# play-with-HOI-generation/HOIG

Hardware: AMD Instinct MI355X
Metric: HOGAN train images/sec at 256x256 (higher is better)
Workload: dtype f16x3 fwd (both operands split hi+lo on fp16, 3 MFMAs per product) / bf16x2 bwd (dy split hi+lo, weights and x single bf16, 2 MFMAs per product), f32 accumulate; 1 GPU; 256x256 HO3Dv3-shaped synthetic, batch 8 per GPU, G+D full step (generator_spade_attn, VGG19 surrogate weights); global_batch=8, parallelism=dp1

## Files before the change

hoig_amd/csrc/conv_bf16_common.h:

```cpp
#pragma once
#include "common.h"

namespace hoig_detail {

#define HOIG_NS_SWITCH(ns, ...)                                                \
    do {                                                                       \
        if ((ns) == 2) { constexpr int NSX = 2; __VA_ARGS__; }                 \
        else if ((ns) == 3) { constexpr int NSX = 3; __VA_ARGS__; }            \
        else { constexpr int NSX = 1; __VA_ARGS__; }                           \
    } while (0)
#define HOIG_F16_SWITCH(flag, ...)                                             \
    do {                                                                       \
        if (flag) { constexpr bool F16X = true; __VA_ARGS__; }                 \
        else { constexpr bool F16X = false; __VA_ARGS__; }                     \
    } while (0)
__host__ __device__ constexpr int ns_a(int nsx) { return nsx == 1 ? 1 : 2; }
__host__ __device__ constexpr int ns_b(int nsx) { return nsx == 2 ? 2 : 1; }
inline int ns_of_precision(int precision) {
    return precision == HOIG_PREC_BF16X3 ? 2 : (precision == HOIG_PREC_F16X2 ? 3 : 1);
}
inline bool is_16bit_precision(int precision) {
    return precision == HOIG_PREC_BF16X3 || precision == HOIG_PREC_BF16 || precision == HOIG_PREC_F16X2;
}

typedef __bf16 bf2_t __attribute__((ext_vector_type(2)));
typedef float f2_t __attribute__((ext_vector_type(2)));
__device__ __forceinline__ unsigned cvt2(float a, float b) {
    f2_t v = {a, b};
    return __builtin_bit_cast(unsigned, __builtin_convertvector(v, bf2_t));
}
typedef _Float16 h2_t __attribute__((ext_vector_type(2)));
typedef _Float16 f16x8 __attribute__((ext_vector_type(8)));
constexpr float W_SCALE_F16 = 256.f;
__device__ __forceinline__ unsigned cvt2h(float a, float b) {
    f2_t v = {a, b};
    return __builtin_bit_cast(unsigned, __builtin_convertvector(v, h2_t));
}
__device__ __forceinline__ void split4h(const float4 v, uint2 &hi, uint2 &lo) {
    hi.x = cvt2h(v.x, v.y);
    hi.y = cvt2h(v.z, v.w);
    const h2_t h0 = __builtin_bit_cast(h2_t, hi.x), h1 = __builtin_bit_cast(h2_t, hi.y);
    lo.x = cvt2h(v.x - (float)h0[0], v.y - (float)h0[1]);
    lo.y = cvt2h(v.z - (float)h1[0], v.w - (float)h1[1]);
}
template <bool F16>
__device__ __forceinline__ f32x16 mfma16(const bf16x8 a, const bf16x8 b, const f32x16 c) {
    if constexpr (F16)
        return __builtin_amdgcn_mfma_f32_32x32x16_f16(__builtin_bit_cast(f16x8, a), __builtin_bit_cast(f16x8, b), c, 0, 0, 0);
    else
        return __builtin_amdgcn_mfma_f32_32x32x16_bf16(a, b, c, 0, 0, 0);
}

__device__ __forceinline__ void split4(const float4 v, uint2 &hi, uint2 &lo) {
    hi.x = cvt2(v.x, v.y);
    hi.y = cvt2(v.z, v.w);
    const float r0 = v.x - __uint_as_float(hi.x << 16), r1 = v.y - __uint_as_float(hi.x & 0xFFFF0000u);
    const float r2 = v.z - __uint_as_float(hi.y << 16), r3 = v.w - __uint_as_float(hi.y & 0xFFFF0000u);
    lo.x = cvt2(r0, r1);
    lo.y = cvt2(r2, r3);
}
template <bool F16>
__device__ __forceinline__ void split4t(const float4 v, uint2 &hi, uint2 &lo) {
    if constexpr (F16) split4h(v, hi, lo);
    else split4(v, hi, lo);
}

__host__ __device__ __forceinline__ size_t plane_index(int n, int k, int K) {
    return ((size_t)(n >> 5) * (K >> 5) + (k >> 5)) * 1024 + (n & 31) * 32 + (((((k & 31) >> 3) ^ ((n >> 2) & 3))) << 3) +
           (k & 7);
}

struct HaloArgs {
    const float *A = nullptr;
    const unsigned short *Wh = nullptr, *Wl = nullptr;
    const float *bias = nullptr;
    float *C = nullptr;
    int Bn = 0, H = 0, W = 0, Cg = 0;
    int N = 0, K = 0;
    int pad = 0;
    int flip = 0;
    int act = 0;
    float slope = 0.f;
    int nblk_n = 0, nblk = 0;
    int tiles_x = 0, tiles_y = 0;
    int nmajor = 0;
    int f16 = 0;
    float oscale = 0.f;
    const float *A2 = nullptr;
    int cg1 = 0;
    float *C2 = nullptr;
    int n1 = 0;
    const float *addend = nullptr;
    const float *in_scale = nullptr, *in_shift = nullptr;
    int in_relu_c0 = 0;
    int b_split = 0;
    const float *A_g2 = nullptr;
    const unsigned short *Wh_g2 = nullptr, *Wl_g2 = nullptr;
    const float *bias_g2 = nullptr, *addend_g2 = nullptr;
    float *C_g2 = nullptr;
    int a_split = 0;
    double *stats = nullptr;
};

struct Geom {
    int Bn = 0, Hg = 0, Wg = 0, Cg = 0;
    int Hp = 0, Wp = 0;
    int R = 0, S = 0, stride = 0, pad = 0;
    int gatherT = 0, phase_major = 0, tile_skip = 0;
};

struct Args {
    const float *A = nullptr;
    const unsigned short *Wh = nullptr;
    const unsigned short *Wl = nullptr;
    const float *bias = nullptr;
    float *C = nullptr;
    Geom g;
    int M = 0, N = 0, K = 0;
    int act = 0;
    float slope = 0.f;
    int nblk_n = 0, nblk = 0;
    int ksplit = 0, steps_per_split = 0;
    int f16 = 0;
    float oscale = 0.f;
};

__device__ __forceinline__ void decode_m(const Geom &g, int m, int &b, int &hp, int &wp) {
    if (!g.phase_major) {
        const int hw = g.Hp * g.Wp;
        b = m / hw;
        const int rem = m - b * hw;
        hp = rem / g.Wp;
        wp = rem - hp * g.Wp;
    } else {
        const int W2 = g.Wp >> 1, q = (g.Hp >> 1) * W2, bq = g.Bn * q;
        const int ph = m / bq;
        const int rem = m - ph * bq;
        b = rem / q;
        const int r2 = rem - b * q;
        const int h2 = r2 / W2;
        hp = 2 * h2 + (ph >> 1);
        wp = 2 * (r2 - h2 * W2) + (ph & 1);
    }
}
__device__ __forceinline__ int row_base(const Geom &g, int p) { return g.gatherT ? p + g.pad : p * g.stride - g.pad; }
__device__ __forceinline__ int gcoord(const Geom &g, int base, int r, int lim) {
    if (!g.gatherT) {
        const int c = base + r;
        return (c >= 0 && c < lim) ? c : -1;
    }
    int t = base - r;
    if (t < 0) return -1;
    if (g.stride == 2) {
        if (t & 1) return -1;
        t >>= 1;
    } else if (g.stride != 1) {
        if (t % g.stride) return -1;
        t /= g.stride;
    }
    return t < lim ? t : -1;
}
__device__ __forceinline__ bool tap_alive(const Geom &g, int hp, int wp, int rs) {
    const int r = rs / g.S, s = rs - r * g.S;
    return (((hp + g.pad - r) & 1) == 0) && (((wp + g.pad - s) & 1) == 0);
}

struct WFlatArgs {
    const float *X = nullptr, *DY = nullptr;
    float *DW = nullptr, *DB = nullptr;
    int Ci = 0, Co = 0, Wc = 0, HWc = 0, Q = 0, Ho = 0, Wo = 0, HPOS = 0;
    int nblk_ci = 0, nblk = 0, n_mtiles = 0, mt_per_split = 0;
};
int launch_wgrad_flat5(const float *x, const float *dy, float *dw, float *dbias, int Bn, int Hi, int Wi, int Ci, int Co, int ns,
                       hipStream_t st);

int launch_igemm_m16(Args a, int ns, int cfg, hipStream_t st);

struct FlatArgs {
    const float *A = nullptr;
    const unsigned short *Wh = nullptr, *Wl = nullptr;
    const float *bias = nullptr;
    float *C = nullptr;
    const float *addend = nullptr;
    int Bn = 0, Hc = 0, Wc = 0;
    int Hs = 0, Ws = 0, oy = 0, ox = 0;
    int Hd = 0, Wd = 0;
    int KS = 0, Cg = 0, N = 0, K = 0, flip = 0, f16 = 0;
    int act = 0;
    float slope = 0.f, oscale = 0.f;
    int HWc = 0, Q = 0, HP = 0;
    int nblk = 0, nblk_n = 0, steps_per_split = 0;
};
int launch_flat_m16(FlatArgs a, int ns, hipStream_t st);
int launch_halo5_m16(FlatArgs a, int ns, hipStream_t st);

struct WHaloArgs {
    const float *DY = nullptr, *X = nullptr, *X2 = nullptr;
    int ci1 = 0;
    float *DW = nullptr, *DB = nullptr;
    int Bn = 0, H = 0, W = 0, Co = 0, Ci = 0;
    int Hin = 0, Win = 0, pad = 0;
    int tout = 0;
    int tiles_x = 0, tiles_y = 0, n_mtiles = 0, mt_per_split = 0;
    int nblk_ci = 0, nblk = 0;
    int b_split = 0;
    const float *DY_g2 = nullptr, *X_g2 = nullptr;
    float *DW_g2 = nullptr;
};

int launch_halo_s2_m16p(const HaloArgs &a, int ns, bool scatter, bool rows8, hipStream_t st);
int launch_dgrad_thin(const float *dy, const unsigned short *wh, const unsigned short *wl, float *dx, int M, int N, int ns, hipStream_t st);
int launch_wgrad_dma(const WHaloArgs &a, int ns, dim3 grid, hipStream_t st);

int launch_halo3_m16(HaloArgs a, int ns, int bn, hipStream_t st);
int launch_halo_s2_m16(const HaloArgs &a, int ns, bool scatter, hipStream_t st);

template <int KS>
int launch_halo(HaloArgs a, int ns, hipStream_t st);
int launch_halo3(HaloArgs a, int ns, hipStream_t st);
template <bool SCATTER>
int launch_halo_s2(HaloArgs a, int ns, hipStream_t st);

}
```

hoig_amd/csrc/conv_halo16.hip:

```cpp
#include "conv_bf16_common.h"
#include "conv_m16_common.h"
#include "tuning.h"

namespace hoig_detail {
namespace {

template <int WM, int BN>
struct M16Layout {
    static constexpr int TH = 2 * WM, HW = 34, HPIX = (TH + 2) * HW;
    static constexpr int PHALF = HPIX * 32;
    static constexpr int P23 = round128(PHALF) + 64;
    static constexpr int PLANE_P = round128(P23 + PHALF);
    static constexpr int W23 = BN * 32 + 64;
    static constexpr int PLANE_W = round128(W23 + BN * 32);
    static constexpr size_t bytes(int nsx) { return (size_t)ns_a(nsx) * PLANE_P + 2 * 3 * ns_b(nsx) * PLANE_W; }
};

template <int NSX, int WM, int WN, int BN, bool F16, bool ASPLIT = false, bool WDMA = false, bool NORMIN = false>
__global__ __launch_bounds__(64 * WM * WN) void conv_halo3_m16_kernel(const HaloArgs p) {
    constexpr int NS = NSX == 1 ? 1 : 2, NB = NSX == 2 ? 2 : 1;
    using LY = M16Layout<WM, BN>;
    constexpr int KS = 3, TH = LY::TH, HW = LY::HW, HPIX = LY::HPIX;
    constexpr int NT = 64 * WM * WN;
    constexpr int P23 = LY::P23, PLANE_P = LY::PLANE_P, W23 = LY::W23, PLANE_W = LY::PLANE_W;
    constexpr int RB = BN * 4 >= NT ? BN * 4 / NT : 1;
    constexpr bool B_PART = BN * 4 < NT;
    constexpr int MT = 4;
    constexpr int NTW = BN / (16 * WN);
    constexpr int ABUF = NS * PLANE_P, BBUF = KS * NB * PLANE_W;
    extern __shared__ __attribute__((aligned(16))) unsigned char smem[];
    unsigned char *Pbase = smem;
    unsigned char *Wbase = smem + ABUF;

    const int tid = threadIdx.x, lane = tid & 63, wave = tid >> 6;
    const int l15 = lane & 15, lg = lane >> 4;
    const int wm = wave / WN, wn = wave % WN;
    const int tile = hoig_xcd_remap(blockIdx.x, p.nblk);
    const int n_mt = p.nblk / p.nblk_n;
    int mt_ = p.nmajor ? tile % n_mt : tile / p.nblk_n;
    const int n0 = (p.nmajor ? tile / n_mt : tile % p.nblk_n) * BN;
    const int tx_ = mt_ % p.tiles_x;
    mt_ /= p.tiles_x;
    const int ty_ = mt_ % p.tiles_y, b = mt_ / p.tiles_y;
    const int y0 = ty_ * TH, x0 = tx_ * 32;
    const bool g2 = p.b_split > 0 && b >= p.b_split;
    const int bi = g2 ? b - p.b_split : b;
    const float *const gA = g2 ? p.A_g2 : p.A;
    const unsigned short *const gWh = g2 ? p.Wh_g2 : p.Wh, *const gWl = g2 ? p.Wl_g2 : p.Wl;
    const float *const gbias = g2 ? p.bias_g2 : p.bias, *const gadd = g2 ? p.addend_g2 : p.addend;
    float *const gC = g2 ? p.C_g2 : p.C;

    const int brow = tid >> 2, bpos = tid & 3;
    const unsigned short *wrow_h[RB], *wrow_l[RB];
    int woff[RB];
#pragma unroll
    for (int i = 0; i < RB; ++i) {
        const int row = brow + (NT / 4) * i;
        const int n = n0 + row;
        const bool ok = n < p.N && (!B_PART || row < BN);
        const size_t o = ((size_t)(n >> 5) * (p.K >> 5)) * 1024 + (n & 31) * 32 + bpos * 8;
        wrow_h[i] = ok ? gWh + o : nullptr;
        wrow_l[i] = (NB == 2 && ok) ? gWl + o : nullptr;
        const int c = bpos ^ ((row >> 2) & 3);
        woff[i] = (c >> 1) * W23 + row * 32 + (c & 1) * 16;
    }
    int wread[NTW], pread[MT];
#pragma unroll
    for (int j = 0; j < NTW; ++j) wread[j] = (lg >> 1) * W23 + (wn * (NTW * 16) + j * 16 + l15) * 32 + (lg & 1) * 16;
#pragma unroll
    for (int m = 0; m < MT; ++m)
        pread[m] = (lg >> 1) * P23 + ((wm * 2 + (m >> 1)) * HW + (m & 1) * 16 + l15) * 32 + (lg & 1) * 16;

    f32x4 acc[NTW][MT];
#pragma unroll
    for (int j = 0; j < NTW; ++j)
#pragma unroll
        for (int m = 0; m < MT; ++m) acc[j][m] = f32x4{0.f, 0.f, 0.f, 0.f};

    uint4 rbh[KS][RB], rbl[KS][RB];
    const int ncb = p.Cg >> 5, T = ncb * KS;
    auto load_b = [&](int step) {
        const int cb = step / KS, r = step - cb * KS;
#pragma unroll
        for (int t = 0; t < KS; ++t) {
            const int tap = r * KS + t;
            const int wtap = p.flip ? (KS * KS - 1 - tap) : tap;
            const size_t koff = (size_t)(wtap * p.Cg + cb * 32) * 32;
#pragma unroll
            for (int i = 0; i < RB; ++i) {
                rbh[t][i] = wrow_h[i] ? *reinterpret_cast<const uint4 *>(wrow_h[i] + koff) : make_uint4(0, 0, 0, 0);
                if (NB == 2)
                    rbl[t][i] = wrow_l[i] ? *reinterpret_cast<const uint4 *>(wrow_l[i] + koff) : make_uint4(0, 0, 0, 0);
            }
        }
    };
    auto store_b = [&](int buf) {
#pragma unroll
        for (int t = 0; t < KS; ++t) {
            unsigned char *Wh = Wbase + buf * BBUF + t * NB * PLANE_W, *Wl = Wh + PLANE_W;
#pragma unroll
            for (int i = 0; i < RB; ++i) {
                if (B_PART && brow >= BN) continue;
                *reinterpret_cast<uint4 *>(Wh + woff[i]) = rbh[t][i];
                if (NB == 2) *reinterpret_cast<uint4 *>(Wl + woff[i]) = rbl[t][i];
            }
        }
    };
    constexpr int NPIECE_STEP = KS * NB * (BN / 32) * 2, NPW = (NPIECE_STEP + WM * WN - 1) / (WM * WN);
    const int wave_u = __builtin_amdgcn_readfirstlane(wave);
    const unsigned lds_w0 = __builtin_amdgcn_readfirstlane((unsigned)(size_t)(__attribute__((address_space(3))) unsigned char *)Wbase);
    const int drow = lane >> 1;
    const unsigned dlane0 = drow * 32 + (((0 + (lane & 1)) ^ ((drow >> 2) & 3)) << 3);
    const unsigned dlane1 = drow * 32 + (((2 + (lane & 1)) ^ ((drow >> 2) & 3)) << 3);
    auto dma_piece = [&](int step, int buf, int i) {
        const int q = wave_u + (WM * WN) * i;
        if (q >= NPIECE_STEP) return;
        const int h = q & 1, blk = (q >> 1) % (BN / 32), tp = (q >> 1) / (BN / 32);
        const int t = tp / NB, pl = tp - t * NB;
        const int cb = step / KS, r = step - cb * KS;
        const int tap = r * KS + t;
        const int wtap = p.flip ? (KS * KS - 1 - tap) : tap;
        const size_t koff = (size_t)(wtap * p.Cg + cb * 32) * 32;
        const unsigned short *plane = pl ? gWl : gWh;
        const unsigned short *src = plane + ((size_t)((n0 >> 5) + blk) * (p.K >> 5)) * 1024 + koff + (h ? dlane1 : dlane0);
        const unsigned to = __builtin_amdgcn_readfirstlane(lds_w0 + buf * BBUF + tp * PLANE_W + h * W23 + blk * 1024);
        unsigned keep;
        asm volatile("s_mov_b32 %0, m0\n\ts_mov_b32 m0, %2\n\ts_nop 0\n\tglobal_load_lds_dwordx4 %1, off\n\ts_mov_b32 m0, %0"
                     : "=&s"(keep) : "v"(src), "s"(to) : "memory");
    };
    constexpr int HSLICES = (HPIX * 8 + NT - 1) / NT;
    float4 hreg[HSLICES];
    float4 nsc = make_float4(1.f, 1.f, 1.f, 1.f), nsh = make_float4(0.f, 0.f, 0.f, 0.f);
    bool nrelu = false;
    unsigned hin = 0;
    auto halo_load = [&](int cb) {
        if constexpr (ASPLIT) {
            const unsigned short *Aimg = reinterpret_cast<const unsigned short *>(gA) + (size_t)bi * p.H * p.W * 2 * p.Cg + cb * 32;
#pragma unroll
            for (int sl = 0; sl < HSLICES; ++sl) {
                const int i = tid + NT * sl;
                float4 v = make_float4(0.f, 0.f, 0.f, 0.f);
                if (i < HPIX * 8 && (NS == 2 || !(i & 4))) {
                    const int pix = i >> 3, plane = (i >> 2) & 1, c8 = i & 3;
                    const int hy = pix / HW, hx = pix - hy * HW;
                    const int gy = y0 - p.pad + hy, gx = x0 - p.pad + hx;
                    if (gy >= 0 && gy < p.H && gx >= 0 && gx < p.W)
                        v = *reinterpret_cast<const float4 *>(Aimg + ((size_t)gy * p.W + gx) * 2 * p.Cg + plane * p.Cg + c8 * 8);
                }
                hreg[sl] = v;
            }
            return;
        }
        const bool second = p.A2 != nullptr && cb * 32 >= p.cg1;
        const int ld = p.A2 ? (second ? p.Cg - p.cg1 : p.cg1) : p.Cg;
        const float *Aimg = (second ? p.A2 : gA) + (size_t)bi * p.H * p.W * ld + (second ? cb * 32 - p.cg1 : cb * 32);
        if constexpr (NORMIN) {
            const size_t co = (size_t)bi * p.Cg + cb * 32 + (tid & 7) * 4;
            nsc = *reinterpret_cast<const float4 *>(p.in_scale + co);
            nsh = *reinterpret_cast<const float4 *>(p.in_shift + co);
            nrelu = cb * 32 + (tid & 7) * 4 >= p.in_relu_c0;
            hin = 0;
        }
#pragma unroll
        for (int sl = 0; sl < HSLICES; ++sl) {
            const int i = tid + NT * sl;
            float4 v = make_float4(0.f, 0.f, 0.f, 0.f);
            if (i < HPIX * 8) {
                const int pix = i >> 3, c4 = i & 7;
                const int hy = pix / HW, hx = pix - hy * HW;
                const int gy = y0 - p.pad + hy, gx = x0 - p.pad + hx;
                if (gy >= 0 && gy < p.H && gx >= 0 && gx < p.W) {
                    v = *reinterpret_cast<const float4 *>(Aimg + ((size_t)gy * p.W + gx) * ld + c4 * 4);
                    if constexpr (NORMIN) hin |= 1u << sl;
                }
            }
            hreg[sl] = v;
        }
    };
    auto halo_store = [&]() {
        unsigned char *Ph = Pbase, *Pl = Ph + PLANE_P;
        if constexpr (ASPLIT) {
#pragma unroll
            for (int sl = 0; sl < HSLICES; ++sl) {
                const int i = tid + NT * sl;
                if (i < HPIX * 8 && (NS == 2 || !(i & 4))) {
                    const int pix = i >> 3, plane = (i >> 2) & 1, c8 = i & 3;
                    *reinterpret_cast<float4 *>(Pbase + plane * PLANE_P + (c8 >> 1) * P23 + pix * 32 + (c8 & 1) * 16) = hreg[sl];
                }
            }
            return;
        }
#pragma unroll
        for (int sl = 0; sl < HSLICES; ++sl) {
            const int i = tid + NT * sl;
            if (i < HPIX * 8) {
                const int pix = i >> 3, c4 = i & 7;
                uint2 hi, lo;
                float4 v = hreg[sl];
                if constexpr (NORMIN) {
                    if ((hin >> sl) & 1u) {
                        v.x = fmaf(v.x, nsc.x, nsh.x); v.y = fmaf(v.y, nsc.y, nsh.y);
                        v.z = fmaf(v.z, nsc.z, nsh.z); v.w = fmaf(v.w, nsc.w, nsh.w);
                        if (nrelu) { v.x = fmaxf(v.x, 0.f); v.y = fmaxf(v.y, 0.f); v.z = fmaxf(v.z, 0.f); v.w = fmaxf(v.w, 0.f); }
                    }
                }
                split4t<F16>(v, hi, lo);
                const int off = (c4 >> 2) * P23 + pix * 32 + (c4 & 3) * 8;
                *reinterpret_cast<uint2 *>(Ph + off) = hi;
                if (NS == 2) *reinterpret_cast<uint2 *>(Pl + off) = lo;
            }
        }
    };

    struct PF {
        bf16x8 h[MT], l[MT];
    };
    struct WF {
        bf16x8 h, l;
    };
    auto compute = [&](int r, int bbuf, int dma_step) {
        const unsigned char *Ph = Pbase, *Pl = Ph + PLANE_P;
        const unsigned char *Wst = Wbase + bbuf * BBUF;
        auto read_p = [&](PF &f, int t, int m) {
            const int off = pread[m] + (r * HW + t) * 32;
            f.h[m] = *reinterpret_cast<const bf16x8 *>(Ph + off);
            if (NS == 2) f.l[m] = *reinterpret_cast<const bf16x8 *>(Pl + off);
        };
        auto read_w = [&](WF &f, int t, int j) {
            const unsigned char *Wh = Wst + t * NB * PLANE_W, *Wl = Wh + PLANE_W;
            f.h = *reinterpret_cast<const bf16x8 *>(Wh + wread[j]);
            if (NB == 2) f.l = *reinterpret_cast<const bf16x8 *>(Wl + wread[j]);
        };
        PF pf[2];
        WF wf[2];
#pragma unroll
        for (int m = 0; m < MT; ++m) read_p(pf[0], 0, m);
        read_w(wf[0], 0, 0);
        constexpr int NG = KS * NTW;
        constexpr int PPG = (MT + NTW - 1) / NTW;
#pragma unroll
        for (int g = 0; g < NG; ++g) {
            const int t = g / NTW, j = g % NTW;
            if (g + 1 < NG) read_w(wf[(g + 1) & 1], (g + 1) / NTW, (g + 1) % NTW);
            if (t + 1 < KS) {
#pragma unroll
                for (int q = 0; q < PPG; ++q)
                    if (j * PPG + q < MT) read_p(pf[(t + 1) & 1], t + 1, j * PPG + q);
            }
            if constexpr (WDMA) {
                if (dma_step >= 0 && g < NPW) dma_piece(dma_step, bbuf ^ 1, g);
            }
            __builtin_amdgcn_sched_barrier(0);
            const PF &pc = pf[t & 1];
            const WF &wc = wf[g & 1];
#pragma unroll
            for (int m = 0; m < MT; ++m) {
                if (NS == 2) acc[j][m] = mfma_m16<F16>(wc.h, pc.l[m], acc[j][m]);
                if (NB == 2) acc[j][m] = mfma_m16<F16>(wc.l, pc.h[m], acc[j][m]);
                acc[j][m] = mfma_m16<F16>(wc.h, pc.h[m], acc[j][m]);
            }
            __builtin_amdgcn_sched_barrier(0);
        }
    };

    halo_load(0);
    halo_store();
    if constexpr (WDMA) {
#pragma unroll
        for (int i = 0; i < NPW; ++i) dma_piece(0, 0, i);
        asm volatile("s_waitcnt vmcnt(0)" ::: "memory");
    } else {
        load_b(0);
        store_b(0);
        if (T > 1) load_b(1);
    }
    __syncthreads();
    int bbuf = 0;
#pragma unroll 1
    for (int step = 0; step < T; ++step) {
        const int cb = step / KS, r = step - cb * KS;
        const bool more = step + 1 < T;
        const bool boundary = more && r == KS - 1;
        if constexpr (!WDMA) {
            if (more) store_b(bbuf ^ 1);
            if (step + 2 < T) load_b(step + 2);
        }
        if (boundary) halo_load(cb + 1);
        compute(r, bbuf, (WDMA && more) ? step + 1 : -1);
        if (boundary) {
            __syncthreads();
            halo_store();
        }
        if constexpr (WDMA) asm volatile("s_waitcnt vmcnt(0)" ::: "memory");
        __syncthreads();
        bbuf ^= 1;
    }

    const float nslope = p.act == HOIG_ACT_NONE ? 1.f : (p.act == HOIG_ACT_RELU ? 0.f : p.slope);
    const bool special = p.act == HOIG_ACT_TANH || p.act == HOIG_ACT_SIGMOID;
    float4 bias_r[NTW];
#pragma unroll
    for (int j = 0; j < NTW; ++j) {
        const int n = n0 + wn * (NTW * 16) + j * 16 + lg * 4;
        bias_r[j] = (gbias && n < p.N) ? *reinterpret_cast<const float4 *>(gbias + n) : make_float4(0.f, 0.f, 0.f, 0.f);
    }
    float st1[NTW][4], st2[NTW][4];
#pragma unroll
    for (int j = 0; j < NTW; ++j)
#pragma unroll
        for (int q = 0; q < 4; ++q) st1[j][q] = st2[j][q] = 0.f;
#pragma unroll
    for (int m = 0; m < MT; ++m) {
        const int oy = y0 + wm * 2 + (m >> 1), ox = x0 + (m & 1) * 16 + l15;
        const size_t pix = ((size_t)bi * p.H + oy) * p.W + ox;
#pragma unroll
        for (int j = 0; j < NTW; ++j) {
            const int n = n0 + wn * (NTW * 16) + j * 16 + lg * 4;
            if (n < p.N) {
                float v[4];
                const float bq[4] = {bias_r[j].x, bias_r[j].y, bias_r[j].z, bias_r[j].w};
#pragma unroll
                for (int q = 0; q < 4; ++q) v[q] = fast_act(acc[j][m][q] * p.oscale + bq[q], nslope, special, p.act, p.slope);
                if (gadd) {
                    const float4 ad = *reinterpret_cast<const float4 *>(gadd + pix * p.N + n);
                    v[0] += ad.x; v[1] += ad.y; v[2] += ad.z; v[3] += ad.w;
                }
#pragma unroll
                for (int q = 0; q < 4; ++q) {
                    st1[j][q] += v[q];
                    st2[j][q] += v[q] * v[q];
                }
                const float4 o = make_float4(v[0], v[1], v[2], v[3]);
                if (!p.C2) *reinterpret_cast<float4 *>(gC + pix * p.N + n) = o;
                else if (n < p.n1) *reinterpret_cast<float4 *>(gC + pix * p.n1 + n) = o;
                else *reinterpret_cast<float4 *>(p.C2 + pix * (p.N - p.n1) + (n - p.n1)) = o;
            }
        }
    }
    if (p.stats) m16_stats_epilogue<NTW, WM, BN, NT>(st1, st2, smem, p.stats, b, p.N, n0, wm, wn, lane, tid);
}

template <int NSX, int BN, bool SCATTER, bool F16>
__global__ __launch_bounds__(256) void conv_halo_s2_m16_kernel(const HaloArgs p) {
    constexpr int NS = NSX == 1 ? 1 : 2, NB = NSX == 2 ? 2 : 1;
    constexpr int TH = 4, TW = 32, NT = 256, WN = 2;
    constexpr int RB = BN * 4 / NT;
    constexpr int HH = TH + 1, HW = TW + 1, HPIX = HH * HW;
    constexpr int PHALF = HPIX * 32, P23 = round128(PHALF) + 64, PLANE_P = round128(P23 + PHALF);
    constexpr int W23 = BN * 32 + 64, PLANE_W = round128(W23 + BN * 32);
    constexpr int MT = 4, NTW = BN / (16 * WN);
    __shared__ __attribute__((aligned(16))) unsigned char smem[NS * PLANE_P + 2 * NB * PLANE_W];
    unsigned char *Ph = smem, *Pl = smem + PLANE_P;
    unsigned char *Wbase = smem + NS * PLANE_P;

    const int tid = threadIdx.x, lane = tid & 63, wave = tid >> 6;
    const int l15 = lane & 15, lg = lane >> 4;
    const int wm = wave / WN, wn = wave % WN;
    int tile = hoig_xcd_remap(blockIdx.x, p.nblk);
    int P = 0, Q = 0;
    if (SCATTER) {
        P = (tile >> 1) & 1;
        Q = tile & 1;
        tile >>= 2;
    }
    int mt_ = tile / p.nblk_n;
    const int n0 = (tile % p.nblk_n) * BN;
    const int tx_ = mt_ % p.tiles_x;
    mt_ /= p.tiles_x;
    const int ty_ = mt_ % p.tiles_y, b = mt_ / p.tiles_y;
    const int y0 = ty_ * TH, x0 = tx_ * TW;

    const int brow = tid >> 2, bpos = tid & 3;
    const unsigned short *wrow_h[RB], *wrow_l[RB];
    int woff[RB];
#pragma unroll
    for (int i = 0; i < RB; ++i) {
        const int row = brow + (NT / 4) * i;
        const int n = n0 + row;
        const size_t o = ((size_t)(n >> 5) * (p.K >> 5)) * 1024 + (n & 31) * 32 + bpos * 8;
        wrow_h[i] = n < p.N ? p.Wh + o : nullptr;
        wrow_l[i] = (NB == 2 && n < p.N) ? p.Wl + o : nullptr;
        const int c = bpos ^ ((row >> 2) & 3);
        woff[i] = (c >> 1) * W23 + row * 32 + (c & 1) * 16;
    }
    int wread[NTW], pread[MT];
#pragma unroll
    for (int j = 0; j < NTW; ++j) wread[j] = (lg >> 1) * W23 + (wn * (NTW * 16) + j * 16 + l15) * 32 + (lg & 1) * 16;
#pragma unroll
    for (int m = 0; m < MT; ++m)
        pread[m] = (lg >> 1) * P23 + ((wm * 2 + (m >> 1)) * HW + (m & 1) * 16 + l15) * 32 + (lg & 1) * 16;

    f32x4 acc[NTW][MT];
#pragma unroll
    for (int j = 0; j < NTW; ++j)
#pragma unroll
        for (int m = 0; m < MT; ++m) acc[j][m] = f32x4{0.f, 0.f, 0.f, 0.f};

    struct Step {
        int cb, ntap, tap[2], pp, qq;
        bool load;
    };
    const int spc = SCATTER ? ((P ? 2 : 1) * (Q ? 2 : 1) + 1) / 2 : 5;
    const int ncb = p.Cg >> 5, T = ncb * spc;
    auto step_info = [&](int step) -> Step {
        Step s_;
        s_.cb = step / spc;
        const int idx = step - s_.cb * spc;
        s_.pp = s_.qq = 0;
        if (!SCATTER) {
            s_.load = idx != 1;
            switch (idx) {
                case 0: s_.pp = 1; s_.qq = 1; s_.ntap = 2; s_.tap[0] = 0; s_.tap[1] = 2; break;
                case 1: s_.pp = 1; s_.qq = 1; s_.ntap = 2; s_.tap[0] = 6; s_.tap[1] = 8; break;
                case 2: s_.pp = 1; s_.qq = 0; s_.ntap = 2; s_.tap[0] = 1; s_.tap[1] = 7; break;
                case 3: s_.pp = 0; s_.qq = 1; s_.ntap = 2; s_.tap[0] = 3; s_.tap[1] = 5; break;
                default: s_.ntap = 1; s_.tap[0] = 4; s_.tap[1] = 4; break;
            }
        } else {
            s_.load = idx == 0;
            const int r0 = P ? 0 : 1, r1 = 2, s0 = Q ? 0 : 1, s1 = 2;
            if (P && Q) {
                s_.ntap = 2;
                s_.tap[0] = (idx ? r1 : r0) * 3 + s0;
                s_.tap[1] = (idx ? r1 : r0) * 3 + s1;
            } else if (P) {
                s_.ntap = 2; s_.tap[0] = r0 * 3 + s0; s_.tap[1] = r1 * 3 + s0;
            } else if (Q) {
                s_.ntap = 2; s_.tap[0] = r0 * 3 + s0; s_.tap[1] = r0 * 3 + s1;
            } else {
                s_.ntap = 1; s_.tap[0] = s_.tap[1] = 4;
            }
        }
        return s_;
    };
    auto tap_off = [&](int tap) -> int {
        const int r = tap / 3, s_ = tap - r * 3;
        const int dr = SCATTER ? (r == 0) : (r != 0), dc = SCATTER ? (s_ == 0) : (s_ != 0);
        return (dr * HW + dc) * 32;
    };

    uint4 rbh[2][RB], rbl[2][RB];
    auto load_b = [&](const Step &s_) {
#pragma unroll
        for (int t = 0; t < 2; ++t) {
            const size_t koff = (size_t)(s_.tap[t] * p.Cg + s_.cb * 32) * 32;
#pragma unroll
            for (int i = 0; i < RB; ++i) {
                rbh[t][i] = wrow_h[i] ? *reinterpret_cast<const uint4 *>(wrow_h[i] + koff) : make_uint4(0, 0, 0, 0);
                if (NB == 2)
                    rbl[t][i] = wrow_l[i] ? *reinterpret_cast<const uint4 *>(wrow_l[i] + koff) : make_uint4(0, 0, 0, 0);
            }
        }
    };
    auto store_b = [&]() {
#pragma unroll
        for (int t = 0; t < 2; ++t) {
            unsigned char *Wh = Wbase + t * NB * PLANE_W, *Wl = Wh + PLANE_W;
#pragma unroll
            for (int i = 0; i < RB; ++i) {
                *reinterpret_cast<uint4 *>(Wh + woff[i]) = rbh[t][i];
                if (NB == 2) *reinterpret_cast<uint4 *>(Wl + woff[i]) = rbl[t][i];
            }
        }
    };
    const float *Aimg = p.A + (size_t)b * p.H * p.W * p.Cg;
    constexpr int HSLICES = (HPIX * 8 + NT - 1) / NT;
    float4 hregs[2][HSLICES];
    auto halo_load = [&](const Step &s_, float4 (&hreg)[HSLICES]) {
#pragma unroll
        for (int sl = 0; sl < HSLICES; ++sl) {
            const int i = tid + NT * sl;
            float4 v = make_float4(0.f, 0.f, 0.f, 0.f);
            if (i < HPIX * 8) {
                const int pix = i >> 3, c4 = i & 7;
                const int hy = pix / HW, hx = pix - hy * HW;
                const int gy = SCATTER ? y0 + hy : 2 * (y0 - 1 + hy) + s_.pp;
                const int gx = SCATTER ? x0 + hx : 2 * (x0 - 1 + hx) + s_.qq;
                if (gy >= 0 && gy < p.H && gx >= 0 && gx < p.W)
                    v = *reinterpret_cast<const float4 *>(Aimg + ((size_t)gy * p.W + gx) * p.Cg + s_.cb * 32 + c4 * 4);
            }
            hreg[sl] = v;
        }
    };
    auto halo_store = [&](const float4 (&hreg)[HSLICES]) {
#pragma unroll
        for (int sl = 0; sl < HSLICES; ++sl) {
            const int i = tid + NT * sl;
            if (i < HPIX * 8) {
                const int pix = i >> 3, c4 = i & 7;
                uint2 hi, lo;
                split4t<F16>(hreg[sl], hi, lo);
                const int off = (c4 >> 2) * P23 + pix * 32 + (c4 & 3) * 8;
                *reinterpret_cast<uint2 *>(Ph + off) = hi;
                if (NS == 2) *reinterpret_cast<uint2 *>(Pl + off) = lo;
            }
        }
    };
    auto compute = [&](const Step &s_) {
#pragma unroll
        for (int t = 0; t < 2; ++t) {
            if (t >= s_.ntap) break;
            const int tapoff = tap_off(s_.tap[t]);
            const unsigned char *Wh = Wbase + t * NB * PLANE_W, *Wl = Wh + PLANE_W;
            bf16x8 ph[MT], pl[MT];
#pragma unroll
            for (int m = 0; m < MT; ++m) {
                ph[m] = *reinterpret_cast<const bf16x8 *>(Ph + pread[m] + tapoff);
                if (NS == 2) pl[m] = *reinterpret_cast<const bf16x8 *>(Pl + pread[m] + tapoff);
            }
            bf16x8 wh[2], wl[2];
            wh[0] = *reinterpret_cast<const bf16x8 *>(Wh + wread[0]);
            if (NB == 2) wl[0] = *reinterpret_cast<const bf16x8 *>(Wl + wread[0]);
#pragma unroll
            for (int j = 0; j < NTW; ++j) {
                if (j + 1 < NTW) {
                    wh[(j + 1) & 1] = *reinterpret_cast<const bf16x8 *>(Wh + wread[j + 1]);
                    if (NB == 2) wl[(j + 1) & 1] = *reinterpret_cast<const bf16x8 *>(Wl + wread[j + 1]);
                }
                __builtin_amdgcn_sched_barrier(0);
#pragma unroll
                for (int m = 0; m < MT; ++m) {
                    if (NS == 2) acc[j][m] = mfma_m16<F16>(wh[j & 1], pl[m], acc[j][m]);
                    if (NB == 2) acc[j][m] = mfma_m16<F16>(wl[j & 1], ph[m], acc[j][m]);
                    acc[j][m] = mfma_m16<F16>(wh[j & 1], ph[m], acc[j][m]);
                }
                __builtin_amdgcn_sched_barrier(0);
            }
        }
    };

    Step cur = step_info(0);
    halo_load(cur, hregs[0]);
    load_b(cur);
    halo_store(hregs[0]);
    store_b();
    Step nxt = cur;
    if (T > 1) {
        nxt = step_info(1);
        if (nxt.load) halo_load(nxt, hregs[1]);
    }
    __syncthreads();
    auto one_step = [&](int step, float4 (&mine)[HSLICES], float4 (&other)[HSLICES]) {
        const bool more = step + 1 < T;
        if (more) load_b(nxt);
        if (step + 2 < T) {
            const Step n2 = step_info(step + 2);
            if (n2.load) halo_load(n2, mine);
        }
        compute(cur);
        if (more) {
            __syncthreads();
            if (nxt.load) halo_store(other);
            store_b();
            __syncthreads();
            cur = nxt;
            if (step + 2 < T) nxt = step_info(step + 2);
        }
    };
#pragma unroll 1
    for (int step = 0; step < T; step += 2) {
        one_step(step, hregs[0], hregs[1]);
        if (step + 1 < T) one_step(step + 1, hregs[1], hregs[0]);
    }

    const float nslope = p.act == HOIG_ACT_NONE ? 1.f : (p.act == HOIG_ACT_RELU ? 0.f : p.slope);
    const bool special = p.act == HOIG_ACT_TANH || p.act == HOIG_ACT_SIGMOID;
    float4 bias_r[NTW];
#pragma unroll
    for (int j = 0; j < NTW; ++j) {
        const int n = n0 + wn * (NTW * 16) + j * 16 + lg * 4;
        bias_r[j] = (p.bias && n < p.N) ? *reinterpret_cast<const float4 *>(p.bias + n) : make_float4(0.f, 0.f, 0.f, 0.f);
    }
    float st1[NTW][4], st2[NTW][4];
#pragma unroll
    for (int j = 0; j < NTW; ++j)
#pragma unroll
        for (int q = 0; q < 4; ++q) st1[j][q] = st2[j][q] = 0.f;
    const int Ho = SCATTER ? 2 * p.H : p.tiles_y * TH, Wo = SCATTER ? 2 * p.W : p.tiles_x * TW;
#pragma unroll
    for (int m = 0; m < MT; ++m) {
        const int cy = y0 + wm * 2 + (m >> 1), cx = x0 + (m & 1) * 16 + l15;
        const int oy = SCATTER ? 2 * cy + P : cy, ox = SCATTER ? 2 * cx + Q : cx;
        const size_t pix = ((size_t)b * Ho + oy) * Wo + ox;
#pragma unroll
        for (int j = 0; j < NTW; ++j) {
            const int n = n0 + wn * (NTW * 16) + j * 16 + lg * 4;
            if (n < p.N) {
                float v[4];
                const float bq[4] = {bias_r[j].x, bias_r[j].y, bias_r[j].z, bias_r[j].w};
#pragma unroll
                for (int q = 0; q < 4; ++q) v[q] = fast_act(acc[j][m][q] * p.oscale + bq[q], nslope, special, p.act, p.slope);
                if (p.addend) {
                    const float4 ad = *reinterpret_cast<const float4 *>(p.addend + pix * p.N + n);
                    v[0] += ad.x; v[1] += ad.y; v[2] += ad.z; v[3] += ad.w;
                }
#pragma unroll
                for (int q = 0; q < 4; ++q) {
                    st1[j][q] += v[q];
                    st2[j][q] += v[q] * v[q];
                }
                *reinterpret_cast<float4 *>(p.C + pix * p.N + n) = make_float4(v[0], v[1], v[2], v[3]);
            }
        }
    }
    if (p.stats) m16_stats_epilogue<NTW, 2, BN, NT>(st1, st2, smem, p.stats, b, p.N, n0, wm, wn, lane, tid);
}

template <int NS, int BN>
int launch_one(const HaloArgs &a, hipStream_t st) {
    constexpr int WM = 4, WN = 2;
    constexpr int shm = (int)M16Layout<WM, BN>::bytes(NS);
    const dim3 grid(a.nblk), block(64 * WM * WN);
    const bool wdma = hoig_tuning(HOIG_TUNE_WDMA16) != 0 && a.N % BN == 0;
    if (a.a_split) {
        if (a.in_scale) return HOIG_EUNSUPPORTED;
        if constexpr (NS == 2) return HOIG_EUNSUPPORTED;
        else {
            if (a.f16 || a.A2) return HOIG_EUNSUPPORTED;
            if (a.b_split > 0) BN == 64 ? HOIG_ROUTE_D(halo3_m16_64_split_pair) : HOIG_ROUTE_D(halo3_m16_128_split_pair);
            else BN == 64 ? HOIG_ROUTE_D(halo3_m16_64_split) : HOIG_ROUTE_D(halo3_m16_128_split);
            if (wdma) return hoig_launch<conv_halo3_m16_kernel<NS, WM, WN, BN, false, true, true>, shm>(grid, block, shm, st, a);
            return hoig_launch<conv_halo3_m16_kernel<NS, WM, WN, BN, false, true>, shm>(grid, block, shm, st, a);
        }
    }
    if (a.in_scale) {
        if (!a.f16 || a.N % BN || !a.in_shift || a.b_split > 0) return HOIG_EUNSUPPORTED;
        BN == 64 ? HOIG_ROUTE_F(halo3_m16_64_normin) : HOIG_ROUTE_F(halo3_m16_128_normin);
        return hoig_launch<conv_halo3_m16_kernel<NS, WM, WN, BN, true, false, true, true>, shm>(grid, block, shm, st, a);
    }
    if (a.b_split > 0 && a.f16) BN == 64 ? HOIG_ROUTE_F(halo3_m16_64_pair) : HOIG_ROUTE_F(halo3_m16_128_pair);
    else if (BN == 64) HOIG_ROUTE_FD(a.f16, halo3_m16_64);
    else HOIG_ROUTE_FD(a.f16, halo3_m16_128);
    HOIG_F16_SWITCH(a.f16,
                    if (wdma) return hoig_launch<conv_halo3_m16_kernel<NS, WM, WN, BN, F16X, false, true>, shm>(grid, block, shm, st, a);
                    return hoig_launch<conv_halo3_m16_kernel<NS, WM, WN, BN, F16X>, shm>(grid, block, shm, st, a));
}

template <bool SCATTER>
int launch_s2(const HaloArgs &a, int ns, hipStream_t st) {
    const bool n64 = (a.N % 128) != 0;
    const int pipe = hoig_tuning(HOIG_TUNE_S2_PIPE);
    const bool rows8_ok = a.nblk >= 512 && !(a.tiles_y & 1) && a.N % 128 == 0;
    if (rows8_ok && (pipe == 1 || pipe == 3)) return launch_halo_s2_m16p(a, ns, SCATTER, true, st);
    if (pipe == 2 || (pipe != 0 && a.nblk <= 256)) return launch_halo_s2_m16p(a, ns, SCATTER, false, st);
    if (n64) SCATTER ? HOIG_ROUTE_FD(a.f16, s2s_m16_64) : HOIG_ROUTE_FD(a.f16, s2g_m16_64);
    else SCATTER ? HOIG_ROUTE_FD(a.f16, s2s_m16_128) : HOIG_ROUTE_FD(a.f16, s2g_m16_128);
    if (n64)
        HOIG_NS_SWITCH(ns, HOIG_F16_SWITCH(a.f16, return hoig_launch<conv_halo_s2_m16_kernel<NSX, 64, SCATTER, F16X>>(a.nblk, 256, 0, st, a)));
    HOIG_NS_SWITCH(ns, HOIG_F16_SWITCH(a.f16, return hoig_launch<conv_halo_s2_m16_kernel<NSX, 128, SCATTER, F16X>>(a.nblk, 256, 0, st, a)));
}

}

int launch_halo_s2_m16(const HaloArgs &a, int ns, bool scatter, hipStream_t st) {
    if (a.N % 64 || a.Cg % 32) return HOIG_EUNSUPPORTED;
    return scatter ? launch_s2<true>(a, ns, st) : launch_s2<false>(a, ns, st);
}

int launch_halo3_m16(HaloArgs a, int ns, int bn, hipStream_t st) {
    if (a.H % 8 || a.W % 32 || a.Cg % 32 || a.N % 4) return HOIG_EUNSUPPORTED;
    if (a.b_split > 0 && (a.A2 || a.C2 || a.stats || a.b_split >= a.Bn)) return HOIG_EUNSUPPORTED;
    if (bn == 128) HOIG_NS_SWITCH(ns, return launch_one<NSX, 128>(a, st));
    if (bn == 64) HOIG_NS_SWITCH(ns, return launch_one<NSX, 64>(a, st));
    return HOIG_EUNSUPPORTED;
}

}
```

hoig_amd/csrc/conv_igemm_bf16.hip:

```cpp
#include "conv_bf16_common.h"
#include "tuning.h"
#include <cstdlib>

namespace {
using namespace hoig_detail;

template <int BK>
__device__ __forceinline__ int lds_swz(int row) {
    return BK == 32 ? ((row >> 2) & 3) : ((row >> 1) & 7);
}
template <int BK>
__device__ __forceinline__ int lds_off(int row, int k) {
    return row * (BK * 2) + (((k >> 3) ^ lds_swz<BK>(row)) << 4) + ((k & 4) << 1);
}

template <int BM, int BN, int WM, int WN, int NSX, int BK, bool F16>
__global__ __launch_bounds__(WM * WN * 64) void igemm_bf16_kernel(const Args p) {
    constexpr int NS = NSX == 1 ? 1 : 2, NB = NSX == 2 ? 2 : 1;
    constexpr int NT = WM * WN * 64;
    constexpr int TM = BM / (32 * WM), TN = BN / (32 * WN);
    constexpr int TPR_A = BK / 4, TPR_B = BK / 8;
    constexpr int RA = BM * TPR_A / NT;
    constexpr int RB = BN * TPR_B / NT;
    constexpr int AROWS = NT / TPR_A, BROWS = NT / TPR_B;
// ... 134 lines not shown
    int cur = 0;
    while (more) {
        const bool nxt = advance();
        if (nxt) load_tiles();
        const unsigned char *Ah = smem + cur * STAGE, *Al = Ah + PLANE_A;
        const unsigned char *Bh = Ah + NS * PLANE_A, *Bl = Bh + PLANE_B;
#pragma unroll
        for (int ks = 0; ks < BK / 16; ++ks) {
            bf16x8 ah[TM], al[TM], bhf[TN], blf[TN];
#pragma unroll
            for (int i = 0; i < TM; ++i) {
                const int off = aread[i] ^ (ks << 5);
                ah[i] = *reinterpret_cast<const bf16x8 *>(Ah + off);
                if (NS == 2) al[i] = *reinterpret_cast<const bf16x8 *>(Al + off);
            }
#pragma unroll
            for (int j = 0; j < TN; ++j) {
                const int off = bread[j] ^ (ks << 5);
                bhf[j] = *reinterpret_cast<const bf16x8 *>(Bh + off);
                if (NB == 2) blf[j] = *reinterpret_cast<const bf16x8 *>(Bl + off);
            }
#pragma unroll
            for (int i = 0; i < TM; ++i)
#pragma unroll
                for (int j = 0; j < TN; ++j) {
                    if (NS == 2)
                        acc[i][j] = mfma16<F16>(al[i], bhf[j], acc[i][j]);
                        if (NB == 2) acc[i][j] = mfma16<F16>(ah[i], blf[j], acc[i][j]);
                    acc[i][j] = mfma16<F16>(ah[i], bhf[j], acc[i][j]);
                }
        }
        if (NSTAGE == 2) {
            if (nxt) store_tiles(cur ^ 1);
            __syncthreads();
            cur ^= 1;
        } else {
            __syncthreads();
            if (nxt) store_tiles(0);
            __syncthreads();
        }
        more = nxt;
    }

    const float nslope = p.act == HOIG_ACT_NONE ? 1.f : (p.act == HOIG_ACT_RELU ? 0.f : p.slope);
    const bool special = p.act == HOIG_ACT_TANH || p.act == HOIG_ACT_SIGMOID;
    float bias_r[TN];
#pragma unroll
    for (int j = 0; j < TN; ++j) {
        const int n = n0 + wn * (TN * 32) + j * 32 + l31;
        bias_r[j] = (p.bias && n < p.N) ? p.bias[n] : 0.f;
    }
#pragma unroll
    for (int i = 0; i < TM; ++i) {
#pragma unroll
        for (int r = 0; r < 16; ++r) {
            const int m = m0 + wm * (TM * 32) + i * 32 + (r & 3) + 8 * (r >> 2) + 4 * lh;
            if (m >= p.M) continue;
            size_t pix = m;
            if (g.phase_major) {
                int b, hp, wp;
                decode_m(g, m, b, hp, wp);
                pix = ((size_t)b * g.Hp + hp) * g.Wp + wp;
            }
#pragma unroll
            for (int j = 0; j < TN; ++j) {
                const int n = n0 + wn * (TN * 32) + j * 32 + l31;
                if (n < p.N) {
                    float v = acc[i][j][r] * p.oscale;
                    if (p.ksplit > 1) {
                        if (blockIdx.y == 0) v += bias_r[j];
                        atomicAdd(&p.C[pix * p.N + n], v);
                    } else {
                        v += bias_r[j];
                        p.C[pix * p.N + n] = fast_act(v, nslope, special, p.act, p.slope);
                    }
                }
            }
        }
    }
}

template <int BM, int BN, int WM, int WN, int BK = 32>
int launch(Args a, int ns, hipStream_t st) {
    constexpr int NT = WM * WN * 64;
    const int nbm = (int)hoig_cdiv(a.M, BM), nbn = (int)hoig_cdiv(a.N, BN);
    a.nblk_n = nbn;
    a.nblk = nbm * nbn;
    if (a.g.gatherT && a.g.stride == 2 && (a.g.Hp % 2 == 0) && (a.g.Wp % 2 == 0)) {
        a.g.phase_major = 1;
        const long per_phase = (long)a.g.Bn * (a.g.Hp / 2) * (a.g.Wp / 2);
        a.g.tile_skip = (per_phase % BM == 0) ? 1 : 0;
    }
    a.ksplit = 1;
    a.steps_per_split = 0;
    const int steps = (a.K / BK);
    constexpr int sk_target = 1024;
    constexpr int sk_maxblk = 192;
    if (a.nblk < sk_maxblk && steps >= 32 && a.act == HOIG_ACT_NONE && !a.g.tile_skip) {
        int want = (int)hoig_cdiv(sk_target, a.nblk);
        if (want > steps / 8) want = steps / 8;
        if (want > 1) {
            a.steps_per_split = (int)hoig_cdiv(steps, want);
            a.ksplit = (int)hoig_cdiv(steps, a.steps_per_split);
            if (hipMemsetAsync(a.C, 0, (size_t)a.M * a.N * sizeof(float), st) != hipSuccess) return HOIG_ELAUNCH;
        }
    }
    dim3 grid(a.nblk, a.ksplit);
    if (BM == 128 && BN == 128) WN == 4 ? HOIG_ROUTE_FD(a.f16, igemm_bf16_128x128w) : HOIG_ROUTE_FD(a.f16, igemm_bf16_128x128);
    else if (BN == 128) HOIG_ROUTE_FD(a.f16, igemm_bf16_64x128);
    else if (BM == 128) HOIG_ROUTE_FD(a.f16, igemm_bf16_128x64);
    else HOIG_ROUTE_FD(a.f16, igemm_bf16_64x64);
    HOIG_NS_SWITCH(ns, HOIG_F16_SWITCH(a.f16, return hoig_launch<igemm_bf16_kernel<BM, BN, WM, WN, NSX, BK, F16X>>(grid, NT, 0, st, a)));
}

struct InNorm {
    const float *scale, *shift;
    int relu_c0;
};
struct PairSet {
    const float *a;
    const unsigned short *wh, *wl;
    const float *bias, *addend;
    float *c;
};

struct Conv {
    const hoig_conv_desc *d = nullptr;
    const float *a = nullptr;
    const unsigned short *wh = nullptr, *wl = nullptr;
    const float *bias = nullptr;
    float *c = nullptr;
    bool dgrad = false;
    hipStream_t st = nullptr;
    const float *a2 = nullptr;
    int cg1 = 0;
    float *c2 = nullptr;
    int n1 = 0;
    const float *addend = nullptr;
    double *stats = nullptr;
    bool a_split = false;
    const PairSet *g2 = nullptr;
    const InNorm *in = nullptr;
};

HaloArgs halo_args(const Conv &q, const Args &p) {
    HaloArgs h;
    h.A = q.a; h.Wh = q.wh; h.Wl = q.wl; h.bias = q.bias; h.C = q.c;
    h.Bn = q.d->B; h.Cg = p.g.Cg; h.N = p.N; h.K = p.K;
    h.act = p.act; h.slope = p.slope;
    h.f16 = p.f16; h.oscale = p.oscale;
    h.addend = q.addend;
    h.stats = q.stats;
    return h;
}
FlatArgs flat_args(const Conv &q, const Args &p, int ks) {
    FlatArgs f;
    f.A = q.a; f.Wh = q.wh; f.Wl = q.wl; f.bias = q.bias; f.C = q.c; f.addend = q.addend;
    f.Bn = q.d->B; f.KS = ks; f.act = p.act; f.slope = p.slope;
    f.Cg = p.g.Cg; f.N = p.N; f.K = p.K; f.flip = q.dgrad ? 1 : 0; f.f16 = p.f16; f.oscale = p.oscale;
    return f;
}

int run(const Conv &q) {
    const hoig_conv_desc *d = q.d;
    if (q.in && (q.dgrad || d->R != 3 || d->S != 3 || d->stride != 1 || d->pad != 1 || d->transposed || q.a_split || q.g2))
        return HOIG_EUNSUPPORTED;
    Args p;
    p.A = q.a; p.Wh = q.wh; p.Wl = q.wl; p.bias = q.bias; p.C = q.c;
    p.f16 = q.dgrad ? 0 : 1;
    p.oscale = q.dgrad ? 1.f : 1.f / W_SCALE_F16;
    Geom &g = p.g;
    g.Bn = d->B;
    if (!q.dgrad) {
        g.Hg = d->Hi; g.Wg = d->Wi; g.Cg = d->Ci; g.Hp = d->Ho; g.Wp = d->Wo;
        g.gatherT = d->transposed ? 1 : 0;
        p.M = d->B * d->Ho * d->Wo; p.N = d->Co; p.K = d->R * d->S * d->Ci;
        p.act = d->act; p.slope = d->slope;
    } else {
        g.Hg = d->Ho; g.Wg = d->Wo; g.Cg = d->Co; g.Hp = d->Hi; g.Wp = d->Wi;
        g.gatherT = d->transposed ? 0 : 1;
        p.M = d->B * d->Hi * d->Wi; p.N = d->Ci; p.K = d->R * d->S * d->Co;
        p.act = HOIG_ACT_NONE; p.slope = 0.f;
    }
    g.R = d->R; g.S = d->S; g.stride = d->stride; g.pad = d->pad;
    if (g.Cg % 32 != 0) return HOIG_EUNSUPPORTED;
    if (g.gatherT && g.stride == 2 && ((g.Hp | g.Wp) & 1)) return HOIG_EUNSUPPORTED;
    const int ns = ns_of_precision(d->precision);
    if (ns == 2 && !q.wl) return HOIG_EINVAL;
    const long t128 = hoig_cdiv(p.M, 128);
    if (p.N <= 32 || p.N % 32 != 0) return HOIG_EUNSUPPORTED;
    if (q.dgrad && !d->transposed && d->R == 1 && d->S == 1 && d->stride == 1 && d->pad == 0 && g.Cg == 128 &&
        p.N >= 1024 && p.N % 64 == 0 && p.M % 128 == 0 && !q.a2 && !q.c2 && !q.addend && !q.stats)
        return launch_dgrad_thin(q.a, q.wh, q.wl, q.c, p.M, p.N, ns, q.st);
    if (!d->transposed && d->stride == 1 && d->R == d->S && 2 * d->pad == d->R - 1 && (d->R == 1 || d->R == 3 || d->R == 5) &&
        d->Wi % 32 == 0 && d->Hi % 4 == 0 && p.N % 64 == 0 &&
        (long)(q.g2 ? 2 : 1) * d->B * (d->Hi / 4) * (d->Wi / 32) * ((p.N + 127) / 128) >= 160) {
        HaloArgs h = halo_args(q, p);
        h.A2 = q.a2; h.cg1 = q.cg1; h.C2 = q.c2; h.n1 = q.n1;
        h.a_split = q.a_split ? 1 : 0;
        if (q.in) { h.in_scale = q.in->scale; h.in_shift = q.in->shift; h.in_relu_c0 = q.in->relu_c0; }
        if (q.a_split && (d->R != 3 || q.a2 || !q.dgrad)) return HOIG_EUNSUPPORTED;
        if ((q.addend || q.stats) && q.c2) return HOIG_EUNSUPPORTED;
        if (q.stats && d->R != 3) return HOIG_EUNSUPPORTED;
        if ((q.a2 || q.c2) && d->R != 3) return HOIG_EUNSUPPORTED;
        if (q.a2 && (q.cg1 % 32 || q.cg1 <= 0 || q.cg1 >= g.Cg)) return HOIG_EINVAL;
        if (q.c2 && (q.n1 % 64 || q.n1 <= 0 || q.n1 >= p.N)) return HOIG_EINVAL;
        h.H = d->Hi; h.W = d->Wi;
        if (q.g2) {
            if (d->R != 3 || q.a2 || q.c2 || q.stats) return HOIG_EUNSUPPORTED;
            h.Bn = 2 * d->B; h.b_split = d->B;
            h.A_g2 = q.g2->a; h.Wh_g2 = q.g2->wh; h.Wl_g2 = q.g2->wl; h.bias_g2 = q.g2->bias; h.addend_g2 = q.g2->addend; h.C_g2 = q.g2->c;
        }
        h.pad = d->pad;
        h.flip = q.dgrad ? 1 : 0;
        if (d->R == 1) return launch_halo<1>(h, ns, q.st);
        if (d->R == 3) return launch_halo3(h, ns, q.st);
        return launch_halo<5>(h, ns, q.st);
    }
    if (q.a2 || q.c2 || q.a_split || q.g2 || q.in) return HOIG_EUNSUPPORTED;
    if (hoig_tuning(HOIG_TUNE_FLAT5) >= 2 && !d->transposed && d->stride == 1 && d->R == 3 && d->S == 3 && d->pad == 1 &&
        p.N % 128 == 0 && !q.stats) {
        FlatArgs f = flat_args(q, p, 3);
        f.Hc = d->Hi + 2; f.Wc = d->Wi + 2;
        f.Hs = d->Hi; f.Ws = d->Wi; f.oy = f.ox = 1; f.Hd = d->Hi; f.Wd = d->Wi;
        const int rc = launch_flat_m16(f, ns, q.st);
        if (rc != HOIG_EUNSUPPORTED) return rc;
    }
    if (hoig_tuning(HOIG_TUNE_FLAT5) != 0 && !d->transposed && d->stride == 1 && d->R == 5 && d->S == 5 && d->pad == 0 &&
        d->Ho == d->Hi - 4 && d->Wo == d->Wi - 4 && p.N % 128 == 0 && !q.stats) {
        FlatArgs f = flat_args(q, p, 5);
        f.Hc = d->Hi; f.Wc = d->Wi;
        if (!q.dgrad) {
            f.Hs = d->Hi; f.Ws = d->Wi; f.oy = f.ox = 0; f.Hd = d->Ho; f.Wd = d->Wo;
        } else {
            f.Hs = d->Ho; f.Ws = d->Wo; f.oy = f.ox = 4; f.Hd = d->Hi; f.Wd = d->Wi;
        }
        const int rc = launch_flat_m16(f, ns, q.st);
        if (rc != HOIG_EUNSUPPORTED) return rc;
        if (hoig_tuning(HOIG_TUNE_HALO5) != 0) {
            const int rc5 = launch_halo5_m16(f, ns, q.st);
            if (rc5 != HOIG_EUNSUPPORTED) return rc5;
        }
    }
    if (d->stride == 2 && d->R == 3 && d->S == 3 && d->pad == 1 && d->Hi % 2 == 0 && d->Wi % 2 == 0 &&
        p.N % 64 == 0) {
        const int fine_h = d->transposed ? d->Ho : d->Hi, fine_w = d->transposed ? d->Wo : d->Wi;
        const int coarse_h = d->transposed ? d->Hi : d->Ho, coarse_w = d->transposed ? d->Wi : d->Wo;
        if (fine_h == 2 * coarse_h && fine_w == 2 * coarse_w && coarse_w % 32 == 0 && coarse_h % 4 == 0) {
            HaloArgs h = halo_args(q, p);
            h.pad = 1;
            const bool gather = !g.gatherT;
            if (gather) {
                h.H = fine_h; h.W = fine_w;
                return launch_halo_s2<false>(h, ns, q.st);
            }
            h.H = coarse_h; h.W = coarse_w;
            return launch_halo_s2<true>(h, ns, q.st);
        }
    }
    if (q.addend || q.stats) return HOIG_EUNSUPPORTED;
    const int t16 = hoig_tuning(HOIG_TUNE_IGEMM16);
    const bool m16 = t16 >= 2 || (t16 == 1 && !q.dgrad);
    if (p.N <= 64) {
        if (t128 >= 512) return m16 ? launch_igemm_m16(p, ns, 3, q.st) : launch<128, 64, 2, 2>(p, ns, q.st);
        return m16 ? launch_igemm_m16(p, ns, 4, q.st) : launch<64, 64, 2, 2>(p, ns, q.st);
    }
    const long n128 = hoig_cdiv(p.N, 128);
    if (t128 * n128 >= 512) return m16 ? launch_igemm_m16(p, ns, 0, q.st) : launch<128, 128, 2, 2>(p, ns, q.st);
    if (t128 * n128 >= 128) return m16 ? launch_igemm_m16(p, ns, 1, q.st) : launch<128, 128, 2, 4>(p, ns, q.st);
    return m16 ? launch_igemm_m16(p, ns, 2, q.st) : launch<64, 128, 2, 2>(p, ns, q.st);
}

template <class... T>
bool usable(const hoig_conv_desc *d, const T *...needed) {
    return d && (... && needed) && is_16bit_precision(d->precision);
}

}

extern "C" int hoig_conv2d_fwd_packed(const hoig_conv_desc *d, const float *x, const uint16_t *w_hi, const uint16_t *w_lo,
                                      const float *bias, float *y, hoig_stream_t stream) {
    if (!usable(d, x, w_hi, y)) return HOIG_EINVAL;
    return run(Conv{.d = d, .a = x, .wh = w_hi, .wl = w_lo, .bias = bias, .c = y, .st = (hipStream_t)stream});
}

extern "C" int hoig_conv2d_bwd_data_packed(const hoig_conv_desc *d, const float *dy, const uint16_t *wt_hi,
                                           const uint16_t *wt_lo, float *dx, hoig_stream_t stream) {
    if (!usable(d, dy, wt_hi, dx)) return HOIG_EINVAL;
    return run(Conv{.d = d, .a = dy, .wh = wt_hi, .wl = wt_lo, .c = dx, .dgrad = true, .st = (hipStream_t)stream});
}

extern "C" int hoig_conv2d_fwd_packed_stats(const hoig_conv_desc *d, const float *x, const uint16_t *w_hi, const uint16_t *w_lo,
                                            const float *bias, float *y, double *stats, hoig_stream_t stream) {
    if (!usable(d, x, w_hi, y, stats)) return HOIG_EINVAL;
    return run(Conv{.d = d, .a = x, .wh = w_hi, .wl = w_lo, .bias = bias, .c = y, .st = (hipStream_t)stream, .stats = stats});
}
extern "C" int hoig_conv2d_cat_fwd_packed_stats(const hoig_conv_desc *d, const float *x1, int C1, const float *x2,
                                                const uint16_t *w_hi, const uint16_t *w_lo, const float *bias, float *y,
                                                double *stats, hoig_stream_t stream) {
    if (!usable(d, x1, x2, w_hi, y, stats)) return HOIG_EINVAL;
    return run(Conv{.d = d, .a = x1, .wh = w_hi, .wl = w_lo, .bias = bias, .c = y, .st = (hipStream_t)stream, .a2 = x2, .cg1 = C1, .stats = stats});
}

extern "C" int hoig_conv2d_fwd_packed_normin(const hoig_conv_desc *d, const float *x, int C1, const float *x2, const uint16_t *w_hi,
                                             const uint16_t *w_lo, const float *bias, const float *in_scale, const float *in_shift,
                                             int in_relu_c0, float *y, double *stats, hoig_stream_t stream) {
    if (!usable(d, x, w_hi, y, in_scale, in_shift) || in_relu_c0 < 0) return HOIG_EINVAL;
    const InNorm in{in_scale, in_shift, in_relu_c0};
    return run(Conv{.d = d, .a = x, .wh = w_hi, .wl = w_lo, .bias = bias, .c = y, .st = (hipStream_t)stream, .a2 = x2, .cg1 = x2 ? C1 : 0,
                    .stats = stats, .in = &in});
}

extern "C" int hoig_conv2d_bwd_data_packed_add(const hoig_conv_desc *d, const float *dy, const uint16_t *wt_hi,
                                               const uint16_t *wt_lo, const float *addend, float *dx, hoig_stream_t stream) {
    if (!usable(d, dy, wt_hi, dx, addend)) return HOIG_EINVAL;
    return run(Conv{.d = d, .a = dy, .wh = wt_hi, .wl = wt_lo, .c = dx, .dgrad = true, .st = (hipStream_t)stream, .addend = addend});
}

extern "C" int hoig_conv2d_bwd_data_packed_split(const hoig_conv_desc *d, const uint16_t *dy_split, const uint16_t *wt_hi,
                                                 const uint16_t *wt_lo, const float *addend, float *dx, hoig_stream_t stream) {
    if (!usable(d, dy_split, wt_hi, dx)) return HOIG_EINVAL;
    if (d->precision == HOIG_PREC_BF16X3 || d->transposed || d->stride != 1 || d->R != 3 || d->S != 3) return HOIG_EUNSUPPORTED;
    return run(Conv{.d = d, .a = reinterpret_cast<const float *>(dy_split), .wh = wt_hi, .wl = wt_lo, .c = dx, .dgrad = true,
                    .st = (hipStream_t)stream, .addend = addend, .a_split = true});
}

extern "C" int hoig_conv2d_fwd_packed_pair(const hoig_conv_desc *d, const float *xa, const float *xb, const uint16_t *wa_hi,
                                           const uint16_t *wa_lo, const uint16_t *wb_hi, const uint16_t *wb_lo, const float *bias_a,
                                           const float *bias_b, float *ya, float *yb, hoig_stream_t stream) {
    if (!usable(d, xa, xb, wa_hi, wb_hi, ya, yb)) return HOIG_EINVAL;
    if (d->transposed || d->stride != 1 || d->R != 3 || d->S != 3) return HOIG_EUNSUPPORTED;
    const PairSet g2{xb, wb_hi, wb_lo, bias_b, nullptr, yb};
    return run(Conv{.d = d, .a = xa, .wh = wa_hi, .wl = wa_lo, .bias = bias_a, .c = ya, .st = (hipStream_t)stream, .g2 = &g2});
}
extern "C" int hoig_conv2d_bwd_data_packed_split_pair(const hoig_conv_desc *d, const uint16_t *dys_a, const uint16_t *dys_b,
                                                      const uint16_t *wta_hi, const uint16_t *wta_lo, const uint16_t *wtb_hi,
                                                      const uint16_t *wtb_lo, const float *addend_a, const float *addend_b, float *dxa,
                                                      float *dxb, hoig_stream_t stream) {
    if (!usable(d, dys_a, dys_b, wta_hi, wtb_hi, dxa, dxb)) return HOIG_EINVAL;
    if (d->precision == HOIG_PREC_BF16X3 || d->transposed || d->stride != 1 || d->R != 3 || d->S != 3) return HOIG_EUNSUPPORTED;
    if ((addend_a == nullptr) != (addend_b == nullptr)) return HOIG_EINVAL;
    const PairSet g2{reinterpret_cast<const float *>(dys_b), wtb_hi, wtb_lo, nullptr, addend_b, dxb};
    return run(Conv{.d = d, .a = reinterpret_cast<const float *>(dys_a), .wh = wta_hi, .wl = wta_lo, .c = dxa, .dgrad = true,
                    .st = (hipStream_t)stream, .addend = addend_a, .a_split = true, .g2 = &g2});
}

extern "C" int hoig_conv2d_cat_fwd_packed(const hoig_conv_desc *d, const float *x1, int C1, const float *x2,
                                          const uint16_t *w_hi, const uint16_t *w_lo, const float *bias, float *y,
                                          hoig_stream_t stream) {
    if (!usable(d, x1, x2, w_hi, y)) return HOIG_EINVAL;
    return run(Conv{.d = d, .a = x1, .wh = w_hi, .wl = w_lo, .bias = bias, .c = y, .st = (hipStream_t)stream, .a2 = x2, .cg1 = C1});
}
extern "C" int hoig_conv2d_cat_bwd_data_packed(const hoig_conv_desc *d, const float *dy, const uint16_t *wt_hi,
                                               const uint16_t *wt_lo, float *dx1, int C1, float *dx2,
                                               hoig_stream_t stream) {
    if (!usable(d, dy, wt_hi, dx1, dx2)) return HOIG_EINVAL;
    return run(Conv{.d = d, .a = dy, .wh = wt_hi, .wl = wt_lo, .c = dx1, .dgrad = true, .st = (hipStream_t)stream, .c2 = dx2, .n1 = C1});
}
```

hoig_amd/csrc/conv_route.h:

```cpp
#pragma once

#define HOIG_CONV_ROUTES(W, D, F, FD)                                                                                              \
          \
    W(wgrad_thin_in_ws) W(wgrad_thin_in_direct) W(wgrad_thin_out_ws) W(wgrad_thin_out_direct)                                      \
    W(wgrad_small)                                                                                                                 \
                                                                                        \
    W(wgrad_flat5) W(wgrad_tile5)                                                                                                  \
                                                                 \
    W(wgrad_halo_th4) W(wgrad_halo_cm2) W(wgrad_halo_cm1) W(wgrad_halo_s2_cm2) W(wgrad_halo_s2_cm1) W(wgrad_halo_5x5)              \
    W(wgrad_halo_tout)        \
                                                                                                  \
    W(wgrad_dma) W(wgrad_dma_pair)                                                                                                 \
    W(wgrad_bf16_64) W(wgrad_bf16_128)                                                                                             \
                                                                                 \
    W(wgrad_f32_32x64) W(wgrad_f32_32x128) W(wgrad_f32_64x128) W(wgrad_f32_128x64) W(wgrad_f32_128x128)                            \
                                                                                 \
    FD(igemm_f32_128x32) FD(igemm_f32_128x64) FD(igemm_f32_64x64) FD(igemm_f32_128x128) FD(igemm_f32_64x128)                       \
                           \
    FD(halo1_64) FD(halo1_128w) FD(halo1_128) FD(same5_64) FD(same5_128w) FD(same5_128)                                            \
                                                                                                             \
    FD(halo3_64) FD(halo3_128w) FD(halo3_128)                                                                                      \
         \
    FD(halo3_m16_64) FD(halo3_m16_128)                                                                                             \
    D(halo3_m16_64_split) D(halo3_m16_128_split) D(halo3_m16_64_split_pair) D(halo3_m16_128_split_pair)                            \
    F(halo3_m16_64_pair) F(halo3_m16_128_pair) F(halo3_m16_64_normin) F(halo3_m16_128_normin)                                      \
                                                   \
    FD(flat_m16_k3) FD(flat_m16_k5) FD(halo5_m16) FD(halo5_m16_ksplit)                                                             \
     \
    FD(s2g_64) FD(s2g_128) FD(s2s_64) FD(s2s_128)                                                                                  \
    FD(s2g_m16_64) FD(s2g_m16_128) FD(s2s_m16_64) FD(s2s_m16_128)                                                                  \
    FD(s2g_m16p4_64) FD(s2g_m16p4_128) FD(s2s_m16p4_64) FD(s2s_m16p4_128) FD(s2g_m16p8_128) FD(s2s_m16p8_128)                      \
                   \
    FD(igemm_m16_128x128) FD(igemm_m16_128x128w) FD(igemm_m16_64x128) FD(igemm_m16_128x64) FD(igemm_m16_64x64)                     \
    FD(igemm_bf16_128x128) FD(igemm_bf16_128x128w) FD(igemm_bf16_64x128) FD(igemm_bf16_128x64) FD(igemm_bf16_64x64)                \
                                                                                \
    D(k128) D(thin) D(thin_out) D(small)                                                                                           \
    F(head7) F(small) F(small_ci) F(dot) F(thin) F(thin_out)                                                                       \
                                        \
    F(f6_64) F(f6_128) F(f6_64_normin) F(f6_128_normin)

enum HoigConvRoute {
    HOIG_ROUTE_NONE = 0,
#define HOIG_R_W(n) HOIG_ROUTE_##n,
#define HOIG_R_D(n) HOIG_ROUTE_dgrad_##n,
#define HOIG_R_F(n) HOIG_ROUTE_fwd_##n,
#define HOIG_R_FD(n) HOIG_ROUTE_fwd_##n, HOIG_ROUTE_dgrad_##n,
    HOIG_CONV_ROUTES(HOIG_R_W, HOIG_R_D, HOIG_R_F, HOIG_R_FD)
#undef HOIG_R_W
#undef HOIG_R_D
#undef HOIG_R_F
#undef HOIG_R_FD
    HOIG_ROUTE_COUNT
};

enum { HOIG_PASS_FWD = 0, HOIG_PASS_DGRAD = 1, HOIG_PASS_WGRAD = 2 };

extern thread_local int hoig_route_last[3];

static inline void hoig_route_set(int which, int id) { hoig_route_last[which] = id; }
#define HOIG_ROUTE_W(name) hoig_route_set(HOIG_PASS_WGRAD, HOIG_ROUTE_##name)
#define HOIG_ROUTE_F(name) hoig_route_set(HOIG_PASS_FWD, HOIG_ROUTE_fwd_##name)
#define HOIG_ROUTE_D(name) hoig_route_set(HOIG_PASS_DGRAD, HOIG_ROUTE_dgrad_##name)
#define HOIG_ROUTE_FD(fwd, name) ((fwd) ? HOIG_ROUTE_F(name) : HOIG_ROUTE_D(name))
```

hoig_amd/csrc/tuning.h:

```cpp
#pragma once
enum HoigTuning { HOIG_TUNE_IGEMM16 = 0, HOIG_TUNE_S2_16, HOIG_TUNE_FLAT5, HOIG_TUNE_WFLAT5, HOIG_TUNE_HEAD16, HOIG_TUNE_D_EARLY, HOIG_TUNE_SPLIT_GRADS, HOIG_TUNE_PAIR, HOIG_TUNE_WDMA16, HOIG_TUNE_S2_PIPE, HOIG_TUNE_NORM_IN, HOIG_TUNE_WINO8, HOIG_TUNE_HALO5, HOIG_TUNE_PNG_WINDOW, HOIG_TUNE_COUNT };
int hoig_tuning(int id);
```

hoig_amd/csrc/tuning.hip:

```cpp
#include <cstring>
#include "hoig_kernels.h"
#include "tuning.h"
#include "conv_route.h"

namespace {
struct Entry {
    const char *key;
    int value;
};
Entry g_table[HOIG_TUNE_COUNT] = {
    {"igemm16", 1},
    {"s2_16", 1},
    {"flat5", 2},
    {"wflat5", 1},
    {"head16", 1},
    {"d_early", 1},
    {"split_grads", 1},
    {"pair", 2},
    {"wdma16", 2},
    {"s2_pipe", 1},
    {"norm_in", 1},
    {"wino8", 0},
    {"halo5", 1},
    {"png_window", 0},
};
}

int hoig_tuning(int id) { return (id >= 0 && id < HOIG_TUNE_COUNT) ? g_table[id].value : 0; }

extern "C" int hoig_set_tuning(const char *key, int value) {
    if (!key) return -1;
    for (int i = 0; i < HOIG_TUNE_COUNT; ++i)
        if (strcmp(g_table[i].key, key) == 0) {
            const int prev = g_table[i].value;
            if (value >= 0) g_table[i].value = value;
            return prev;
        }
    return -1;
}

thread_local int hoig_route_last[3] = {0, 0, 0};

extern "C" int hoig_conv_last_route(int which) { return (which >= 0 && which < 3) ? hoig_route_last[which] : -1; }

extern "C" const char *hoig_conv_route_name(int id) {
    static const char *const names[HOIG_ROUTE_COUNT] = {
        "none",
#define HOIG_R_W(n) #n,
#define HOIG_R_D(n) "dgrad_" #n,
#define HOIG_R_F(n) "fwd_" #n,
#define HOIG_R_FD(n) "fwd_" #n, "dgrad_" #n,
        HOIG_CONV_ROUTES(HOIG_R_W, HOIG_R_D, HOIG_R_F, HOIG_R_FD)
#undef HOIG_R_W
#undef HOIG_R_D
#undef HOIG_R_F
#undef HOIG_R_FD
    };
    return (id >= 0 && id < HOIG_ROUTE_COUNT) ? names[id] : nullptr;
}
```

hoig_amd/models/networks/generator.py:

```python
import os

import torch

from ... import ops
from ..._lib import ACT_NONE, ACT_RELU, ACT_TANH, ACT_SIGMOID
from ...nn import ParamTree
from .schema import GeneratorConfig, generator_schema


def to_nhwc(t):
    if t is None:
        return None
    v = t.permute(0, 2, 3, 1)
    if v.is_contiguous():
        return v
    return ops.nchw_to_nhwc(t)


def as_nchw(t):
    return t.permute(0, 3, 1, 2)


_FORK_STREAMS = os.environ.get('HOIG_STREAMS', '1') == '1'


def forks_streams():
    return _FORK_STREAMS


class Generator(ParamTree):
    def __init__(self, bg_dim, img_dim, obj_dim, img_cond_dim=0, obj_cond_dim=0, conv_dim=64, repeat_num=6,
                 gen_name='generator_spade_attn', device=None):
        self.cfg = GeneratorConfig(gen_name, bg_dim, img_dim, obj_dim, img_cond_dim, obj_cond_dim, conv_dim, repeat_num)
        sch = generator_schema(self.cfg)
        device = device if device is not None else torch.device('cuda', torch.cuda.current_device())
        split = ['attn_%d.fully_connect_layer.0.weight' % l for l in self.cfg.attn_layers]
        split += ['%s.attetion_reg_bg.0.weight' % m for m in ('src_model', 'tsf_model')]
        heads_y = ['obj_model.img_reg.0.weight'] + ['%s.attetion_reg_bg.0.weight#s' % m for m in ('src_model', 'tsf_model')]
        super().__init__(sch.shapes, device, sch.transposed, split, adjacent=[heads_y])
        self._name = 'generator'
        self._seg_cache = {}
        for m in ('src_model', 'tsf_model'):
            names = [m + '.img_reg.0.weight', m + '.attetion_reg_hand.0.weight', m + '.attetion_reg_bg.0.weight#t']
            self.fuse_conv_weights(m + '.heads_x.weight', names)
        self.fuse_conv_weights('obj_model.heads_y.weight', heads_y)

    @property
    def name(self):
        return self._name

    def _branch_streams(self, device):
        if getattr(self, '_streams', None) is None:
            self._streams = tuple(ops.new_stream(device, role) for role in ('g_bg', 'g_obj', 'g_src'))
        return self._streams

    def _conv(self, x, name, stride=1, pad=1, act=ACT_NONE, to_norm=False):
        return ops.conv2d(x, self.P[name + '.weight'], self.P.get(name + '.bias'), stride, pad, act, dead_bias=to_norm)

    def _convT(self, x, name):
        return ops.conv_transpose2d(x, self.P[name + '.weight'], norm_next=True)

    def _in(self, x, name, act=ACT_NONE, residual=None):
        return ops.instance_norm(x, self.P[name + '.weight'], self.P[name + '.bias'], act=act, residual=residual)

    def _seg_at(self, seg, h, w):
        key = (id(seg), h, w)
        if key not in self._seg_cache:
            self._seg_cache[key] = ops.resize_nearest(seg, h, w)
        return self._seg_cache[key]

    def _spade(self, x, seg, name, act, fork=False):
        s = self._seg_at(seg, x.shape[1], x.shape[2])
        actv = self._conv(s, name + '.mlp_shared.0', act=ACT_RELU)
        if name + '.mlp_gb.weight' in self.F:
            gb = ops.conv2d(actv, self.F[name + '.mlp_gb.weight'], self.F[name + '.mlp_gb.bias'], 1, 1)
            return ops.spade_norm_fused(x, gb, act=act, fork=fork)
        gamma = self._conv(actv, name + '.mlp_gamma')
        beta = self._conv(actv, name + '.mlp_beta')
        y = ops.spade_norm(x, gamma, beta, act=act)
        return (y, x) if fork else y

    def _conv_fork(self, x, name, stride=1, pad=1):
        return ops.conv2d_fork(x, self.P[name + '.weight'], self.P.get(name + '.bias'), stride, pad, dead_bias=True)

    def _conv_in_relu(self, x, name, stride=1, pad=1, transposed=False, fork=False):
        if fork:
            h, x = self._conv_fork(x, name + '.0', stride, pad)
            return self._in(h, name + '.1', act=ACT_RELU), x
        h = self._convT(x, name + '.0') if transposed else self._conv(x, name + '.0', stride, pad, to_norm=True)
        return self._in(h, name + '.1', act=ACT_RELU)

    def _resblock(self, x, name):
        if not torch.is_grad_enabled():
            with ops.small_map_sums():
                h = self._conv(x, name + '.main.0', to_norm=True)
            y = ops.conv2d_after_norm(h, self.P[name + '.main.1.weight'], self.P[name + '.main.1.bias'], self.P[name + '.main.3.weight'],
                                      self.P.get(name + '.main.3.bias'), norm_next=True)
            if y is None:
                y = self._conv(self._in(h, name + '.main.1', act=ACT_RELU), name + '.main.3', to_norm=True)
            return self._in(y, name + '.main.4', residual=x)
        h, x = self._conv_fork(x, name + '.main.0')
        h = self._in(h, name + '.main.1', act=ACT_RELU)
        return self._in(self._conv(h, name + '.main.3', to_norm=True), name + '.main.4', residual=x)

    def _spade_resblock(self, x, seg, name):
        h, x = self._spade(x, seg, name + '.norm_0', ACT_RELU, fork=True)
        dx = self._conv(h, name + '.conv_0', to_norm=True)
        dx = self._conv(self._spade(dx, seg, name + '.norm_1', ACT_RELU), name + '.conv_1')
        return ops.add(x, dx)

    def _resblock_pair(self, sx, tx, ns, nt, sy):
        on_src, to_main, to_src = sy
        P = self.P
        hs, ht, sx, tx = ops.conv2d_pair(to_main(sx), tx, P[ns + '.main.0.weight'], P[nt + '.main.0.weight'], dead_bias=True, fork=True)
        to_src(hs); to_src(sx)
        with on_src():
            hs = self._in(hs, ns + '.main.1', act=ACT_RELU)
        ht = self._in(ht, nt + '.main.1', act=ACT_RELU)
        hs, ht = ops.conv2d_pair(to_main(hs), ht, P[ns + '.main.3.weight'], P[nt + '.main.3.weight'], dead_bias=True)
        to_src(hs)
        with on_src():
            sx = self._in(hs, ns + '.main.4', residual=sx)
        return sx, self._in(ht, nt + '.main.4', residual=tx)

    def _spade_resblock_pair(self, sx, tx, segs, segt, ns, nt, sy):
        on_src, to_main, to_src = sy
        P = self.P
        with on_src():
            hs, sx = self._spade(sx, segs, ns + '.norm_0', ACT_RELU, fork=True)
        ht, tx = self._spade(tx, segt, nt + '.norm_0', ACT_RELU, fork=True)
        ds, dt = ops.conv2d_pair(to_main(hs), ht, P[ns + '.conv_0.weight'], P[nt + '.conv_0.weight'], P.get(ns + '.conv_0.bias'),
                                 P.get(nt + '.conv_0.bias'), dead_bias=True)
        to_src(ds)
        with on_src():
            hs = self._spade(ds, segs, ns + '.norm_1', ACT_RELU)
        ht = self._spade(dt, segt, nt + '.norm_1', ACT_RELU)
        ds, dt = ops.conv2d_pair(to_main(hs), ht, P[ns + '.conv_1.weight'], P[nt + '.conv_1.weight'], P.get(ns + '.conv_1.bias'),
                                 P.get(nt + '.conv_1.bias'))
        to_src(ds)
        with on_src():
            sx = ops.add(sx, ds)
        return sx, ops.add(tx, dt)

    def _resnet_pair(self, sx, tx, segs, segt, i, sy):
        c = self.cfg
        ns, nt = 'src_model.resnets.%d' % i, 'tsf_model.resnets.%d' % i
        spade = c.spade_layers[1] if i < c.repeat_num // 2 else c.spade_layers[2]
        wkey = '.conv_0.weight' if spade else '.main.0.weight'
        if not ops.pair_ok(sx, tx, self.P[ns + wkey], self.P[nt + wkey]):
            return None
        if spade:
            return self._spade_resblock_pair(sx, tx, segs, segt, ns, nt, sy)
        return self._resblock_pair(sx, tx, ns, nt, sy)

    def _spade_block(self, x, seg, name, down, fork=False):
        if fork:
            h, x = self._conv_fork(x, name + '.conv', stride=2)
            return self._spade(h, seg, name + '.norm', ACT_RELU), x
        h = self._conv(x, name + '.conv', stride=2, to_norm=True) if down else self._convT(x, name + '.conv')
        return self._spade(h, seg, name + '.norm', ACT_RELU)

    def _bg_net_steps(self, x, out):
        c, p = self.cfg, 'bg_model.model'
        x = self._in(self._conv(x, p + '.0', pad=3, to_norm=True), p + '.1', act=ACT_RELU)
        yield
        idx = 3
        for _ in range(c.n_down):
            x = self._in(self._conv(x, p + '.%d' % idx, stride=2, to_norm=True), p + '.%d' % (idx + 1), act=ACT_RELU)
            idx += 3
            yield
        for _ in range(c.repeat_num):
            x = self._resblock(x, p + '.%d' % idx)
            idx += 1
            yield
        for _ in range(c.n_down):
            x = self._in(self._convT(x, p + '.%d' % idx), p + '.%d' % (idx + 1), act=ACT_RELU)
            idx += 3
            yield
        out[0] = self._conv(x, p + '.%d' % idx, pad=3, act=ACT_TANH)

    def _bg_net(self, x):
        out = [None]
        for _ in self._bg_net_steps(x, out):
            pass
        return out[0]

    def _enc_level(self, x, seg, p, i):
        if self.cfg.spade_layers[0]:
            return self._spade_block(x, seg, p + '.encoders.%d' % i, True, fork=True)
        return self._conv_in_relu(x, p + '.encoders.%d' % i, stride=2, fork=True)

    def _resnet(self, x, seg, p, i):
        c = self.cfg
        if (c.spade_layers[1] if i < c.repeat_num // 2 else c.spade_layers[2]):
            return self._spade_resblock(x, seg, p + '.resnets.%d' % i)
        return self._resblock(x, p + '.resnets.%d' % i)

    def _decode_level(self, x, enc, seg, p, i):
        nd = self.cfg.n_down
        name = p + '.skippers.%d' % i
        if self.cfg.spade_layers[3]:
            x = self._spade_block(x, seg, p + '.decoders.%d' % i, False)
        elif not torch.is_grad_enabled() and self.P.get(name + '.0.bias') is None:
            dn = p + '.decoders.%d' % i
            xr = self._convT(x, dn + '.0')
            y = ops.conv2d_after_norm(xr, self.P[dn + '.1.weight'], self.P[dn + '.1.bias'], self.P[name + '.0.weight'], None,
                                      first=enc[nd - 1 - i], norm_next=True)
            if y is not None:
                return self._in(y, name + '.1', act=ACT_RELU)
            x = self._in(xr, dn + '.1', act=ACT_RELU)
        else:
            x = self._conv_in_relu(x, p + '.decoders.%d' % i, transposed=True)
        if self.P.get(name + '.0.bias') is None:
            return self._in(ops.conv2d_cat2(enc[nd - 1 - i], x, self.P[name + '.0.weight'], norm_next=True), name + '.1', act=ACT_RELU)
        return self._conv_in_relu(ops.cat_channels([enc[nd - 1 - i], x]), name)

    def _decode(self, x, enc, seg, p):
        for i in range(self.cfg.n_down):
            x = self._decode_level(x, enc, seg, p, i)
        return x

    def _unet_steps(self, x, seg, p, out):
        e = self._conv_in_relu(x, p + '.encoders.0', pad=3)
        yield
        enc = [e]
        for i in range(1, self.cfg.n_down + 1):
            e, enc[-1] = self._enc_level(e, seg, p, i)
            enc.append(e)
            yield
        for i in range(self.cfg.repeat_num):
            e = self._resnet(e, seg, p, i)
            yield
        for i in range(self.cfg.n_down):
            e = self._decode_level(e, enc, seg, p, i)
            if i + 1 < self.cfg.n_down:
                yield
        out[0] = e

    def _unet(self, x, seg, p):
        out = [None]
        for _ in self._unet_steps(x, seg, p, out):
            pass
        return out[0]

    def _tscale(self, T, h):
        key = ('T', id(T), h)
        if key not in self._seg_cache:
            self._seg_cache[key] = ops.resize_bilinear_ac(T, h, h)
        return self._seg_cache[key]

    def _attn_source(self, x, layer):
        if layer not in self.cfg.attn_layers:
            return None, x
        return ops.attn_source_conv(x, self.P['attn_%d.fully_connect_layer.0.weight#s' % layer], fork=True)

    def _transform(self, x, T, layer, y=None, gs=None):
        h = x.shape[1]
        ts = self._tscale(T, h)
        if layer in self.cfg.attn_layers:
            key = ('F', id(T), h)
            if key not in self._seg_cache:
                self._seg_cache[key] = ops.attn_flow(ts)
            p = 'attn_%d.fully_connect_layer' % layer
            return ops.local_attention(x, y, self._seg_cache[key], self.P[p + '.0.weight#t'], self.P[p + '.0.weight#s'],
                                       self.P[p + '.0.bias'], self.P[p + '.2.weight'], self.P[p + '.2.bias'], gs=gs, fork=True)
        return ops.grid_sample(x, ts), x, y

    def forward(self, bg_inputs, src_obj_inputs, tsf_obj_inputs, src_hand_inputs, tsf_hand_inputs, T,
                src_obj_conds=None, src_hand_conds=None, tsf_obj_conds=None, tsf_hand_conds=None,
                src_armask=None, tsf_armask=None):
        if src_obj_conds is None or src_hand_conds is None or tsf_obj_conds is None or tsf_hand_conds is None:
            raise NotImplementedError('Generator.forward without conds (use_spade=False) is unreachable in the reference: '
                                      'Trainer.forward passes arguments in an order that mismatches obj_dim/img_dim '
                                      '(trainer.py:395-398 vs :263-264)')
        outs = self.forward_nhwc(to_nhwc(bg_inputs), to_nhwc(src_obj_inputs), to_nhwc(tsf_obj_inputs),
                                 to_nhwc(src_hand_inputs), to_nhwc(tsf_hand_inputs), T.contiguous(),
                                 to_nhwc(src_obj_conds), to_nhwc(src_hand_conds), to_nhwc(tsf_obj_conds),
                                 to_nhwc(tsf_hand_conds), to_nhwc(src_armask), to_nhwc(tsf_armask))
        return tuple(as_nchw(o) for o in outs)

    @staticmethod
    def stack_inputs(bg, src_obj, tsf_obj, src_hand_c, tsf_hand_c, src_obj_c, tsf_obj_c, src_armask=None, tsf_armask=None):
        src_bg_in = [bg, src_hand_c] + ([src_armask] if src_armask is not None else [])
        tsf_bg_in = [bg, tsf_hand_c] + ([tsf_armask] if tsf_armask is not None else [])
        return (torch.cat([ops.cat_channels(src_bg_in), ops.cat_channels(tsf_bg_in)], dim=0),
                torch.cat([src_obj, tsf_obj], dim=0), torch.cat([src_obj_c, tsf_obj_c], dim=0))

    def forward_nhwc(self, bg, src_obj, tsf_obj, src_hand, tsf_hand, T, src_obj_c, src_hand_c, tsf_obj_c, tsf_hand_c,
                     src_armask=None, tsf_armask=None, stacked=None):
        c = self.cfg
        self._seg_cache = {}
        ops.attn_index_clear()
        nb = bg.shape[0]
        main = torch.cuda.current_stream()
        fork = _FORK_STREAMS and bg.is_cuda
        self.refresh_planes()
        if stacked is None:
            stacked = self.stack_inputs(bg, src_obj, tsf_obj, src_hand_c, tsf_hand_c, src_obj_c, tsf_obj_c, src_armask, tsf_armask)
        bg_in, obj_in, obj_c = stacked
        if fork:
            s_bg, s_obj, s_src = self._branch_streams(bg.device)
            s_bg.wait_stream(main)
            s_obj.wait_stream(main)
            s_src.wait_stream(main)
            for st_, role in ((s_bg, 'g_bg'), (s_obj, 'g_obj'), (s_src, 'g_src')):
                with torch.cuda.stream(st_):
                    ops.test_delay(role)
            bg_out, obj_out = [None], [None]
            branches = [(self._bg_net_steps(bg_in, bg_out), s_bg), (self._unet_steps(obj_in, obj_c, 'obj_model', obj_out), s_obj)]
            for t_, st_ in ((bg_in, s_bg), (obj_in, s_obj), (obj_c, s_obj)):
                ops.cross_stream(t_, st_)
        else:
            branches = []
            bg_both = self._bg_net(bg_in)

        def advance(all_the_way=False):
            for gen, st_ in branches:
                with torch.cuda.stream(st_):
                    if all_the_way:
                        for _ in gen:
                            pass
                    else:
                        next(gen, None)

        import contextlib
        fork_src = fork
        on_src = (lambda: torch.cuda.stream(s_src)) if fork_src else contextlib.nullcontext

        def src_ready(t_):
            if fork_src:
                main.wait_stream(s_src)
                ops.cross_stream(t_, main)
            return t_

        with on_src():
            sx = self._conv_in_relu(src_hand, 'src_model.encoders.0', pad=3)
        tx = self._conv_in_relu(tsf_hand, 'tsf_model.encoders.0', pad=3)
        advance()
        s_enc, t_enc = [sx], [tx]
        for i in range(1, c.n_down + 1):
            with on_src():
                sx, s_enc[-1] = self._enc_level(sx, src_hand_c, 'src_model', i)
                gs, sx = self._attn_source(sx, i)
            tx, t_enc[-1] = self._enc_level(tx, tsf_hand_c, 'tsf_model', i)
            warped, sx, tx = self._transform(src_ready(sx), T, i, y=tx, gs=None if gs is None else src_ready(gs))
            tx = ops.add(tx, warped)
            s_enc.append(sx)
            t_enc.append(tx)
            advance()
        def to_src(t_):
            if fork_src:
                s_src.wait_stream(main)
                ops.cross_stream(t_, s_src)
            return t_

        for i in range(c.repeat_num):
            pair = self._resnet_pair(sx, tx, src_hand_c, tsf_hand_c, i, (on_src, src_ready, to_src))
            if pair is not None:
                sx, tx = pair
                with on_src():
                    gs, sx = self._attn_source(sx, i + c.n_down + 1)
            else:
                with on_src():
                    sx = self._resnet(sx, src_hand_c, 'src_model', i)
                    gs, sx = self._attn_source(sx, i + c.n_down + 1)
                tx = self._resnet(tx, tsf_hand_c, 'tsf_model', i)
            warped, sx, tx = self._transform(src_ready(sx), T, i + c.n_down + 1, y=tx, gs=None if gs is None else src_ready(gs))
            tx = ops.add(tx, warped)
            advance()
        advance(True)
        if fork:
            with torch.cuda.stream(s_bg):
                bg_both = ops.delay_backward(bg_out[0], 'g_bg')
            with torch.cuda.stream(s_obj):
                obj_both = ops.delay_backward(obj_out[0], 'g_obj')

        if not fork:
            obj_both = self._unet(obj_in, obj_c, 'obj_model')
        fused_y = self.F.get('obj_model.heads_y.weight') if obj_both.is_cuda else None
        if fused_y is not None:
            with (torch.cuda.stream(s_obj) if fork else contextlib.nullcontext()):
                obj_o, my_src, my_tsf = ops.conv_heads(obj_both, fused_y, (3, 1, 1), (ACT_TANH, ACT_NONE, ACT_NONE))
        if fork:
            main.wait_stream(s_bg)
            main.wait_stream(s_obj)
            ops.cross_stream(bg_both, main)
            ops.cross_stream(obj_both, main)
            if fused_y is not None:
                ops.cross_stream(obj_o, main)
                ops.cross_stream(my_tsf, main)
                ops.cross_stream(my_src, s_src)
        src_img_bg, tsf_img_bg = bg_both[:nb], bg_both[nb:]
        sy, ty = obj_both[:nb], obj_both[nb:]
        if fork_src:
            s_src.wait_stream(s_obj)
            ops.cross_stream(obj_both, s_src)
        with on_src():
            sx = self._decode(sx, s_enc, src_hand_c, 'src_model')
        tx = self._decode(tx, t_enc, tsf_hand_c, 'tsf_model')

        if fused_y is not None:
            my = {'src_model': my_src[:nb], 'tsf_model': my_tsf[nb:]}

        def regress(x, y, p):
            fused = self.F.get(p + '.heads_x.weight')
            if fused is not None and x.is_cuda:
                img, mh, mbt = ops.conv_heads(x, fused, (3, 1, 1), (ACT_TANH, ACT_SIGMOID, ACT_NONE))
            else:
                img = self._conv(x, p + '.img_reg.0', pad=3, act=ACT_TANH)
                mh = self._conv(x, p + '.attetion_reg_hand.0', pad=3, act=ACT_SIGMOID)
                mbt = ops.conv2d(x, self.P[p + '.attetion_reg_bg.0.weight#t'], None, 1, 3)
            mby = my[p] if fused_y is not None else ops.conv2d(y, self.P[p + '.attetion_reg_bg.0.weight#s'], None, 1, 3)
            mb = ops.add_act(mbt, mby, ACT_SIGMOID)
            return img, mh, mb

        with on_src():
            src_hand_o, src_mask_hand, src_mask_bg = regress(sx, sy, 'src_model')
            src_hand_o = ops.delay_backward(src_hand_o, 'g_src')
        tsf_hand_o, tsf_mask_hand, tsf_mask_bg = regress(tx, ty, 'tsf_model')
        if fork_src:
            main.wait_stream(s_src)
            for t_ in (src_hand_o, src_mask_hand, src_mask_bg):
                ops.cross_stream(t_, main)
        if fused_y is None:
            obj_o = self._conv(obj_both, 'obj_model.img_reg.0', pad=3, act=ACT_TANH)
        src_obj_o, tsf_obj_o = obj_o[:nb], obj_o[nb:]
        self._seg_cache = {}
        return (src_img_bg, tsf_img_bg, src_obj_o, src_hand_o, src_mask_bg, src_mask_hand,
                tsf_obj_o, tsf_hand_o, tsf_mask_bg, tsf_mask_hand)
```

hoig_amd/ops.py:

```python
import collections
import contextlib
import ctypes
import os

import torch
from torch.autograd import Function

from . import _lib as L
from ._lib import ConvDesc

_PREC = {'f32': L.PREC_F32, 'bf16x3': L.PREC_BF16X3, 'f16x3': L.PREC_BF16X3, 'f16x2': L.PREC_F16X2, 'bf16x2': L.PREC_F16X2,
         'bf16': L.PREC_BF16, 'f16': L.PREC_BF16, 'f16f6': L.PREC_F16F6}
precision = precision_dgrad = precision_wgrad = L.PREC_F32


def set_precision(name):
    global precision, precision_dgrad, precision_wgrad
    parts = name.split(':')
    if len(parts) > 3:
        raise ValueError('precision %r' % name)
    precision = _PREC[parts[0]]
    if precision == L.PREC_F16F6 and len(parts) == 1:
        parts = [parts[0], 'f16x2']
    if L.PREC_F16F6 in [_PREC[q] for q in parts[1:]]:
# ... 199 lines not shown
    _stream_banks[s.device]['free'][q].insert(0, s.cuda_stream)


def stream_census():
    idle = sum(len(f) for b in _stream_banks.values() for f in b['free'])
    return _streams_made - _streams_destroyed, idle, sum(t.numel() for t in _scratch.values())


def destroy_idle_streams():
    global _streams_destroyed
    for dev, bank in _stream_banks.items():
        torch.cuda.synchronize(dev)
        for f in bank['free']:
            while f:
                h = f.pop()
                _scratch.pop((dev, h), None)
                L.call('hoig_stream_destroy', h)
                _streams_destroyed += 1


_scratch = {}


def _ensure_scratch(nbytes):
    cur = torch.cuda.current_stream()
    key = (cur.device, cur.cuda_stream)
    if nbytes > 0 and key not in _scratch:
        t = torch.empty(L.lib.hoig_stream_scratch_bytes(), dtype=torch.uint8, device=cur.device)
        _scratch[key] = t
        L.call('hoig_stream_scratch_set', cur.cuda_stream, t.data_ptr(), t.numel())


def wgrad_call(name, d, *args):
    _ensure_scratch(L.lib.hoig_conv2d_bwd_weight_scratch_bytes(ctypes.byref(d)))
    L.call(name, ctypes.byref(d), *args)


_TEST_DELAYS = {}
_test_fired = set()


def test_step_begins():
    _test_fired.clear()


def test_delay(role, where='fwd'):
    cycles = _TEST_DELAYS.get(role)
    if not cycles or (role, where) in _test_fired:
        return
    _test_fired.add((role, where))
    torch.cuda._sleep(int(cycles))


class _DelayBackward(Function):
    @staticmethod
    def forward(ctx, x, role):
        ctx.role = role
        return x.view_as(x)

    @staticmethod
    def backward(ctx, g):
        test_delay(ctx.role, 'bwd')
        return g, None


def delay_backward(x, role):
    if _TEST_DELAYS.get(role) and torch.is_tensor(x) and x.requires_grad:
        return _DelayBackward.apply(x, role)
    return x


_wgrad_streams = {}
_WGRAD_MODE = os.environ.get('HOIG_WGRAD_STREAM', 'auto')
_WGRAD_SIDE = _WGRAD_MODE != '0'
_wgrad_side_paused = False


def pause_wgrad_side(paused):
    global _wgrad_side_paused
    _wgrad_side_paused = bool(paused) and _WGRAD_MODE == 'auto'


def _wgrad_side_stream(device):
    if not _WGRAD_SIDE or _wgrad_side_paused:
        return None
    s = _wgrad_streams.get(device)
    if s is None:
        s = _wgrad_streams[device] = new_stream(device, 'wgrad')
    if _capture_depth:
        _capture_forked.add(s)
    return s


_wgrad_pending = collections.deque()

_capture_depth = 0
_capture_hold = []


_capture_forked = set()


_has_gpu = None


def capturing():
    global _has_gpu
    if _capture_depth > 0:
        return True
    if _has_gpu is None:
        _has_gpu = torch.cuda.is_available()
    return _has_gpu and torch.cuda.is_current_stream_capturing()


def begin_capture():
    global _capture_depth
    _capture_depth += 1


def end_capture():
    global _capture_depth
    _capture_depth -= 1
    if _capture_depth == 0:
        _capture_hold.clear()
        _capture_forked.clear()
        _wgrad_pending.clear()


class graph_capture(object):

    def __init__(self, graph, pool=None):
        self._ctx = torch.cuda.graph(graph, pool=pool, capture_error_mode='thread_local')

    def __enter__(self):
        begin_capture()
        try:
            return self._ctx.__enter__()
        except BaseException:
            end_capture()
            raise

    def __exit__(self, *exc):
        try:
            if exc[0] is None:
                join_wgrad_streams()
            return self._ctx.__exit__(*exc)
        finally:
            end_capture()


def cross_stream(t, stream):
    if t is None:
        return t
    if capturing():
        _capture_hold.append(t)
    else:
        t.record_stream(stream)
    return t


def _wgrad_hold(side, tensors):
    if capturing():
        _capture_hold.append(tensors)
        return
    for t in tensors:
        t.record_stream(side)
    ev = torch.cuda.Event()
    ev.record(side)
    _wgrad_pending.append((ev, tensors))
    while _wgrad_pending and _wgrad_pending[0][0].query():
        _wgrad_pending.popleft()


def wgrad_side_streams():
    return list(_wgrad_streams.values())


def join_wgrad_streams():
    if capturing():
        for s in list(_capture_forked):
            torch.cuda.current_stream(s.device).wait_stream(s)
        _capture_forked.clear()
        return
    for s in _wgrad_streams.values():
        torch.cuda.current_stream(s.device).wait_stream(s)
    _wgrad_pending.clear()


class _SplitToken(object):
    __slots__ = ('readers', 'offered', '__weakref__')

    def __init__(self):
        self.readers, self.offered = 0, None


_split_live = set()


def _split_backward_ok(d, w, live_bias, transposed):
    if not L.lib.hoig_set_tuning(b'split_grads', -1) or transposed or live_bias or d.act != L.ACT_NONE:
        return False
    if not getattr(w, '_hoig_flat', False) or (d.R, d.S, d.stride, d.pad) != (3, 3, 1, 1) or (d.Ho, d.Wo) != (d.Hi, d.Wi):
        return False
    if d.Co % 128 or d.Ci % 32 or d.Wo % 32 or d.Ho % 8:
        return False
    dg, wg = _bwd_descs(d)
    return dg.precision in (L.PREC_F16X2, L.PREC_BF16) and wg.precision in (L.PREC_F16X2, L.PREC_BF16)


def _tag_split(y, slot=0):
    tok = _SplitToken()
    toks = getattr(y.grad_fn, 'split_toks', None)
    if toks is None:
        toks = y.grad_fn.split_toks = {}
    toks[slot] = tok
    y._hoig_split_grad = tok
    return y


def _claim_split(x):
    tok = getattr(x, '_hoig_split_grad', None)
    if tok is not None:
        tok.readers += 1
    return tok


def _writes_split(tok):
    return tok is not None and tok.readers == 1


def _offer_split(tok, dx):
    tok.offered = dx
    _split_live.add(tok)


def _take_split(ctx, dy, slot=0):
    tok = getattr(ctx, 'split_toks', {}).get(slot)
    if tok is None or tok.offered is None:
        return False
    off, tok.offered = tok.offered, None
    _split_live.discard(tok)
    if dy is not off and (dy.data_ptr() != off.data_ptr() or dy.shape != off.shape):
        raise RuntimeError('a norm wrote this convolution\'s incoming gradient as bf16 hi | lo planes, but the gradient that arrived is '
                           'another tensor: the tagged output had a second consumer (autograd summed plane bits with an fp32 gradient) '
                           'or a hook replaced it.  Give the second consumer its own copy, or set the tuning key split_grads=0.')
    return True


def check_split_grads_consumed():
    if _split_live:
        n = len(_split_live)
        for tok in list(_split_live):
            tok.offered = None
        _split_live.clear()
        raise RuntimeError('%d pre-split gradient tensor(s) were not consumed by a convolution backward' % n)


def _unsplit(dys):
    out = torch.empty_like(dys)
    L.call('hoig_unsplit_planes_bf16', _p(dys), _p(out), dys.numel() // dys.shape[-1], dys.shape[-1], _st())
    return out


def _wgrad_launch(device, on_caller, held, launch, d, *args):
    side = None if on_caller else _wgrad_side_stream(device)
    if side is not None:
        side.wait_stream(torch.cuda.current_stream())
    with torch.cuda.stream(side) if side is not None else contextlib.nullcontext():
        if side is not None:
            test_delay('wgrad')
        made = launch(d, *args) if callable(launch) else wgrad_call(launch, d, *args, _st())
    made = tuple(made or ())
    if side is not None:
        _wgrad_hold(side, tuple(held) + made)
    return side is not None, made


def _wgrad_from_split(d, x, dys, dw):
    if L.attempt('hoig_conv2d_bwd_weight_split', ctypes.byref(d), _p(x), _p(dys), _p(dw), _st()):
        return ()
    plain = _unsplit(dys)
    wgrad_call('hoig_conv2d_bwd_weight', d, _p(x), _p(plain), _p(dw), None, _st())
    return (plain,)


def _wgrad_pair_from_split(d, xs, dys, dws):
    if None not in dws and L.attempt('hoig_conv2d_bwd_weight_split_pair', ctypes.byref(d), _p(xs[0]), _p(xs[1]), _p(dys[0]), _p(dys[1]),
                                     _p(dws[0]), _p(dws[1]), _st()):
        return ()
    made = ()
    for x, sp, dw in zip(xs, dys, dws):
        if dw is not None:
            made += _wgrad_from_split(d, x, sp, dw)
    return made


def _dgrad_from_split(d, dys, w, planes, add, dx, unsplit=None):
    if not L.attempt('hoig_conv2d_bwd_data_packed_split', ctypes.byref(d), _p(dys), _p(planes[0]), _p(planes[1]), _p(add), _p(dx), _st()):
        _conv_dgrad_raw(d, unsplit if unsplit is not None else _unsplit(dys), w, dx, False, addend=add)


class _Conv(Function):
    @staticmethod
    def forward(ctx, x, w, b, stride, pad, transposed, act, slope, out_hw, prec, dead_bias=False, fork=False):
        _chk(x, 'x'); _chk(w, 'w'); _chk(b, 'bias')
        assert x.is_contiguous() and x.dim() == 4
        B, Hi, Wi, Ci = x.shape
        if transposed:
            ci_w, Co, R, S = w.shape
        else:
            Co, ci_w, R, S = w.shape
        assert ci_w == Ci, 'channel mismatch %d vs %d' % (ci_w, Ci)
        assert tuple(w.stride()) == packed_strides(w.shape, transposed), 'conv weight is not in packed layout'
        if out_hw is None:
            if transposed:
                raise ValueError('out_hw required for transposed conv')
            out_hw = ((Hi + 2 * pad - R) // stride + 1, (Wi + 2 * pad - S) // stride + 1)
        Ho, Wo = out_hw
        y = torch.empty((B, Ho, Wo, Co), dtype=x.dtype, device=x.device)
        d = ConvDesc(B, Hi, Wi, Ci, Ho, Wo, Co, R, S, stride, pad, 1 if transposed else 0, act, slope, prec)
        _conv_fwd_raw(d, x, w, b, y, transposed, norm_next=dead_bias)
        ctx.d = d
        ctx.d_dg, ctx.d_wg = _bwd_descs(d)
        ctx.transposed = transposed
        ctx.has_bias = b is not None and not dead_bias
        ctx.save_for_backward(x, w, b, y if act != L.ACT_NONE else None)
        ctx.fork = fork
        ctx.split_ok = dead_bias and _split_backward_ok(d, w, ctx.has_bias, transposed)
        if fork:
            ctx.set_materialize_grads(False)
            return y, x
        return y

    @staticmethod
    def backward(ctx, dy, dxr=None):
        _grad_epoch()
        x, w, b, y = ctx.saved_tensors
        d = ctx.d
        if dy is None:
            return (dxr,) + (None,) * 11
        dy = dy.contiguous()
        if _take_split(ctx, dy):
            return _Conv._backward_split(ctx, dy, dxr, x, w)
        dw_ret = db_ret = None
        db, ret_b = None, False
        if ctx.has_bias and ctx.needs_input_grad[2]:
            db, ret_b = _grad_target(b)
            db_ret = db if ret_b else None
        if d.act != L.ACT_NONE:
            g = torch.empty_like(dy)
            if db is not None:
                L.call('hoig_act_bwd_colsum', _p(y), _p(dy), _p(g), _p(db), d.act, d.slope, dy.numel() // d.Co, d.Co, _st())
                db = None
            else:
                L.call('hoig_act_bwd', _p(y), _p(dy), _p(g), d.act, d.slope, dy.numel(), _st())
        else:
            g = dy
        if ctx.needs_input_grad[1]:
            dw, ret_w = _grad_target(w)
            _wgrad_launch(x.device, ret_w or (db is not None and ret_b), (x, g),
                          'hoig_conv2d_bwd_weight', ctx.d_wg, _p(x), _p(g), _p(dw), _p(db))
            dw_ret = dw if ret_w else None
        elif db is not None:
            L.call('hoig_colsum_accum', _p(g), _p(db), g.numel() // d.Co, d.Co, _st())
        dx = None
        if ctx.needs_input_grad[0]:
            dx = torch.empty_like(x)
            _conv_dgrad_raw(ctx.d_dg, g, w, dx, ctx.transposed, addend=dxr.contiguous() if dxr is not None else None)
        return dx, dw_ret, db_ret, None, None, None, None, None, None, None, None, None

    @staticmethod
    def _backward_split(ctx, dys, dxr, x, w):
        unsplit = None
        if ctx.needs_input_grad[1]:
            dw, ret_w = _grad_target(w)
            on_side, made = _wgrad_launch(x.device, ret_w, (x, dys), _wgrad_from_split, ctx.d_wg, x, dys, dw)
            if made and not on_side:
                unsplit = made[0]
        dx = None
        if ctx.needs_input_grad[0]:
            dx = torch.empty_like(x)
            add = dxr.contiguous() if dxr is not None else None
            _dgrad_from_split(ctx.d_dg, dys, w, _packed_planes(w, False, True), add, dx, unsplit)
        return (dx, (dw if (ctx.needs_input_grad[1] and ret_w) else None)) + (None,) * 10


def conv2d(x, w, b=None, stride=1, pad=0, act=L.ACT_NONE, slope=0.0, prec=None, dead_bias=False):
    y = _Conv.apply(x, w, b, stride, pad, False, act, slope, None, precision if prec is None else prec, dead_bias)
    return _tag_split(y) if getattr(y.grad_fn, 'split_ok', False) else y


def conv2d_fork(x, w, b=None, stride=1, pad=0, act=L.ACT_NONE, slope=0.0, prec=None, dead_bias=False):
    if not x.requires_grad:
        return conv2d(x, w, b, stride, pad, act, slope, prec, dead_bias), x
    y, xr = _Conv.apply(x, w, b, stride, pad, False, act, slope, None, precision if prec is None else prec, dead_bias, True)
    return (_tag_split(y) if getattr(y.grad_fn, 'split_ok', False) else y), xr


def pair_ok(xa, xb, wa, wb, prec=None):
    prec = precision if prec is None else prec
    mode = L.lib.hoig_set_tuning(b'pair', -1)
    if not mode or (mode == 2 and not capturing()) or prec in (L.PREC_F32, L.PREC_F16F6) or not xa.is_cuda:
        return False
    if xa.shape != xb.shape or wa.shape != wb.shape or tuple(wa.shape[2:]) != (3, 3) or wa.shape[1] != xa.shape[-1]:
        return False
    if not (getattr(wa, '_hoig_flat', False) and getattr(wb, '_hoig_flat', False)):
        return False
    B, H, W_, Ci = xa.shape
    Co = wa.shape[0]
    if W_ % 32 or H % 8 or Ci % 32 or Co % 128 or 2 * B * (H // 8) * (W_ // 32) * (Co // 128) < 96:
        return False
    return precision_dgrad in (L.PREC_F16X2, L.PREC_BF16) and precision_wgrad in (L.PREC_F16X2, L.PREC_BF16) and prec == precision


class _ConvPair(Function):

    @staticmethod
    def forward(ctx, xa, xb, wa, wb, ba, bb, prec, dead_bias, fork):
        for t in (xa, xb, wa, wb, ba, bb):
            _chk(t)
        assert xa.is_contiguous() and xb.is_contiguous()
        B, H, W_, Ci = xa.shape
        Co = wa.shape[0]
        d = ConvDesc(B, H, W_, Ci, H, W_, Co, 3, 3, 1, 1, 0, L.ACT_NONE, 0.0, prec)
        ya, yb = torch.empty((B, H, W_, Co), dtype=xa.dtype, device=xa.device), torch.empty((B, H, W_, Co), dtype=xa.dtype, device=xa.device)
        live = ba is not None and not dead_bias
        (ha, la), (hb, lb) = _packed_planes(wa, False, False), _packed_planes(wb, False, False)
        if not L.attempt('hoig_conv2d_fwd_packed_pair', ctypes.byref(d), _p(xa), _p(xb), _p(ha), _p(la), _p(hb), _p(lb),
                         _p(ba) if live else None, _p(bb) if live else None, _p(ya), _p(yb), _st()):
            _conv_fwd_raw(d, xa, wa, ba if live else None, ya)
            _conv_fwd_raw(d, xb, wb, bb if live else None, yb)
        ctx.d_dg, ctx.d_wg = _bwd_descs(d)
        ctx.live_bias = live
        ctx.save_for_backward(xa, xb, wa, wb, ba if live else None, bb if live else None)
        ctx.split_ok = dead_bias and _split_backward_ok(d, wa, live, False)
        ctx.fork = fork
        if fork:
            ctx.set_materialize_grads(False)
            return ya, yb, xa, xb
        return ya, yb

    @staticmethod
    def backward(ctx, dya, dyb, dxra=None, dxrb=None):
        _grad_epoch()
        xa, xb, wa, wb, ba, bb = ctx.saved_tensors
        if dya is None or dyb is None:
            raise RuntimeError('conv2d_pair: both outputs must be used (a grouped launch has no half)')
        d_dg, d_wg = ctx.d_dg, ctx.d_wg
        B, H, W_, Co = dya.shape
        npix = B * H * W_
        dys, db_ret = [], [None, None]
        for i, (dy, b) in enumerate(((dya, ba), (dyb, bb))):
            dy = dy.contiguous()
            if _take_split(ctx, dy, i):
                dys.append(dy)
                continue
            if ctx.live_bias and ctx.needs_input_grad[4 + i]:
                db, ret_b = _grad_target(b)
                L.call('hoig_colsum_accum', _p(dy), _p(db), npix, Co, _st())
                db_ret[i] = db if ret_b else None
            sp = torch.empty_like(dy)
            L.call('hoig_split_planes_bf16', _p(dy), _p(sp), npix, Co, _st())
            dys.append(sp)
        need = (bool(ctx.needs_input_grad[2]), bool(ctx.needs_input_grad[3]))
        dwa, ret_a = _grad_target(wa) if need[0] else (None, False)
        dwb, ret_b = _grad_target(wb) if need[1] else (None, False)
        if need[0] or need[1]:
            _wgrad_launch(xa.device, ret_a or ret_b, (xa, xb, dys[0], dys[1]), _wgrad_pair_from_split, d_wg, (xa, xb), dys, (dwa, dwb))
        dxa = dxb = None
        if ctx.needs_input_grad[0] or ctx.needs_input_grad[1]:
            dxa, dxb = torch.empty_like(xa), torch.empty_like(xb)
            adds = [None if t is None else t.contiguous() for t in (dxra, dxrb)]
            if (adds[0] is None) != (adds[1] is None):
                adds = [t if t is not None else torch.zeros_like(xa) for t in adds]
            pa, pb = _packed_planes(wa, False, True), _packed_planes(wb, False, True)
            if not L.attempt('hoig_conv2d_bwd_data_packed_split_pair', ctypes.byref(d_dg), _p(dys[0]), _p(dys[1]), _p(pa[0]), _p(pa[1]),
                             _p(pb[0]), _p(pb[1]), _p(adds[0]), _p(adds[1]), _p(dxa), _p(dxb), _st()):
                _dgrad_from_split(d_dg, dys[0], wa, pa, adds[0], dxa)
                _dgrad_from_split(d_dg, dys[1], wb, pb, adds[1], dxb)
        return dxa, dxb, (dwa if (need[0] and ret_a) else None), (dwb if (need[1] and ret_b) else None), db_ret[0], db_ret[1], None, None, None


def conv2d_pair(xa, xb, wa, wb, ba=None, bb=None, prec=None, dead_bias=False, fork=False):
    out = _ConvPair.apply(xa, xb, wa, wb, ba, bb, precision if prec is None else prec, dead_bias, fork)
    if getattr(out[0].grad_fn, 'split_ok', False):
        _tag_split(out[0], 0)
        _tag_split(out[1], 1)
    return out


class _ConvCat2(Function):

    @staticmethod
    def forward(ctx, x1, x2, w, prec, norm_next=False):
        B, H, W_, C1 = x1.shape
        C2 = x2.shape[-1]
        Co = w.shape[0]
        assert tuple(w.stride()) == packed_strides(w.shape, False), 'conv weight is not in packed layout'
        d = ConvDesc(B, H, W_, C1 + C2, H, W_, Co, 3, 3, 1, 1, 0, L.ACT_NONE, 0.0, prec)
        y = torch.empty((B, H, W_, Co), dtype=x1.dtype, device=x1.device)
        hi, lo = _packed_planes(w, False, False)
        ws = _conv_stats_workspace(y) if norm_next else None
        done = False
        if prec == L.PREC_F16F6 and (C1 + C2) % 64 == 0 and Co % 64 == 0 and H % 8 == 0:
            qh, ql = _f6_planes(w)
            done = L.attempt('hoig_conv2d_fwd_f6_ex', ctypes.byref(d), _p(x1), C1, _p(x2), _p(hi), _p(qh), _p(ql), None, None, None, 0,
                             _p(y), _p(ws), _st())
        d = _x3(d)
        if not done and ws is not None:
            done = L.attempt('hoig_conv2d_cat_fwd_packed_stats', ctypes.byref(d), _p(x1), C1, _p(x2), _p(hi), _p(lo), None, _p(y), _p(ws), _st())
        if not done:
            L.call('hoig_conv2d_cat_fwd_packed', ctypes.byref(d), _p(x1), C1, _p(x2), _p(hi), _p(lo), None, _p(y), _st())
        elif ws is not None:
            _stats_offer(y)
        ctx.d_dg, ctx.d_wg = _bwd_descs(d)
        ctx.save_for_backward(x1, x2, w)
        return y

    @staticmethod
    def backward(ctx, dy):
        _grad_epoch()
        x1, x2, w = ctx.saved_tensors
        C1 = x1.shape[-1]
        dy = dy.contiguous()
        dw, ret_w = _grad_target(w)
        _wgrad_launch(dy.device, ret_w, (x1, x2, dy), 'hoig_conv2d_cat_bwd_weight', ctx.d_wg, _p(x1), C1, _p(x2), _p(dy), _p(dw), None)
        dx1, dx2 = torch.empty_like(x1), torch.empty_like(x2)
        hi, lo = _packed_planes(w, False, True)
        L.call('hoig_conv2d_cat_bwd_data_packed', ctypes.byref(ctx.d_dg), _p(dy), _p(hi), _p(lo), _p(dx1), C1, _p(dx2), _st())
        return dx1, dx2, (dw if ret_w else None), None, None


def conv2d_cat2(x1, x2, w, prec=None, norm_next=False):
    prec = precision if prec is None else prec
    B, H, W_, C1 = x1.shape
    C2 = x2.shape[-1]
    Co = w.shape[0]
    ok = (prec != L.PREC_F32 and x1.is_cuda and tuple(w.shape[2:]) == (3, 3) and w.shape[1] == C1 + C2 and
          C1 % 64 == 0 and C2 % 64 == 0 and Co % 64 == 0 and W_ % 32 == 0 and H % 4 == 0 and
          B * (H // 4) * (W_ // 32) * ((Co + 127) // 128) >= 160 and B * (H // 4) * (W_ // 32) * ((C1 + C2 + 127) // 128) >= 160 and
          x1.shape[:3] == x2.shape[:3] and x1.is_contiguous() and x2.is_contiguous())
    if not ok:
        return conv2d(cat_channels([x1, x2]), w, None, 1, 1, prec=prec, dead_bias=norm_next)
    return _ConvCat2.apply(x1, x2, w, prec, norm_next)


def conv2d_after_norm(xraw, gamma, beta, w, b=None, first=None, norm_next=False, eps=1e-5):
    assert not torch.is_grad_enabled(), 'conv2d_after_norm has no backward'
    _chk(xraw, 'x'); _chk(w, 'w')
    B, H, W_, C = xraw.shape
    HW = H * W_
    C1 = first.shape[-1] if first is not None else 0
    Co = w.shape[0]
    if (precision == L.PREC_F32 or tuple(w.shape[2:]) != (3, 3) or w.shape[1] != C1 + C or C % 32 or C1 % 32 or Co % 64
            or W_ % 32 or H % 8 or not xraw.is_contiguous() or (first is not None and (not first.is_contiguous() or first.shape[:3] != xraw.shape[:3]))
            or not L.lib.hoig_set_tuning(b'norm_in', -1)):
        _stats_drop(xraw)
        return None
    dev = xraw.device
    mean = torch.empty(B * C, dtype=torch.float32, device=dev)
    rstd = torch.empty_like(mean)
    ws, have = _norm_workspace(L.lib.hoig_inorm_workspace_bytes(B, HW, C) // 4, dev, take=(xraw.data_ptr(), B, HW, C))
    if have:
        L.call('hoig_inorm_stats_from_sums', _p(xraw), B, HW, C, eps, _p(mean), _p(rstd), _p(ws), _st())
    else:
        L.call('hoig_inorm_stats', _p(xraw), B, HW, C, eps, _p(mean), _p(rstd), _p(ws), _st())
    Cg = C1 + C
    fold = torch.empty(2, B, Cg, dtype=torch.float32, device=dev)
    if C1:
        fold[0, :, :C1] = 1.0
        fold[1, :, :C1] = 0.0
    L.call('hoig_inorm_fold', _p(mean), _p(rstd), _p(gamma), _p(beta), B, C, fold.data_ptr() + 4 * C1, fold.data_ptr() + 4 * (B * Cg + C1), Cg,
           _st())
    y = torch.empty((B, H, W_, Co), dtype=xraw.dtype, device=dev)
    d = ConvDesc(B, H, W_, Cg, H, W_, Co, 3, 3, 1, 1, 0, L.ACT_NONE, 0.0, precision)
    hi, lo = _packed_planes(w, False, False)
    sws = _conv_stats_workspace(y) if norm_next else None
    a, a2 = (first, xraw) if first is not None else (xraw, None)
    done = False
    if precision == L.PREC_F16F6 and Cg % 64 == 0:
        qh, ql = _f6_planes(w)
        done = L.attempt('hoig_conv2d_fwd_f6_ex', ctypes.byref(d), _p(a), C1, _p(a2), _p(hi), _p(qh), _p(ql), _p(b), fold.data_ptr(),
                         fold.data_ptr() + 4 * B * Cg, C1, _p(y), _p(sws), _st())
    if not done:
        d = _x3(d)
        if not L.attempt('hoig_conv2d_fwd_packed_normin', ctypes.byref(d), _p(a), C1, _p(a2), _p(hi), _p(lo), _p(b), fold.data_ptr(),
                         fold.data_ptr() + 4 * B * Cg, C1, _p(y), _p(sws), _st()):
            return None
    if sws is not None:
        _stats_offer(y)
    return y


class _ConvHeads(Function):

    @staticmethod
    def forward(ctx, x, w, splits, acts, prec):
        _chk(x, 'x'); _chk(w, 'w')
        assert x.is_contiguous() and tuple(w.stride()) == packed_strides(w.shape, False)
        B, H, W_, Ci = x.shape
        Co, _, R, S = w.shape
        assert sum(splits) == Co and len(splits) == len(acts)
        assert Co <= 16, 'the activation codes of the fused heads are 4 bits x 16 channels (hoig_conv2d_fwd_heads)'
        if Co > 16:
            raise ValueError('conv_heads: %d output channels, the per-channel activation codes hold 16' % Co)
        d = _x3(ConvDesc(B, H, W_, Ci, H, W_, Co, R, S, 1, R // 2, 0, L.ACT_NONE, 0.0, prec))
        codes, ch = 0, 0
        for n, a in zip(splits, acts):
            for _ in range(n):
                codes |= (a & 15) << (4 * ch)
                ch += 1
        y = torch.empty((B, H, W_, Co), dtype=x.dtype, device=x.device)
        L.call('hoig_conv2d_fwd_heads', ctypes.byref(d), _p(x), _p(w), None, _p(y), codes, _st())
        outs, off = [], 0
        for n in splits:
            o = torch.empty((B, H, W_, n), dtype=x.dtype, device=x.device)
            _copy_channels(y, o, off, 0, n)
            outs.append(o)
            off += n
        ctx.d_dg, ctx.d_wg = _bwd_descs(d)
        ctx.cfg = (tuple(splits), tuple(acts))
        ctx.save_for_backward(x, w, *[o if a != L.ACT_NONE else None for o, a in zip(outs, acts)])
        return tuple(outs)

    @staticmethod
    def backward(ctx, *douts):
        _grad_epoch()
        x, w = ctx.saved_tensors[:2]
        ys = ctx.saved_tensors[2:]
        splits, acts = ctx.cfg
        B, H, W_, _ = x.shape
        Co = w.shape[0]
        g = torch.empty((B, H, W_, Co), dtype=x.dtype, device=x.device)
        off = 0
        for n, a, yv, dy in zip(splits, acts, ys, douts):
            if dy is None:
                dy = torch.zeros((B, H, W_, n), dtype=x.dtype, device=x.device)
            dy = dy.contiguous()
            if a != L.ACT_NONE:
                t = torch.empty_like(dy)
                L.call('hoig_act_bwd', _p(yv), _p(dy), _p(t), a, 0.0, dy.numel(), _st())
                dy = t
            _copy_channels(dy, g, 0, off, n)
            off += n
        dw_ret = None
        if ctx.needs_input_grad[1]:
            dw, ret_w = _grad_target(w)
            wgrad_call('hoig_conv2d_bwd_weight', ctx.d_wg, _p(x), _p(g), _p(dw), None, _st())
            dw_ret = dw if ret_w else None
        dx = None
        if ctx.needs_input_grad[0]:
            dx = torch.empty_like(x)
            _conv_dgrad_raw(ctx.d_dg, g, w, dx)
        return dx, dw_ret, None, None, None


def conv_heads(x, w, splits, acts, prec=None):
    return _ConvHeads.apply(x, w, tuple(splits), tuple(acts), precision if prec is None else prec)


def conv_transpose2d(x, w, stride=2, pad=1, output_padding=1, prec=None, norm_next=False):
    B, Hi, Wi, _ = x.shape
    R, S = w.shape[2], w.shape[3]
    out_hw = ((Hi - 1) * stride - 2 * pad + R + output_padding, (Wi - 1) * stride - 2 * pad + S + output_padding)
    return _Conv.apply(x, w, None, stride, pad, True, L.ACT_NONE, 0.0, out_hw, precision if prec is None else prec, norm_next)


def set_f6_min_tiles(n):
    return L.lib.hoig_set_f6_min_tiles(int(n))


def _f6_planes(w):
    co, ci, r, s = w.shape
    owner = getattr(w, '_hoig_owner', None)
    if owner is not None and hasattr(owner, 'packed_f6'):
        planes = owner.packed_f6(w)
        if planes is not None:
            return planes
    return _cached_planes(
        'f6', (w.data_ptr(), tuple(w.shape)), w,
        lambda: tuple(torch.empty(L.lib.hoig_f6_plane_bytes(co, r * s, ci), dtype=torch.uint8, device=w.device) for _ in range(2)),
        lambda qh, ql: L.call('hoig_pack_conv_weight_f6', _p(w), co, r * s, ci, _p(qh), _p(ql), _st()))


def _wino_planes(w):
    co, ci = w.shape[0], w.shape[1]
    return _cached_planes(
        'wino', (w.data_ptr(), tuple(w.shape)), w,
        lambda: tuple(torch.empty(L.lib.hoig_wino_plane_halfs(co, ci), dtype=torch.int16, device=w.device) for _ in range(2)),
        lambda uh, ul: L.call('hoig_pack_conv_weight_wino', _p(w), co, ci, _p(uh), _p(ul), _st()))


def _x3(d):
    if d.precision != L.PREC_F16F6:
        return d
    c = ConvDesc.from_buffer_copy(d)
    c.precision = L.PREC_BF16X3
    return c


def packed_planes(ci, co):
    if ci % 32 or co % 32:
        return 0
    return (1 if co > 32 else 0) | (2 if ci > 32 else 0)


def _conv_fwd_raw(d, x, w, b, y, transposed=False, norm_next=False):
    if _conv_fwd_ladder(d, x, w, b, y, transposed, norm_next):
        _stats_offer(y)


def _conv_fwd_ladder(d, x, w, b, y, transposed, norm_next):
    ws = None
    packed = d.precision != L.PREC_F32 and packed_planes(d.Ci, d.Co) & 1
    if norm_next and packed:
        ws = _conv_stats_workspace(y)
    elif norm_next and d.precision != L.PREC_F32 and not transposed and d.Ci <= 12 and d.Co % 64 == 0 and d.stride == 1:
        ws0 = _conv_stats_workspace(y)
        if ws0 is not None and L.attempt('hoig_conv2d_fwd_stats', ctypes.byref(_x3(d)), _p(x), _p(w), _p(b), _p(y), _p(ws0), _st()):
            return True
    if d.precision == L.PREC_F16F6:
        if (not transposed and d.R == 3 and d.S == 3 and d.stride == 1 and d.pad == 1 and d.Ci % 64 == 0 and d.Co % 64 == 0
                and d.Hi % 8 == 0 and d.Wi % 32 == 0):
            hi, _ = _packed_planes(w, False, False)
            qh, ql = _f6_planes(w)
            if L.attempt('hoig_conv2d_fwd_f6_ex', ctypes.byref(d), _p(x), 0, None, _p(hi), _p(qh), _p(ql), _p(b), None, None, 0, _p(y),
                         _p(ws), _st()):
                return ws is not None
        d = _x3(d)
    if (ws is None and d.precision == L.PREC_BF16X3 and not transposed and d.R == 3 and d.S == 3 and d.stride == 1 and d.pad == 1
            and d.Ci % 32 == 0 and d.Co % 64 == 0 and d.Hi % 16 == 0 and d.Wi % 16 == 0 and L.lib.hoig_set_tuning(b'wino8', -1) == 1
            and d.B * (d.Hi // 16) * (d.Wi // 16) * (d.Co // 64) <= 256 and d.B * (d.Hi // 8) * ((d.Wi + 31) // 32) * ((d.Co + 127) // 128) <= 128):
        uh, ul = _wino_planes(w)
        if L.attempt('hoig_conv2d_fwd_wino', ctypes.byref(d), _p(x), _p(uh), _p(ul), _p(b), _p(y), _st()):
            return False
    if ws is not None:
        hi, lo = _packed_planes(w, transposed, False)
        if L.attempt('hoig_conv2d_fwd_packed_stats', ctypes.byref(d), _p(x), _p(hi), _p(lo), _p(b), _p(y), _p(ws), _st()):
            return True
    if packed:
        hi, lo = _packed_planes(w, transposed, False)
        if L.attempt('hoig_conv2d_fwd_packed', ctypes.byref(d), _p(x), _p(hi), _p(lo), _p(b), _p(y), _st()):
            return False
    L.call('hoig_conv2d_fwd', ctypes.byref(d), _p(x), _p(w), _p(b), _p(y), _st())
    return False


def _conv_dgrad_raw(d, g, w, dx, transposed=False, addend=None):
    packed = d.precision != L.PREC_F32 and packed_planes(d.Ci, d.Co) & 2
    if packed:
        hi, lo = _packed_planes(w, transposed, True)
        if addend is not None and L.attempt('hoig_conv2d_bwd_data_packed_add', ctypes.byref(d), _p(g), _p(hi), _p(lo), _p(addend), _p(dx), _st()):
            return
    out = dx if addend is None else torch.empty_like(dx)
    if not (packed and L.attempt('hoig_conv2d_bwd_data_packed', ctypes.byref(d), _p(g), _p(hi), _p(lo), _p(out), _st())):
        L.call('hoig_conv2d_bwd_data', ctypes.byref(d), _p(g), _p(w), _p(out), _st())
    if addend is not None:
        L.call('hoig_add', _p(out), _p(addend), _p(dx), dx.numel(), _st())


def _reexport():
    import importlib
    import sys
    g = globals()
    for mod in ('ops_norm', 'ops_small', 'ops_attn', 'ops_loss', 'ops_daug'):
        if __package__ + '.' + mod in sys.modules:
            raise ImportError('import hoig_amd.ops first: it was reached from the import of hoig_amd.%s, whose names it '
                              're-exports and which is not complete yet' % mod)
        m = importlib.import_module('.' + mod, __package__)
        for k, v in vars(m).items():
            if not k.startswith('__') and k not in ('_o', 'L', 'ConvDesc', 'Function', 'torch', 'contextlib'):
                g[k] = v


_reexport()
```

hoig_amd/ops_norm.py:

```python
import contextlib

import torch
from torch.autograd import Function

from . import _lib as L
from .ops import _chk, _claim_split, _grad_epoch, _grad_target, _offer_split, _p, _st, _writes_split

_norm_ws = {}


_stats_pending = {}


def _norm_workspace(nfloats, device, take=None):
    key = (device, torch.cuda.current_stream(device).cuda_stream)
    ws = _norm_ws.get(key)
    pend = _stats_pending.pop(key, None)
    if pend is not None and pend == take:
        return ws, True
    if ws is None or ws.numel() < nfloats:
        ws = torch.zeros(max(nfloats, 1 << 20), dtype=torch.float32, device=device)
        _norm_ws[key] = ws
    elif pend is not None:
        ws[:pend[1] * 4 * pend[3]].zero_()
    return (ws, False) if take is not None else ws


_small_sums = [False]


@contextlib.contextmanager
def small_map_sums():
    prev, _small_sums[0] = _small_sums[0], True
    try:
        yield
    finally:
        _small_sums[0] = prev


def _conv_stats_workspace(y):
    B, H, W_, C = y.shape
    if (H * W_ <= 1024 and not _small_sums[0]) or C % 4 or B * 4 * C > (1 << 18):
        return None
    return _norm_workspace(L.lib.hoig_inorm_workspace_bytes(B, H * W_, C) // 4, y.device)


def _stats_drop(x):
    key = (x.device, torch.cuda.current_stream(x.device).cuda_stream)
    pend = _stats_pending.get(key)
    if pend is not None and pend[0] == x.data_ptr():
        _norm_workspace(1, x.device)


def _stats_offer(y):
    B, H, W_, C = y.shape
    _stats_pending[(y.device, torch.cuda.current_stream(y.device).cuda_stream)] = (y.data_ptr(), B, H * W_, C)


class _INorm(Function):
    @staticmethod
    def forward(ctx, x, p0, p1, mode, act, slope, residual, eps):
        _chk(x, 'x')
        assert x.is_contiguous()
        B, H, W, C = x.shape
        HW = H * W
        if act != L.ACT_NONE and residual is not None:
            raise ValueError('activation + residual in one instance-norm epilogue is not defined')
        mean = torch.empty(B * C, dtype=torch.float32, device=x.device)
        rstd = torch.empty_like(mean)
        y = torch.empty_like(x)
        if HW > 1024 or not L.attempt('hoig_inorm_fwd_fused', _p(x), mode, _p(p0), _p(p1), C, act, slope, _p(residual), eps, _p(y), _p(mean),
                                      _p(rstd), B, HW, C, _st()):
            ws, have = _norm_workspace(L.lib.hoig_inorm_workspace_bytes(B, HW, C) // 4, x.device, take=(x.data_ptr(), B, HW, C))
            if have:
                L.call('hoig_inorm_stats_from_sums', _p(x), B, HW, C, eps, _p(mean), _p(rstd), _p(ws), _st())
            else:
                L.call('hoig_inorm_stats', _p(x), B, HW, C, eps, _p(mean), _p(rstd), _p(ws), _st())
            L.call('hoig_inorm_apply', _p(x), _p(mean), _p(rstd), mode, _p(p0), _p(p1), act, slope, _p(residual), _p(y),
                   B, HW, C, _st())
        ctx.cfg = (mode, act, slope, B, HW, C, residual is not None)
        ctx.split_tok = _claim_split(x)
        y_free = act in (L.ACT_RELU, L.ACT_LRELU) and mode in (0, 1)
        ctx.save_for_backward(x, mean, rstd, p0, p1, y if (act != L.ACT_NONE and not y_free) else None)
        return y

    @staticmethod
    def backward(ctx, dy):
        _grad_epoch()
        x, mean, rstd, p0, p1, y = ctx.saved_tensors
        mode, act, slope, B, HW, C, has_res = ctx.cfg
        dy = dy.contiguous()
        dx = torch.empty_like(x)
        dp0 = dp1 = r0 = r1 = None
        if mode == 1:
            dp0, ret0 = _grad_target(p0)
            dp1, ret1 = _grad_target(p1)
            r0, r1 = (dp0 if ret0 else None), (dp1 if ret1 else None)
        elif mode == 2:
            dp0, dp1 = torch.empty_like(x), torch.empty_like(x)
            r0, r1 = dp0, dp1
        split_dx = _writes_split(ctx.split_tok)
        sfx = '_split' if split_dx else ''
        p1m = _p(p1) if mode == 1 else None
        if not L.attempt('hoig_inorm_bwd_fused_add' + sfx, _p(x), _p(mean), _p(rstd), mode, _p(p0), p1m, C, _p(y), _p(dy), act, slope, None, _p(dx),
                         _p(dp0), _p(dp1), B, HW, C, _st()):
            ws = _norm_workspace(L.lib.hoig_inorm_workspace_bytes(B, HW, C) // 4, x.device)
            L.call('hoig_inorm_bwd_add_ld' + sfx, _p(x), _p(mean), _p(rstd), mode, _p(p0), p1m, C, _p(y), _p(dy), act, slope, None, _p(dx),
                   _p(dp0), _p(dp1), B, HW, C, _p(ws), _st())
        if split_dx:
            _offer_split(ctx.split_tok, dx)
        return dx, r0, r1, None, None, None, (dy if has_res else None), None


def instance_norm(x, weight=None, bias=None, act=L.ACT_NONE, slope=0.0, residual=None, eps=1e-5):
    mode = 1 if weight is not None else 0
    return _INorm.apply(x, weight, bias, mode, act, slope, residual, eps)


def spade_norm(x, gamma, beta, act=L.ACT_NONE, slope=0.0, eps=1e-5):
    return _INorm.apply(x, gamma, beta, 2, act, slope, None, eps)


class _SpadeFused(Function):

    @staticmethod
    def forward(ctx, x, gb, act, slope, eps, fork=False):
        _chk(x); _chk(gb)
        assert x.is_contiguous() and gb.is_contiguous()
        B, H, W, C = x.shape
        assert gb.shape[-1] == 2 * C
        HW = H * W
        mean = torch.empty(B * C, dtype=torch.float32, device=x.device)
        rstd = torch.empty_like(mean)
        y = torch.empty_like(x)
        if HW > 1024 or not L.attempt('hoig_inorm_fwd_fused', _p(x), 2, _p(gb), gb.data_ptr() + 4 * C, 2 * C, act, slope, None, eps, _p(y),
                                      _p(mean), _p(rstd), B, HW, C, _st()):
            ws, have = _norm_workspace(L.lib.hoig_inorm_workspace_bytes(B, HW, C) // 4, x.device, take=(x.data_ptr(), B, HW, C))
            if have:
                L.call('hoig_inorm_stats_from_sums', _p(x), B, HW, C, eps, _p(mean), _p(rstd), _p(ws), _st())
            else:
                L.call('hoig_inorm_stats', _p(x), B, HW, C, eps, _p(mean), _p(rstd), _p(ws), _st())
            L.call('hoig_inorm_apply_ld', _p(x), _p(mean), _p(rstd), 2, _p(gb), gb.data_ptr() + 4 * C, 2 * C, act, slope, None,
                   _p(y), B, HW, C, _st())
        ctx.cfg = (act, slope, B, HW, C)
        ctx.split_tok = _claim_split(x)
        ctx.save_for_backward(x, mean, rstd, gb, y if act != L.ACT_NONE else None)
        if fork:
            ctx.set_materialize_grads(False)
            return y, x
        return y

    @staticmethod
    def backward(ctx, dy, dxr=None):
        x, mean, rstd, gb, y = ctx.saved_tensors
        act, slope, B, HW, C = ctx.cfg
        if dy is None:
            return dxr, None, None, None, None, None
        dy = dy.contiguous()
        add = dxr.contiguous() if dxr is not None else None
        dx = torch.empty_like(x)
        dgb = torch.empty_like(gb)
        split_dx = _writes_split(ctx.split_tok)
        sfx = '_split' if split_dx else ''
        if not L.attempt('hoig_inorm_bwd_fused_add' + sfx, _p(x), _p(mean), _p(rstd), 2, _p(gb), None, 2 * C, _p(y), _p(dy), act, slope, _p(add),
                         _p(dx), _p(dgb), dgb.data_ptr() + 4 * C, B, HW, C, _st()):
            ws = _norm_workspace(L.lib.hoig_inorm_workspace_bytes(B, HW, C) // 4, x.device)
            L.call('hoig_inorm_bwd_add_ld' + sfx, _p(x), _p(mean), _p(rstd), 2, _p(gb), None, 2 * C, _p(y), _p(dy), act, slope, _p(add),
                   _p(dx), _p(dgb), dgb.data_ptr() + 4 * C, B, HW, C, _p(ws), _st())
        if split_dx:
            _offer_split(ctx.split_tok, dx)
        return dx, dgb, None, None, None, None


def spade_norm_fused(x, gb, act=L.ACT_NONE, slope=0.0, eps=1e-5, fork=False):
    if fork and not x.requires_grad:
        return _SpadeFused.apply(x, gb, act, slope, eps), x
    return _SpadeFused.apply(x, gb, act, slope, eps, fork)
```

include/hoig_kernels.h:

```cpp
#ifndef HOIG_KERNELS_H
#define HOIG_KERNELS_H

#include <stddef.h>
#include <stdint.h>

#ifdef __cplusplus
extern "C" {
#endif

typedef void *hoig_stream_t;

enum { HOIG_OK = 0, HOIG_EINVAL = -1, HOIG_ELAUNCH = -2, HOIG_EUNSUPPORTED = -3 };

enum { HOIG_ACT_NONE = 0, HOIG_ACT_RELU = 1, HOIG_ACT_LRELU = 2, HOIG_ACT_TANH = 3, HOIG_ACT_SIGMOID = 4 };

enum { HOIG_PREC_F32 = 0, HOIG_PREC_BF16X3 = 1, HOIG_PREC_BF16 = 2, HOIG_PREC_F16X2 = 3, HOIG_PREC_F16F6 = 4 };

typedef struct hoig_conv_desc {
    int32_t B, Hi, Wi, Ci;
    int32_t Ho, Wo, Co;
    int32_t R, S;
    int32_t stride, pad;
    int32_t transposed;
    int32_t act;
    float slope;
    int32_t precision;
} hoig_conv_desc;

int hoig_conv2d_fwd(const hoig_conv_desc *d, const float *x, const float *w, const float *bias ,
                    float *y, hoig_stream_t stream);
int hoig_conv2d_bwd_data(const hoig_conv_desc *d, const float *dy, const float *w, float *dx, hoig_stream_t stream);
int hoig_conv2d_bwd_weight(const hoig_conv_desc *d, const float *x, const float *dy, float *dw, float *dbias,
                           hoig_stream_t stream);

int hoig_split_planes_bf16(const float *x, uint16_t *out, int64_t npix, int C, hoig_stream_t stream);
int hoig_unsplit_planes_bf16(const uint16_t *in, float *out, int64_t npix, int C, hoig_stream_t stream);
int hoig_inorm_bwd_add_ld_split(const float *x, const float *mean, const float *rstd, int mode, const float *p0, const float *p1,
                                int ld_p, const float *y, const float *dy, int act, float slope, const float *addend ,
                                uint16_t *dx_split, float *dp0, float *dp1, int B, int HW, int C, void *workspace,
                                hoig_stream_t stream);
int hoig_inorm_bwd_fused_add_split(const float *x, const float *mean, const float *rstd, int mode, const float *p0, const float *p1,
                                   int ld_p, const float *y, const float *dy, int act, float slope, const float *addend ,
                                   uint16_t *dx_split, float *dp0, float *dp1, int B, int HW, int C, hoig_stream_t stream);
int64_t hoig_wino_plane_halfs(int Co, int Ci);
int hoig_pack_conv_weight_wino(const float *w , int Co, int Ci, uint16_t *u_hi, uint16_t *u_lo, hoig_stream_t stream);
int hoig_conv2d_fwd_wino(const hoig_conv_desc *d, const float *x, const uint16_t *u_hi, const uint16_t *u_lo, const float *bias ,
                         float *y, hoig_stream_t stream);
int hoig_inorm_fold(const float *mean, const float *rstd, const float *gamma , const float *beta , int B, int C,
                    float *scale, float *shift, int ld_out, hoig_stream_t stream);
int hoig_conv2d_fwd_packed_normin(const hoig_conv_desc *d, const float *x, int C1, const float *x2 , const uint16_t *w_hi,
                                  const uint16_t *w_lo, const float *bias , const float *in_scale, const float *in_shift,
                                  int in_relu_c0, float *y, double *stats , hoig_stream_t stream);
int hoig_conv2d_bwd_weight_split(const hoig_conv_desc *d, const float *x, const uint16_t *dy_split, float *dw, hoig_stream_t stream);
int hoig_conv2d_bwd_data_packed_split(const hoig_conv_desc *d, const uint16_t *dy_split, const uint16_t *wt_hi, const uint16_t *wt_lo,
                                      const float *addend , float *dx, hoig_stream_t stream);

int hoig_conv2d_fwd_packed_pair(const hoig_conv_desc *d, const float *xa, const float *xb, const uint16_t *wa_hi, const uint16_t *wa_lo,
                                const uint16_t *wb_hi, const uint16_t *wb_lo, const float *bias_a ,
                                const float *bias_b , float *ya, float *yb, hoig_stream_t stream);
int hoig_conv2d_bwd_data_packed_split_pair(const hoig_conv_desc *d, const uint16_t *dys_a, const uint16_t *dys_b, const uint16_t *wta_hi,
                                           const uint16_t *wta_lo, const uint16_t *wtb_hi, const uint16_t *wtb_lo,
                                           const float *addend_a , const float *addend_b , float *dxa, float *dxb,
                                           hoig_stream_t stream);
int hoig_conv2d_bwd_weight_split_pair(const hoig_conv_desc *d, const float *xa, const float *xb, const uint16_t *dys_a,
                                      const uint16_t *dys_b, float *dwa, float *dwb, hoig_stream_t stream);

int hoig_conv2d_fwd_heads(const hoig_conv_desc *d, const float *x, const float *w, const float *bias , float *y,
                          uint64_t acts, hoig_stream_t stream);

int hoig_pack_conv_weight_bf16(const float *w, int Co, int RS, int Ci, int for_dgrad, uint16_t *hi, uint16_t *lo ,
                               hoig_stream_t stream);
int hoig_pack_conv_weights_bf16_all(const float *flat, const int64_t *segs, int nseg, int64_t ntiles, uint16_t *hi_f,
                                    uint16_t *lo_f, uint16_t *hi_d, uint16_t *lo_d, hoig_stream_t stream);
int hoig_conv2d_fwd_packed(const hoig_conv_desc *d, const float *x, const uint16_t *w_hi, const uint16_t *w_lo,
                           const float *bias , float *y, hoig_stream_t stream);
int hoig_conv2d_bwd_data_packed(const hoig_conv_desc *d, const float *dy, const uint16_t *wt_hi, const uint16_t *wt_lo,
                                float *dx, hoig_stream_t stream);
int hoig_conv2d_fwd_packed_stats(const hoig_conv_desc *d, const float *x, const uint16_t *w_hi, const uint16_t *w_lo,
                                 const float *bias , float *y, double *stats, hoig_stream_t stream);
int hoig_conv2d_cat_fwd_packed_stats(const hoig_conv_desc *d, const float *x1, int C1, const float *x2, const uint16_t *w_hi,
                                     const uint16_t *w_lo, const float *bias , float *y, double *stats,
                                     hoig_stream_t stream);
int hoig_conv2d_fwd_stats(const hoig_conv_desc *d, const float *x, const float *w, const float *bias , float *y, double *stats,
                          hoig_stream_t stream);
int hoig_conv2d_bwd_data_packed_add(const hoig_conv_desc *d, const float *dy, const uint16_t *wt_hi, const uint16_t *wt_lo,
                                    const float *addend, float *dx, hoig_stream_t stream);

int64_t hoig_f6_plane_bytes(int Co, int RS, int Ci);
int hoig_pack_conv_weight_f6(const float *w, int Co, int RS, int Ci, uint8_t *q_hi, uint8_t *q_lo, hoig_stream_t stream);
int hoig_conv2d_fwd_f6(const hoig_conv_desc *d, const float *x, const uint16_t *w_hi, const uint8_t *q_hi, const uint8_t *q_lo,
                       const float *bias , float *y, hoig_stream_t stream);
int hoig_conv2d_fwd_f6_ex(const hoig_conv_desc *d, const float *x, int C1, const float *x2 , const uint16_t *w_hi,
                          const uint8_t *q_hi, const uint8_t *q_lo, const float *bias , const float *in_scale ,
                          const float *in_shift , int in_relu_c0, float *y, double *stats , hoig_stream_t stream);
int hoig_pack_conv_weights_f6_all(const float *flat, const int64_t *rows, int nrows, int64_t ntasks, uint8_t *q_hi, uint8_t *q_lo,
                                  hoig_stream_t stream);
int hoig_set_f6_min_tiles(int n);

int hoig_conv2d_cat_fwd_packed(const hoig_conv_desc *d, const float *x1, int C1, const float *x2, const uint16_t *w_hi,
                               const uint16_t *w_lo, const float *bias , float *y, hoig_stream_t stream);
int hoig_conv2d_cat_bwd_data_packed(const hoig_conv_desc *d, const float *dy, const uint16_t *wt_hi, const uint16_t *wt_lo,
                                    float *dx1, int C1, float *dx2, hoig_stream_t stream);
int hoig_conv2d_cat_bwd_weight(const hoig_conv_desc *d, const float *x1, int C1, const float *x2, const float *dy, float *dw,
                               float *dbias , hoig_stream_t stream);

int64_t hoig_inorm_workspace_bytes(int B, int HW, int C);
int hoig_inorm_stats(const float *x, int B, int HW, int C, float eps, float *mean, float *rstd, void *workspace,
                     hoig_stream_t stream);
int hoig_inorm_apply(const float *x, const float *mean, const float *rstd, int mode, const float *p0, const float *p1,
                     int act, float slope, const float *residual , float *y, int B, int HW, int C,
                     hoig_stream_t stream);
int hoig_inorm_stats_from_sums(const float *y, int B, int HW, int C, float eps, float *mean, float *rstd, void *workspace,
                               hoig_stream_t stream);
int hoig_inorm_apply_ld(const float *x, const float *mean, const float *rstd, int mode, const float *p0, const float *p1,
                        int ld_p, int act, float slope, const float *residual , float *y, int B, int HW, int C,
                        hoig_stream_t stream);
int hoig_inorm_bwd_ld(const float *x, const float *mean, const float *rstd, int mode, const float *p0, const float *p1,
                      int ld_p, const float *y, const float *dy, int act, float slope, float *dx, float *dp0, float *dp1, int B,
                      int HW, int C, void *workspace, hoig_stream_t stream);
int hoig_inorm_fwd_fused(const float *x, int mode, const float *p0, const float *p1, int ld_p, int act, float slope,
                         const float *residual , float eps, float *y, float *mean, float *rstd, int B, int HW,
                         int C, hoig_stream_t stream);
int hoig_inorm_bwd_fused(const float *x, const float *mean, const float *rstd, int mode, const float *p0, const float *p1,
                         int ld_p, const float *y , const float *dy, int act, float slope,
                         float *dx, float *dp0, float *dp1, int B, int HW, int C, hoig_stream_t stream);
int hoig_inorm_bwd_add_ld(const float *x, const float *mean, const float *rstd, int mode, const float *p0, const float *p1,
                          int ld_p, const float *y, const float *dy, int act, float slope, const float *addend, float *dx,
                          float *dp0, float *dp1, int B, int HW, int C, void *workspace, hoig_stream_t stream);
int hoig_inorm_bwd_fused_add(const float *x, const float *mean, const float *rstd, int mode, const float *p0, const float *p1,
                             int ld_p, const float *y, const float *dy, int act, float slope, const float *addend, float *dx,
                             float *dp0, float *dp1, int B, int HW, int C, hoig_stream_t stream);

int hoig_inorm_bwd(const float *x, const float *mean, const float *rstd, int mode, const float *p0, const float *p1,
                   const float *y, const float *dy, int act, float slope, float *dx, float *dp0, float *dp1, int B, int HW,
                   int C, void *workspace, hoig_stream_t stream);

int hoig_replicate_pad_fwd(const float *x, float *y, int B, int H, int W, int C, int pad, hoig_stream_t stream);
int hoig_replicate_pad_bwd(const float *dy, float *dx, int B, int H, int W, int C, int pad, hoig_stream_t stream);
int hoig_replicate_pad_bwd_add(const float *dy, const float *addend, float *dx, int B, int H, int W, int C, int pad,
                               hoig_stream_t stream);
int hoig_attn_pixel_fwd(const float *gt, const float *gs, const float *flow, const float *w2, const float *b2,
                        const float *source, float *hidden, float *attn, float *out, float *kf , int B, int H,
                        int W, int C, hoig_stream_t stream);
int hoig_attn_pixel_bwd(const float *hidden, const float *attn, const float *w2, const float *source, const float *flow,
                        const float *dout, float *dhidden, float *dw2, float *db2, float *e_ws, int B, int H, int W, int C,
                        hoig_stream_t stream);
int64_t hoig_attn_index_ints(int B, int H, int W);
int hoig_attn_build_index(const float *flow, int32_t *index, int B, int H, int W, hoig_stream_t stream);
int hoig_attn_src_gather(const int32_t *index, const float *kf, const float *dout, const float *init, float *dsource, int B,
                         int H, int W, int C, hoig_stream_t stream);
int hoig_attn_gs_gather(const int32_t *index, const float *flow, const float *dhidden, float *dgs, int B, int H, int W,
                        hoig_stream_t stream);

int hoig_block_extractor_forward(const float *source, const float *flow, float *output, int B, int C, int Hs, int Ws,
                                 int Hf, int Wf, int kernel_size, hoig_stream_t stream);
int hoig_block_extractor_backward(const float *source, const float *flow, const float *grad_output, float *grad_source,
                                  float *grad_flow, int B, int C, int Hs, int Ws, int Hf, int Wf, int kernel_size,
                                  hoig_stream_t stream);
int hoig_local_attn_reshape_forward(const float *inputs, float *output, int B, int Hs, int Ws, int kernel_size,
                                    hoig_stream_t stream);
int hoig_local_attn_reshape_backward(const float *grad_output, float *grad_inputs, int B, int Hs, int Ws,
                                     int kernel_size, hoig_stream_t stream);

int hoig_grid_sample_fwd(const float *x, const float *grid, float *y, int B, int H, int W, int C, int Ho, int Wo,
                         hoig_stream_t stream);
int hoig_grid_sample_bwd(const float *grid, const float *dy, float *dx, int B, int H, int W, int C, int Ho, int Wo,
                         hoig_stream_t stream);
int hoig_resize_bilinear_ac(const float *x, float *y, int B, int Hi, int Wi, int C, int Ho, int Wo,
                            hoig_stream_t stream);
int hoig_resize_nearest(const float *x, float *y, int B, int Hi, int Wi, int C, int Ho, int Wo, hoig_stream_t stream);
int hoig_attn_flow(const float *tscale, float *flow, int B, int h, hoig_stream_t stream);

int hoig_maxpool2_fwd(const float *x, float *y, int B, int H, int W, int C, hoig_stream_t stream);
int hoig_maxpool2_bwd(const float *x, const float *y, const float *dy, float *dx, int B, int H, int W, int C,
                      hoig_stream_t stream);

int hoig_nchw_to_nhwc(const float *x, float *y, int B, int C, int H, int W, hoig_stream_t stream);
int hoig_nhwc_to_nchw(const float *x, float *y, int B, int C, int H, int W, hoig_stream_t stream);
int hoig_copy_channels(const float *x, float *y, int64_t npix, int Cx, int x_off, int Cy, int y_off, int Ccopy,
                       int accumulate, hoig_stream_t stream);
int hoig_cat2_channels(const float *x1, int C1, const float *x2, int C2, float *y, int64_t npix, hoig_stream_t stream);
int hoig_add(const float *a, const float *b, float *y, int64_t n, hoig_stream_t stream);
int hoig_add_act(const float *a, const float *b, float *y, int act, float slope, int64_t n, hoig_stream_t stream);
int hoig_act_bwd(const float *y, const float *dy, float *dx, int act, float slope, int64_t n, hoig_stream_t stream);
int hoig_act_bwd_colsum(const float *y, const float *dy, float *g, float *dbias, int act, float slope, int64_t rows, int C,
                        hoig_stream_t stream);
int hoig_colsum_accum(const float *x, float *out, int64_t rows, int C, hoig_stream_t stream);

int hoig_compose_fwd(const float *bg, const float *obj, const float *hand, const float *mbg, const float *mh, float *img,
                     int64_t npix, int C, hoig_stream_t stream);
int hoig_compose_bwd(const float *bg, const float *obj, const float *hand, const float *mbg, const float *mh,
                     const float *dimg, float *dbg, float *dobj, float *dhand, float *dmbg, float *dmh, int64_t npix,
                     int C, hoig_stream_t stream);

enum { HOIG_LOSS_L1 = 0, HOIG_LOSS_MSE = 1, HOIG_LOSS_BCE = 2 };
int hoig_loss_fwd_bwd(int kind, const float *pred, const float *target, float target_const, float gscale, float *out,
                      float *dpred, int64_t n, hoig_stream_t stream);
int hoig_tv_fwd_bwd(const float *m, float gx, float gy, float *out, float *dm, int B, int H, int W, hoig_stream_t stream);
int hoig_loss_accumulate(int kind, const float *pred, const float *target, float target_const, float gscale, float *term,
                         float *dpred, int64_t n, hoig_stream_t stream);
int hoig_tv_accumulate(const float *m, float gx, float gy, float *term, float *dm, int B, int H, int W, hoig_stream_t stream);
int hoig_sum(const float *x, float *out, int64_t n, hoig_stream_t stream);
int hoig_sum_scaled(const float *x, float scale, float *out, int64_t n, hoig_stream_t stream);

int hoig_adam_step(float *param, const float *grad, float *exp_avg, float *exp_avg_sq, int64_t n, double lr,
                   double beta1, double beta2, double eps, int step, float grad_scale, hoig_stream_t stream);

int hoig_adam_tick(double *state, float *derived, hoig_stream_t stream);
int hoig_adam_step_dev(float *param, const float *grad, float *exp_avg, float *exp_avg_sq, int64_t n, const float *derived,
                       float grad_scale, hoig_stream_t stream);
int hoig_adam_pack_step(float *flat, const float *grad, float *exp_avg, float *exp_avg_sq, const float *derived, float grad_scale,
                        const int64_t *segs, int nseg, int64_t ntiles, const int64_t *plain, int64_t nplain, uint16_t *hi_f,
                        uint16_t *lo_f, uint16_t *hi_d, uint16_t *lo_d, hoig_stream_t stream);

int hoig_stream_create(hoig_stream_t *out);
int hoig_stream_destroy(hoig_stream_t stream);
int64_t hoig_stream_scratch_bytes(void);
int64_t hoig_conv2d_bwd_weight_scratch_bytes(const hoig_conv_desc *d);
int hoig_stream_scratch_set(hoig_stream_t stream, void *ptr, int64_t bytes);

int hoig_tensor2im_u8(const float *x, uint8_t *out, int B, int H, int W, int C, int nrow, int unnormalize,
                      hoig_stream_t stream);
int hoig_tensor2im_nhwc_u8(const float *x, uint8_t *out, int64_t n, int unnormalize, hoig_stream_t stream);

int hoig_prep_texture(const float *src_img, const float *src_faces, const int32_t *src_fim, const int32_t *fim_uv,
                      const float *wim_uv, const float *obj_tex_img, unsigned char *occ_ws, float *tex,
                      hoig_stream_t stream);
int hoig_prep_lookup(const int32_t *fim, const float *wim, const float *map_fn, const float *sem_full,
                     const float *faces_uv_coord, int n_faces, const float *tex, const float *src_faces, float *cond,
                     float *seg, float *hand_region, float *rend, float *T, hoig_stream_t stream);
#define HOIG_PREP_MAX_BATCH 32
int hoig_prep_texture_batched(int B, const float *src_img, const float *src_faces, int64_t face_stride, const int32_t *src_fim,
                              const int32_t *const *fim_uv, const float *const *wim_uv, const float *const *obj_tex_img,
                              unsigned char *occ_ws, float *tex, hoig_stream_t stream);
int hoig_prep_lookup_batched(int B, const int32_t *fim, const float *wim, const float *const *map_fn, const float *const *sem_full,
                             const float *const *faces_uv_coord, const int *n_faces, const float *tex, const float *src_faces,
                             int64_t face_stride, float *cond, float *seg, float *hand_region, float *rend, float *T ,
                             hoig_stream_t stream);
int hoig_prep_assemble(int B, const float *src_img, const float *ref_img, const float *cond_s, const float *cond_r,
                       const float *seg_s, const float *seg_r, const float *hr_s, const float *hr_r, const float *rend_s,
                       const float *rend_r, const float *T_raw, float *src_bg, float *tsf_bg, float *src_obj,
                       float *tsf_obj, float *src_hand, float *ref_hand, int hand_channels, float *T_hand, float *smb,
                       float *rmb, float *smh, float *rmh, hoig_stream_t stream);

size_t hoig_rasterize_workspace_bytes(int B, int F);
int hoig_project_faces(const float *cam, int cam_dim, const float *verts, int V, const int64_t *const *face_lists, const int *n_faces,
                       int B, int Fmax, float eye_z, float pad_value, float *faces_out, hoig_stream_t stream);
int hoig_rasterize_fim_wim(const float *faces, int B, int F, int image_size, float near, float far, int32_t *fim,
                           float *wim, void *workspace, hoig_stream_t stream);

int hoig_resize_linear_u8(const uint8_t *src, int B, int Hs, int Ws, int C, uint8_t *dst, int Hd, int Wd, hoig_stream_t stream);
int hoig_warp_affine_u8(const uint8_t *src, int B, int Hs, int Ws, int C, const double *M, int Hd, int Wd, int mode, void *dst,
                        hoig_stream_t stream);

const char *hoig_version(void);

int hoig_set_tuning(const char *key, int value);

int hoig_conv_last_route(int which);
const char *hoig_conv_route_name(int id);

int hoig_mano_lbs(const float *v_template, const float *shapedirs, const float *posedirs, const float *j_template,
                  const float *j_shapedirs, const float *lbs_weights, const int32_t *parents, const float *hands_mean ,
                  const float *hands_components , int ncomps, int V, const float *root, const float *hand,
                  const float *betas, const float *transl , float *verts, int ld_v, float *joints , int B,
                  hoig_stream_t stream);

enum { HOIG_POOL_MAX = 0, HOIG_POOL_AVG = 1 };
int hoig_pool2d_fwd(const float *x, float *y, int B, int H, int W, int C, int k, int stride, int pad_h, int pad_w, int mode,
                    int count_include_pad, hoig_stream_t stream);
int hoig_stage_images_u8(const uint8_t *src, float *y, int B, int Hi, int Wi, int C, int Ho, int Wo, int n_affine, const float *affine,
                         hoig_stream_t stream);
int hoig_pil_bilinear_ksize(int in, int out);
int hoig_pil_bilinear_table(int in, int out, int32_t *table);
int64_t hoig_resize_pil_bilinear_u8_workspace_bytes(int B, int H, int W, int C, int Ho, int Wo);
int hoig_resize_pil_bilinear_u8_host(const uint8_t *src, int B, int H, int W, int C, uint8_t *dst, int Ho, int Wo);
int hoig_resize_pil_bilinear_u8(const uint8_t *src, int B, int H, int W, int C, uint8_t *dst, int Ho, int Wo, const int32_t *table_w,
                                const int32_t *table_h, void *workspace, hoig_stream_t stream);
int hoig_pad2d(const float *x, float *y, int B, int H, int W, int C, int pad_h, int pad_w, hoig_stream_t stream);
int hoig_global_avgpool(const float *x, float *y, int B, int HW, int C, hoig_stream_t stream);
int64_t hoig_lpips_workspace_bytes(int B, int HW);
int hoig_lpips_layer(const float *fx, const float *fy, const float *w, float *out, int B, int HW, int C, void *workspace,
                     hoig_stream_t stream);
int64_t hoig_ssim_workspace_bytes(int B, int H, int W, int C, int win);
int hoig_ssim(const float *x, const float *y, float *ssim_out, float *cs_out, int B, int H, int W, int C, float data_range, float K1,
              float K2, int win, float sigma, void *workspace, hoig_stream_t stream);

enum { HOIG_JPEG_ECODE = 1,
       HOIG_JPEG_EOVERRUN = 2,
       HOIG_JPEG_EMARKER = 4,
       HOIG_JPEG_ETRAILING = 8   };
typedef struct hoig_jpeg_plan {
    int64_t data_off;
    int64_t out_off;
    int64_t coef_off;
    int64_t plane_off;
    int32_t data_len;
    int32_t width, height;
    int32_t ncomp;
    int32_t hs, vs;
    int32_t restart_interval;
    int32_t n_intervals;
    int32_t interval_first;
    int32_t reserved[3];
    uint16_t quant[3][64];
    uint8_t dc_counts[3][16], dc_vals[3][16], ac_counts[3][16], ac_vals[3][256];
} hoig_jpeg_plan;
int64_t hoig_jpeg_decode_workspace_bytes(hoig_jpeg_plan *plans, int n);
int hoig_jpeg_entropy_host(const uint8_t *bytes, int64_t nbytes, const hoig_jpeg_plan *plans, int n, const int32_t *intervals,
                           int64_t n_entries, void *coef, int64_t coef_bytes, int32_t *status);
int hoig_jpeg_decode_bgr_u8(const uint8_t *bytes, int64_t nbytes, const hoig_jpeg_plan *plans_host, const hoig_jpeg_plan *plans_dev,
                            int n, const int32_t *intervals, int64_t n_entries, uint8_t *out, int64_t out_bytes, int32_t *status,
                            void *workspace, int64_t workspace_bytes, hoig_stream_t stream);
int hoig_jpeg_reconstruct_bgr_u8(const hoig_jpeg_plan *plans_host, const hoig_jpeg_plan *plans_dev, int n, uint8_t *out,
                                 int64_t out_bytes, void *workspace, int64_t workspace_bytes, hoig_stream_t stream);

#define HOIG_JPEG_SUBSEQ_BYTES 64
int64_t hoig_jpeg_decode_par_workspace_bytes(hoig_jpeg_plan *plans, int n, int subseq_bytes);
int hoig_jpeg_entropy_par_host(const uint8_t *bytes, int64_t nbytes, const hoig_jpeg_plan *plans, int n, const int32_t *intervals,
                               int64_t n_entries, int subseq_bytes, int lanes, void *coef, int64_t coef_bytes, int32_t *status,
                               int32_t *rounds, int32_t *states, int64_t n_states);
int hoig_jpeg_decode_bgr_u8_par(const uint8_t *bytes, int64_t nbytes, const hoig_jpeg_plan *plans_host, const hoig_jpeg_plan *plans_dev,
                                int n, const int32_t *intervals, int64_t n_entries, uint8_t *out, int64_t out_bytes, int32_t *status,
                                void *workspace, int64_t workspace_bytes, int subseq_bytes, hoig_stream_t stream);

#define HOIG_PNG_SEGMENT_BYTES 8192
int64_t hoig_png_encode_bound(int H, int W, int C, int segment_bytes);
int64_t hoig_png_encode_workspace_bytes(int B, int H, int W, int C, int segment_bytes);
int hoig_png_encode_u8(const uint8_t *src, int B, int H, int W, int C, uint8_t *out, int64_t out_stride, int32_t *sizes, void *workspace,
                       int64_t workspace_bytes, int segment_bytes, hoig_stream_t stream);
int hoig_png_filter_host(const uint8_t *src, int H, int W, int C, uint8_t *filtered);
int hoig_png_deflate_host(const uint8_t *stream, int64_t n, int segment_bytes, int dist_c, int dist_row, uint8_t *out, int64_t out_bytes,
                          int64_t *out_size, int32_t *seg_sizes);
int hoig_png_encode_host(const uint8_t *src, int B, int H, int W, int C, uint8_t *out, int64_t out_stride, int32_t *sizes,
                         int segment_bytes);

enum { HOIG_PNG_ECODE = 1,
       HOIG_PNG_EBTYPE = 2,
       HOIG_PNG_ESTORED = 4,
       HOIG_PNG_EDIST = 8,
       HOIG_PNG_EEARLY = 16,
       HOIG_PNG_EMORE = 32,
       HOIG_PNG_ELESS = 64,
       HOIG_PNG_EFILTER = 128,
       HOIG_PNG_EADLER = 256     };
typedef struct hoig_png_decode_plan {
    int64_t data_off;
    int64_t out_off;
    int64_t pal_off;
    int64_t filt_off;
    int32_t data_len;
    int32_t width, height;
    int32_t color_type;
    int32_t bit_depth;
    int32_t pal_entries;
    int32_t reserved[2];
} hoig_png_decode_plan;
int64_t hoig_png_decode_workspace_bytes(hoig_png_decode_plan *plans, int n);
int hoig_png_inflate_host(const uint8_t *data, int64_t data_len, uint8_t *out, int64_t expect, int32_t *status);
int hoig_png_decode_host(const uint8_t *bytes, int64_t nbytes, const hoig_png_decode_plan *plans, int n, uint8_t *out,
                         int64_t out_bytes, int32_t *status, void *workspace, int64_t workspace_bytes, int bgr);
int hoig_png_decode_u8(const uint8_t *bytes, int64_t nbytes, const hoig_png_decode_plan *plans_host,
                       const hoig_png_decode_plan *plans_dev, int n, uint8_t *out, int64_t out_bytes, int32_t *status, void *workspace,
                       int64_t workspace_bytes, int bgr, hoig_stream_t stream);

enum { HOIG_GEMM_ACCUMULATE = 1,
       HOIG_GEMM_SYMMETRIC = 2,
       HOIG_GEMM_F32 = 4           };
int hoig_gemm_tn_f64(const void *A, int64_t lda, const void *B, int64_t ldb, const double *pivot, double *C, int64_t ldc, int M, int N,
                     int K, int flags, hoig_stream_t stream);
int hoig_gemm_tn_f64_host(const void *A, int64_t lda, const void *B, int64_t ldb, const double *pivot, double *C, int64_t ldc, int M,
                          int N, int K, int flags);
int64_t hoig_pchol_f64_workspace_bytes(int D);
int hoig_pchol_f64(const double *S, int64_t lds, int D, double *L, int64_t ldl, int32_t *piv, int32_t *info, void *workspace,
                   int64_t workspace_bytes, hoig_stream_t stream);
int hoig_pchol_f64_host(const double *S, int64_t lds, int D, double *L, int64_t ldl, int32_t *piv, int32_t *info);
int64_t hoig_sym_eigvals_f64_workspace_bytes(int n);
int hoig_sym_eigvals_f64(const double *A, int64_t lda, int n, double *lambda, int32_t *info, void *workspace, int64_t workspace_bytes,
                         hoig_stream_t stream);
int hoig_sym_eigvals_f64_host(const double *A, int64_t lda, int n, double *lambda, int32_t *info);
int hoig_tridiag_eigvals_f64(const double *d, const double *e, int n, double *lambda, hoig_stream_t stream);
int hoig_tridiag_eigvals_f64_host(const double *d, const double *e, int n, double *lambda);
int hoig_sym_tridiag_f64_host(const double *A, int64_t lda, int n, double *d, double *e);

int64_t hoig_kid_workspace_bytes(int S, int m);
// ... 149 lines not shown
```

Before: 133.3 images/s.

## Fuse SPADE gamma/beta conv with instance-norm apply and fold residual add into conv

Adds a SPADE epilogue variant of the 3x3 halo conv kernel. It interleaves gamma and beta weight blocks so a single tile holds both, then applies the normalization (x-mean)*rstd*(1+gamma)+beta plus the activation directly. It writes the output and gamma, so the full gamma/beta tensor is never materialized and reread by a separate norm kernel. It also adds a forward conv path that takes a residual addend with fused stats, and it has the generator collect the stats sums ahead of time for SPADE. This adds complex routing and a new autograd function, and the epilogue does strided global loads of x.

```diff
diff --git a/hoig_amd/csrc/conv_bf16_common.h b/hoig_amd/csrc/conv_bf16_common.h
--- a/hoig_amd/csrc/conv_bf16_common.h
+++ b/hoig_amd/csrc/conv_bf16_common.h
@@ -100,6 +100,9 @@
     float *C_g2 = nullptr;
     int a_split = 0;
     double *stats = nullptr;
+    const float *sp_x = nullptr, *sp_mean = nullptr, *sp_rstd = nullptr;
+    float *sp_gamma_out = nullptr;
+    int sp_gamma_ld = 0;
 };
 
 struct Geom {
@@ -213,6 +216,7 @@
 int launch_wgrad_dma(const WHaloArgs &a, int ns, dim3 grid, hipStream_t st);
 
 int launch_halo3_m16(HaloArgs a, int ns, int bn, hipStream_t st);
+int launch_halo3_m16_spade(HaloArgs a, hipStream_t st);
 int launch_halo_s2_m16(const HaloArgs &a, int ns, bool scatter, hipStream_t st);
 
 template <int KS>
diff --git a/hoig_amd/csrc/conv_halo16.hip b/hoig_amd/csrc/conv_halo16.hip
--- a/hoig_amd/csrc/conv_halo16.hip
+++ b/hoig_amd/csrc/conv_halo16.hip
@@ -16,8 +16,9 @@
     static constexpr size_t bytes(int nsx) { return (size_t)ns_a(nsx) * PLANE_P + 2 * 3 * ns_b(nsx) * PLANE_W; }
 };
 
-template <int NSX, int WM, int WN, int BN, bool F16, bool ASPLIT = false, bool WDMA = false, bool NORMIN = false>
+template <int NSX, int WM, int WN, int BN, bool F16, bool ASPLIT = false, bool WDMA = false, bool NORMIN = false, bool SPADE_EPI = false>
 __global__ __launch_bounds__(64 * WM * WN) void conv_halo3_m16_kernel(const HaloArgs p) {
+    static_assert(!SPADE_EPI || (F16 && NSX == 2 && BN == 128 && WN == 2 && !ASPLIT && !NORMIN), "SPADE_EPI: the three-term forward on 128-row tiles");
     constexpr int NS = NSX == 1 ? 1 : 2, NB = NSX == 2 ? 2 : 1;
     using LY = M16Layout<WM, BN>;
     constexpr int KS = 3, TH = LY::TH, HW = LY::HW, HPIX = LY::HPIX;
@@ -50,6 +51,8 @@
     const float *const gbias = g2 ? p.bias_g2 : p.bias, *const gadd = g2 ? p.addend_g2 : p.addend;
     float *const gC = g2 ? p.C_g2 : p.C;
 
+    const int sp_c = p.N >> 1;
+    auto wblock = [&](int rb) { return SPADE_EPI ? (rb & 1) * (sp_c >> 5) + (n0 >> 6) + (rb >> 1) : (n0 >> 5) + rb; };
     const int brow = tid >> 2, bpos = tid & 3;
     const unsigned short *wrow_h[RB], *wrow_l[RB];
     int woff[RB];
@@ -57,8 +60,8 @@
     for (int i = 0; i < RB; ++i) {
         const int row = brow + (NT / 4) * i;
         const int n = n0 + row;
-        const bool ok = n < p.N && (!B_PART || row < BN);
-        const size_t o = ((size_t)(n >> 5) * (p.K >> 5)) * 1024 + (n & 31) * 32 + bpos * 8;
+        const bool ok = (SPADE_EPI ? (n0 >> 1) + 32 * (row >> 6) < sp_c : n < p.N) && (!B_PART || row < BN);
+        const size_t o = ((size_t)(SPADE_EPI ? wblock(row >> 5) : n >> 5) * (p.K >> 5)) * 1024 + (n & 31) * 32 + bpos * 8;
         wrow_h[i] = ok ? gWh + o : nullptr;
         wrow_l[i] = (NB == 2 && ok) ? gWl + o : nullptr;
         const int c = bpos ^ ((row >> 2) & 3);
@@ -122,7 +125,7 @@
         const int wtap = p.flip ? (KS * KS - 1 - tap) : tap;
         const size_t koff = (size_t)(wtap * p.Cg + cb * 32) * 32;
         const unsigned short *plane = pl ? gWl : gWh;
-        const unsigned short *src = plane + ((size_t)((n0 >> 5) + blk) * (p.K >> 5)) * 1024 + koff + (h ? dlane1 : dlane0);
+        const unsigned short *src = plane + ((size_t)wblock(blk) * (p.K >> 5)) * 1024 + koff + (h ? dlane1 : dlane0);
         const unsigned to = __builtin_amdgcn_readfirstlane(lds_w0 + buf * BBUF + tp * PLANE_W + h * W23 + blk * 1024);
         unsigned keep;
         asm volatile("s_mov_b32 %0, m0\n\ts_mov_b32 m0, %2\n\ts_nop 0\n\tglobal_load_lds_dwordx4 %1, off\n\ts_mov_b32 m0, %0"
@@ -296,6 +299,47 @@
         bbuf ^= 1;
     }
 
+    if constexpr (SPADE_EPI) {
+        float4 bg[2], bb[2], mu[2], rs[2];
+        int cj[2];
+#pragma unroll
+        for (int j = 0; j < 2; ++j) {
+            const int c = (n0 >> 1) + wn * 32 + j * 16 + lg * 4;
+            cj[j] = c < sp_c ? c : -1;
+            bg[j] = bb[j] = mu[j] = rs[j] = make_float4(0.f, 0.f, 0.f, 0.f);
+            if (cj[j] >= 0) {
+                if (gbias) {
+                    bg[j] = *reinterpret_cast<const float4 *>(gbias + c);
+                    bb[j] = *reinterpret_cast<const float4 *>(gbias + sp_c + c);
+                }
+                mu[j] = *reinterpret_cast<const float4 *>(p.sp_mean + (size_t)bi * sp_c + c);
+                rs[j] = *reinterpret_cast<const float4 *>(p.sp_rstd + (size_t)bi * sp_c + c);
+            }
+        }
+#pragma unroll
+        for (int m = 0; m < MT; ++m) {
+            const int oy = y0 + wm * 2 + (m >> 1), ox = x0 + (m & 1) * 16 + l15;
+            const size_t pix = ((size_t)bi * p.H + oy) * p.W + ox;
+#pragma unroll
+            for (int j = 0; j < 2; ++j) {
+                if (cj[j] < 0) continue;
+                const float4 xv = *reinterpret_cast<const float4 *>(p.sp_x + pix * sp_c + cj[j]);
+                const float xq[4] = {xv.x, xv.y, xv.z, xv.w};
+                const float gq[4] = {bg[j].x, bg[j].y, bg[j].z, bg[j].w}, bq[4] = {bb[j].x, bb[j].y, bb[j].z, bb[j].w};
+                const float mq[4] = {mu[j].x, mu[j].y, mu[j].z, mu[j].w}, rq[4] = {rs[j].x, rs[j].y, rs[j].z, rs[j].w};
+                float ga[4], o[4];
+#pragma unroll
+                for (int q = 0; q < 4; ++q) {
+                    ga[q] = fast_act(acc[j][m][q] * p.oscale + gq[q], 1.f, false, HOIG_ACT_NONE, 0.f);
+                    const float be = fast_act(acc[j + 2][m][q] * p.oscale + bq[q], 1.f, false, HOIG_ACT_NONE, 0.f);
+                    o[q] = hoig_act(fmaf((xq[q] - mq[q]) * rq[q], ga[q] + 1.f, be), p.act, p.slope);
+                }
+                *reinterpret_cast<float4 *>(gC + pix * sp_c + cj[j]) = make_float4(o[0], o[1], o[2], o[3]);
+                *reinterpret_cast<float4 *>(p.sp_gamma_out + pix * p.sp_gamma_ld + cj[j]) = make_float4(ga[0], ga[1], ga[2], ga[3]);
+            }
+        }
+        return;
+    }
     const float nslope = p.act == HOIG_ACT_NONE ? 1.f : (p.act == HOIG_ACT_RELU ? 0.f : p.slope);
     const bool special = p.act == HOIG_ACT_TANH || p.act == HOIG_ACT_SIGMOID;
     float4 bias_r[NTW];
@@ -652,6 +696,24 @@
 
 }
 
+int launch_halo3_m16_spade(HaloArgs a, hipStream_t st) {
+    constexpr int WM = 4, WN = 2, BN = 128;
+    constexpr int shm = (int)M16Layout<WM, BN>::bytes(2);
+    if (a.H % 8 || a.W % 32 || a.Cg % 32 || a.N % 64 || !a.f16 || a.b_split > 0 || a.A2 || a.C2 || a.addend || a.stats || a.a_split ||
+        a.in_scale || !a.sp_x || !a.sp_mean || !a.sp_rstd || !a.sp_gamma_out || a.sp_gamma_ld < a.N / 2 || (a.sp_gamma_ld & 3))
+        return HOIG_EUNSUPPORTED;
+    a.tiles_x = a.W / 32;
+    a.tiles_y = a.H / 8;
+    a.nmajor = 1;
+    a.nblk_n = (int)hoig_cdiv(a.N, BN);
+    a.nblk = a.Bn * a.tiles_x * a.tiles_y * a.nblk_n;
+    const dim3 grid(a.nblk), block(64 * WM * WN);
+    HOIG_ROUTE_F(halo3_m16_128_spade);
+    if (hoig_tuning(HOIG_TUNE_WDMA16) != 0 && a.N % BN == 0)
+        return hoig_launch<conv_halo3_m16_kernel<2, WM, WN, BN, true, false, true, false, true>, shm>(grid, block, shm, st, a);
+    return hoig_launch<conv_halo3_m16_kernel<2, WM, WN, BN, true, false, false, false, true>, shm>(grid, block, shm, st, a);
+}
+
 int launch_halo_s2_m16(const HaloArgs &a, int ns, bool scatter, hipStream_t st) {
     if (a.N % 64 || a.Cg % 32) return HOIG_EUNSUPPORTED;
     return scatter ? launch_s2<true>(a, ns, st) : launch_s2<false>(a, ns, st);
diff --git a/hoig_amd/csrc/conv_igemm_bf16.hip b/hoig_amd/csrc/conv_igemm_bf16.hip
--- a/hoig_amd/csrc/conv_igemm_bf16.hip
+++ b/hoig_amd/csrc/conv_igemm_bf16.hip
@@ -460,6 +460,29 @@
     return run(Conv{.d = d, .a = x1, .wh = w_hi, .wl = w_lo, .bias = bias, .c = y, .st = (hipStream_t)stream, .a2 = x2, .cg1 = C1, .stats = stats});
 }
 
+extern "C" int hoig_conv2d_fwd_packed_add_stats(const hoig_conv_desc *d, const float *x, const uint16_t *w_hi, const uint16_t *w_lo,
+                                                const float *bias, const float *addend, float *y, double *stats, hoig_stream_t stream) {
+    if (!usable(d, x, w_hi, y, addend)) return HOIG_EINVAL;
+    return run(Conv{.d = d, .a = x, .wh = w_hi, .wl = w_lo, .bias = bias, .c = y, .st = (hipStream_t)stream, .addend = addend, .stats = stats});
+}
+
+extern "C" int hoig_conv2d_fwd_packed_spade(const hoig_conv_desc *d, const float *actv, const uint16_t *w_hi, const uint16_t *w_lo,
+                                            const float *bias, const float *x, const float *mean, const float *rstd, int act, float slope,
+                                            float *y, float *gamma_out, int ld_gamma, hoig_stream_t stream) {
+    if (!usable(d, actv, w_hi, y, x, mean, rstd, gamma_out) || !w_lo) return HOIG_EINVAL;
+    if (d->precision != HOIG_PREC_BF16X3 || d->transposed || d->stride != 1 || d->R != 3 || d->S != 3 || d->pad != 1 || d->Ho != d->Hi ||
+        d->Wo != d->Wi || d->act != HOIG_ACT_NONE || d->Co % 64 || d->Ci % 32 || d->Wi % 32 || d->Hi % 8)
+        return HOIG_EUNSUPPORTED;
+    if (ld_gamma < d->Co / 2 || (ld_gamma & 3)) return HOIG_EINVAL;
+    HaloArgs h;
+    h.A = actv; h.Wh = w_hi; h.Wl = w_lo; h.bias = bias; h.C = y;
+    h.Bn = d->B; h.H = d->Hi; h.W = d->Wi; h.Cg = d->Ci; h.N = d->Co; h.K = 9 * d->Ci;
+    h.pad = 1; h.act = act; h.slope = slope;
+    h.f16 = 1; h.oscale = 1.f / W_SCALE_F16;
+    h.sp_x = x; h.sp_mean = mean; h.sp_rstd = rstd; h.sp_gamma_out = gamma_out; h.sp_gamma_ld = ld_gamma;
+    return launch_halo3_m16_spade(h, (hipStream_t)stream);
+}
+
 extern "C" int hoig_conv2d_fwd_packed_normin(const hoig_conv_desc *d, const float *x, int C1, const float *x2, const uint16_t *w_hi,
                                              const uint16_t *w_lo, const float *bias, const float *in_scale, const float *in_shift,
                                              int in_relu_c0, float *y, double *stats, hoig_stream_t stream) {
diff --git a/hoig_amd/csrc/conv_route.h b/hoig_amd/csrc/conv_route.h
--- a/hoig_amd/csrc/conv_route.h
+++ b/hoig_amd/csrc/conv_route.h
@@ -24,6 +24,7 @@
     FD(halo3_m16_64) FD(halo3_m16_128)                                                                                             \
     D(halo3_m16_64_split) D(halo3_m16_128_split) D(halo3_m16_64_split_pair) D(halo3_m16_128_split_pair)                            \
     F(halo3_m16_64_pair) F(halo3_m16_128_pair) F(halo3_m16_64_normin) F(halo3_m16_128_normin)                                      \
+    F(halo3_m16_128_spade)                                         \
                                                    \
     FD(flat_m16_k3) FD(flat_m16_k5) FD(halo5_m16) FD(halo5_m16_ksplit)                                                             \
      \
diff --git a/hoig_amd/csrc/tuning.h b/hoig_amd/csrc/tuning.h
--- a/hoig_amd/csrc/tuning.h
+++ b/hoig_amd/csrc/tuning.h
@@ -1,3 +1,3 @@
 #pragma once
-enum HoigTuning { HOIG_TUNE_IGEMM16 = 0, HOIG_TUNE_S2_16, HOIG_TUNE_FLAT5, HOIG_TUNE_WFLAT5, HOIG_TUNE_HEAD16, HOIG_TUNE_D_EARLY, HOIG_TUNE_SPLIT_GRADS, HOIG_TUNE_PAIR, HOIG_TUNE_WDMA16, HOIG_TUNE_S2_PIPE, HOIG_TUNE_NORM_IN, HOIG_TUNE_WINO8, HOIG_TUNE_HALO5, HOIG_TUNE_PNG_WINDOW, HOIG_TUNE_COUNT };
+enum HoigTuning { HOIG_TUNE_IGEMM16 = 0, HOIG_TUNE_S2_16, HOIG_TUNE_FLAT5, HOIG_TUNE_WFLAT5, HOIG_TUNE_HEAD16, HOIG_TUNE_D_EARLY, HOIG_TUNE_SPLIT_GRADS, HOIG_TUNE_PAIR, HOIG_TUNE_WDMA16, HOIG_TUNE_S2_PIPE, HOIG_TUNE_NORM_IN, HOIG_TUNE_WINO8, HOIG_TUNE_HALO5, HOIG_TUNE_PNG_WINDOW, HOIG_TUNE_SPADE_EPI, HOIG_TUNE_FWD_ADDEND, HOIG_TUNE_COUNT };
 int hoig_tuning(int id);
diff --git a/hoig_amd/csrc/tuning.hip b/hoig_amd/csrc/tuning.hip
--- a/hoig_amd/csrc/tuning.hip
+++ b/hoig_amd/csrc/tuning.hip
@@ -23,6 +23,8 @@
     {"wino8", 0},
     {"halo5", 1},
     {"png_window", 0},
+    {"spade_epi", 1},
+    {"fwd_addend", 1},
 };
 }
 
diff --git a/hoig_amd/models/networks/generator.py b/hoig_amd/models/networks/generator.py
--- a/hoig_amd/models/networks/generator.py
+++ b/hoig_amd/models/networks/generator.py
@@ -1,3 +1,4 @@
+import contextlib
 import os
 
 import torch
@@ -69,10 +70,13 @@
             self._seg_cache[key] = ops.resize_nearest(seg, h, w)
         return self._seg_cache[key]
 
-    def _spade(self, x, seg, name, act, fork=False):
+    def _spade(self, x, seg, name, act, fork=False, epi=True):
         s = self._seg_at(seg, x.shape[1], x.shape[2])
         actv = self._conv(s, name + '.mlp_shared.0', act=ACT_RELU)
         if name + '.mlp_gb.weight' in self.F:
+            if epi and ops.spade_conv_ok(x, actv, self.F[name + '.mlp_gb.weight']):
+                return ops.spade_conv(x, actv, self.F[name + '.mlp_gb.weight'], self.F[name + '.mlp_gb.bias'], act=act, fork=fork)
+            ops.stats_drop(x)
             gb = ops.conv2d(actv, self.F[name + '.mlp_gb.weight'], self.F[name + '.mlp_gb.bias'], 1, 1)
             return ops.spade_norm_fused(x, gb, act=act, fork=fork)
         gamma = self._conv(actv, name + '.mlp_gamma')
@@ -103,11 +107,17 @@
         h = self._in(h, name + '.main.1', act=ACT_RELU)
         return self._in(self._conv(h, name + '.main.3', to_norm=True), name + '.main.4', residual=x)
 
-    def _spade_resblock(self, x, seg, name):
+    def _sums_for_spade(self, H, W, C):
+        return ops.small_map_sums() if ops.spade_epi_shape_ok(H, W, C) else contextlib.nullcontext()
+
+    def _spade_resblock(self, x, seg, name, spade_next=False):
         h, x = self._spade(x, seg, name + '.norm_0', ACT_RELU, fork=True)
-        dx = self._conv(h, name + '.conv_0', to_norm=True)
-        dx = self._conv(self._spade(dx, seg, name + '.norm_1', ACT_RELU), name + '.conv_1')
-        return ops.add(x, dx)
+        with self._sums_for_spade(*x.shape[1:]):
+            dx = self._conv(h, name + '.conv_0', to_norm=True)
+        h = self._spade(dx, seg, name + '.norm_1', ACT_RELU)
+        with self._sums_for_spade(*x.shape[1:]):
+            return ops.conv2d(h, self.P[name + '.conv_1.weight'], self.P.get(name + '.conv_1.bias'), 1, 1, addend=x,
+                              sums_next=spade_next and ops.spade_epi_shape_ok(*x.shape[1:]))
 
     def _resblock_pair(self, sx, tx, ns, nt, sy):
         on_src, to_main, to_src = sy
@@ -127,14 +137,14 @@
         on_src, to_main, to_src = sy
         P = self.P
         with on_src():
-            hs, sx = self._spade(sx, segs, ns + '.norm_0', ACT_RELU, fork=True)
-        ht, tx = self._spade(tx, segt, nt + '.norm_0', ACT_RELU, fork=True)
+            hs, sx = self._spade(sx, segs, ns + '.norm_0', ACT_RELU, fork=True, epi=False)
+        ht, tx = self._spade(tx, segt, nt + '.norm_0', ACT_RELU, fork=True, epi=False)
         ds, dt = ops.conv2d_pair(to_main(hs), ht, P[ns + '.conv_0.weight'], P[nt + '.conv_0.weight'], P.get(ns + '.conv_0.bias'),
                                  P.get(nt + '.conv_0.bias'), dead_bias=True)
         to_src(ds)
         with on_src():
-            hs = self._spade(ds, segs, ns + '.norm_1', ACT_RELU)
-        ht = self._spade(dt, segt, nt + '.norm_1', ACT_RELU)
+            hs = self._spade(ds, segs, ns + '.norm_1', ACT_RELU, epi=False)
+        ht = self._spade(dt, segt, nt + '.norm_1', ACT_RELU, epi=False)
         ds, dt = ops.conv2d_pair(to_main(hs), ht, P[ns + '.conv_1.weight'], P[nt + '.conv_1.weight'], P.get(ns + '.conv_1.bias'),
                                  P.get(nt + '.conv_1.bias'))
         to_src(ds)
@@ -154,11 +164,15 @@
         return self._resblock_pair(sx, tx, ns, nt, sy)
 
     def _spade_block(self, x, seg, name, down, fork=False):
-        if fork:
-            h, x = self._conv_fork(x, name + '.conv', stride=2)
-            return self._spade(h, seg, name + '.norm', ACT_RELU), x
-        h = self._conv(x, name + '.conv', stride=2, to_norm=True) if down else self._convT(x, name + '.conv')
-        return self._spade(h, seg, name + '.norm', ACT_RELU)
+        w = self.P[name + '.conv.weight']
+        H, W = (x.shape[1] // 2, x.shape[2] // 2) if (down or fork) else (2 * x.shape[1], 2 * x.shape[2])
+        with self._sums_for_spade(H, W, w.shape[0] if (down or fork) else w.shape[1]):
+            if fork:
+                h, x = self._conv_fork(x, name + '.conv', stride=2)
+            else:
+                h = self._conv(x, name + '.conv', stride=2, to_norm=True) if down else self._convT(x, name + '.conv')
+        h = self._spade(h, seg, name + '.norm', ACT_RELU)
+        return (h, x) if fork else h
 
     def _bg_net_steps(self, x, out):
         c, p = self.cfg, 'bg_model.model'
@@ -190,10 +204,11 @@
             return self._spade_block(x, seg, p + '.encoders.%d' % i, True, fork=True)
         return self._conv_in_relu(x, p + '.encoders.%d' % i, stride=2, fork=True)
 
-    def _resnet(self, x, seg, p, i):
+    def _resnet(self, x, seg, p, i, chained=False):
         c = self.cfg
-        if (c.spade_layers[1] if i < c.repeat_num // 2 else c.spade_layers[2]):
-            return self._spade_resblock(x, seg, p + '.resnets.%d' % i)
+        spade = lambda k: k < c.repeat_num and (c.spade_layers[1] if k < c.repeat_num // 2 else c.spade_layers[2])
+        if spade(i):
+            return self._spade_resblock(x, seg, p + '.resnets.%d' % i, spade_next=chained and bool(spade(i + 1)))
         return self._resblock(x, p + '.resnets.%d' % i)
 
     def _decode_level(self, x, enc, seg, p, i):
@@ -229,7 +244,7 @@
             enc.append(e)
             yield
         for i in range(self.cfg.repeat_num):
-            e = self._resnet(e, seg, p, i)
+            e = self._resnet(e, seg, p, i, chained=True)
             yield
         for i in range(self.cfg.n_down):
             e = self._decode_level(e, enc, seg, p, i)
diff --git a/hoig_amd/ops.py b/hoig_amd/ops.py
--- a/hoig_amd/ops.py
+++ b/hoig_amd/ops.py
@@ -525,8 +525,8 @@
 
 class _Conv(Function):
     @staticmethod
-    def forward(ctx, x, w, b, stride, pad, transposed, act, slope, out_hw, prec, dead_bias=False, fork=False):
-        _chk(x, 'x'); _chk(w, 'w'); _chk(b, 'bias')
+    def forward(ctx, x, w, b, stride, pad, transposed, act, slope, out_hw, prec, dead_bias=False, fork=False, addend=None, sums_next=False):
+        _chk(x, 'x'); _chk(w, 'w'); _chk(b, 'bias'); _chk(addend, 'addend')
         assert x.is_contiguous() and x.dim() == 4
         B, Hi, Wi, Ci = x.shape
         if transposed:
@@ -542,14 +542,20 @@
         Ho, Wo = out_hw
         y = torch.empty((B, Ho, Wo, Co), dtype=x.dtype, device=x.device)
         d = ConvDesc(B, Hi, Wi, Ci, Ho, Wo, Co, R, S, stride, pad, 1 if transposed else 0, act, slope, prec)
-        _conv_fwd_raw(d, x, w, b, y, transposed, norm_next=dead_bias)
+        if addend is not None:
+            assert addend.shape == y.shape and addend.is_contiguous() and not fork
+            assert act == L.ACT_NONE, 'an addend goes with an un-activated convolution (the backward reads the activation from y)'
+            _conv_fwd_raw(d, x, w, b, y, transposed, norm_next=sums_next, addend=addend)
+        else:
+            _conv_fwd_raw(d, x, w, b, y, transposed, norm_next=dead_bias)
+        ctx.has_addend = addend is not None
         ctx.d = d
         ctx.d_dg, ctx.d_wg = _bwd_descs(d)
         ctx.transposed = transposed
         ctx.has_bias = b is not None and not dead_bias
         ctx.save_for_backward(x, w, b, y if act != L.ACT_NONE else None)
         ctx.fork = fork
-        ctx.split_ok = dead_bias and _split_backward_ok(d, w, ctx.has_bias, transposed)
+        ctx.split_ok = dead_bias and addend is None and _split_backward_ok(d, w, ctx.has_bias, transposed)
         if fork:
             ctx.set_materialize_grads(False)
             return y, x
@@ -561,7 +567,7 @@
         x, w, b, y = ctx.saved_tensors
         d = ctx.d
         if dy is None:
-            return (dxr,) + (None,) * 11
+            return (dxr,) + (None,) * 13
         dy = dy.contiguous()
         if _take_split(ctx, dy):
             return _Conv._backward_split(ctx, dy, dxr, x, w)
@@ -590,7 +596,7 @@
         if ctx.needs_input_grad[0]:
             dx = torch.empty_like(x)
             _conv_dgrad_raw(ctx.d_dg, g, w, dx, ctx.transposed, addend=dxr.contiguous() if dxr is not None else None)
-        return dx, dw_ret, db_ret, None, None, None, None, None, None, None, None, None
+        return (dx, dw_ret, db_ret) + (None,) * 9 + (dy if ctx.has_addend else None, None)
 
     @staticmethod
     def _backward_split(ctx, dys, dxr, x, w):
@@ -605,10 +611,15 @@
             dx = torch.empty_like(x)
             add = dxr.contiguous() if dxr is not None else None
             _dgrad_from_split(ctx.d_dg, dys, w, _packed_planes(w, False, True), add, dx, unsplit)
-        return (dx, (dw if (ctx.needs_input_grad[1] and ret_w) else None)) + (None,) * 10
-
-
-def conv2d(x, w, b=None, stride=1, pad=0, act=L.ACT_NONE, slope=0.0, prec=None, dead_bias=False):
+        return (dx, (dw if (ctx.needs_input_grad[1] and ret_w) else None)) + (None,) * 12
+
+
+def conv2d(x, w, b=None, stride=1, pad=0, act=L.ACT_NONE, slope=0.0, prec=None, dead_bias=False, addend=None, sums_next=False):
+    if addend is not None:
+        if not torch.is_grad_enabled() or not L.lib.hoig_set_tuning(b'fwd_addend', -1):
+            return add(addend, conv2d(x, w, b, stride, pad, act, slope, prec, dead_bias))
+        return _Conv.apply(x, w, b, stride, pad, False, act, slope, None, precision if prec is None else prec, dead_bias, False, addend,
+                           sums_next)
     y = _Conv.apply(x, w, b, stride, pad, False, act, slope, None, precision if prec is None else prec, dead_bias)
     return _tag_split(y) if getattr(y.grad_fn, 'split_ok', False) else y
 
@@ -928,7 +939,20 @@
     return (1 if co > 32 else 0) | (2 if ci > 32 else 0)
 
 
-def _conv_fwd_raw(d, x, w, b, y, transposed=False, norm_next=False):
+def _conv_fwd_raw(d, x, w, b, y, transposed=False, norm_next=False, addend=None):
+    if addend is not None:
+        if d.precision not in (L.PREC_F32, L.PREC_F16F6) and packed_planes(d.Ci, d.Co) & 1:
+            ws = _conv_stats_workspace(y) if norm_next else None
+            hi, lo = _packed_planes(w, transposed, False)
+            for acc in ((ws, None) if ws is not None else (None,)):
+                if L.attempt('hoig_conv2d_fwd_packed_add_stats', ctypes.byref(d), _p(x), _p(hi), _p(lo), _p(b), _p(addend), _p(y), _p(acc), _st()):
+                    if acc is not None:
+                        _stats_offer(y)
+                    return
+        t = torch.empty_like(y)
+        _conv_fwd_ladder(d, x, w, b, t, transposed, False)
+        L.call('hoig_add', _p(addend), _p(t), _p(y), y.numel(), _st())
+        return
     if _conv_fwd_ladder(d, x, w, b, y, transposed, norm_next):
         _stats_offer(y)
 
diff --git a/hoig_amd/ops_norm.py b/hoig_amd/ops_norm.py
--- a/hoig_amd/ops_norm.py
+++ b/hoig_amd/ops_norm.py
@@ -4,6 +4,11 @@
 from torch.autograd import Function
 
 from . import _lib as L
+import ctypes
+import types
+
+from . import ops as _o
+from ._lib import ConvDesc
 from .ops import _chk, _claim_split, _grad_epoch, _grad_target, _offer_split, _p, _st, _writes_split
 
 _norm_ws = {}
@@ -50,6 +55,16 @@
     pend = _stats_pending.get(key)
     if pend is not None and pend[0] == x.data_ptr():
         _norm_workspace(1, x.device)
+
+
+def _stats_have(x):
+    B, H, W_, C = x.shape
+    return _stats_pending.get((x.device, torch.cuda.current_stream(x.device).cuda_stream)) == (x.data_ptr(), B, H * W_, C)
+
+
+def stats_drop(x):
+    if x.is_cuda and x.shape[1] * x.shape[2] <= 1024:
+        _stats_drop(x)
 
 
 def _stats_offer(y):
@@ -176,3 +191,68 @@
     if fork and not x.requires_grad:
         return _SpadeFused.apply(x, gb, act, slope, eps), x
     return _SpadeFused.apply(x, gb, act, slope, eps, fork)
+
+
+def spade_epi_shape_ok(H, W_, C, Ci=None):
+    return (torch.is_grad_enabled() and _o.precision == L.PREC_BF16X3 and L.lib.hoig_set_tuning(b'spade_epi', -1) != 0
+            and W_ % 32 == 0 and H % 8 == 0 and C % 32 == 0 and (Ci is None or Ci % 32 == 0))
+
+
+def spade_conv_ok(x, actv, w):
+    B, H, W_, C = x.shape
+    return (x.is_cuda and spade_epi_shape_ok(H, W_, C, actv.shape[-1]) and tuple(w.shape) == (2 * C, actv.shape[-1], 3, 3)
+            and actv.shape[:3] == x.shape[:3] and _stats_have(x))
+
+
+class _SpadeConv(Function):
+
+    @staticmethod
+    def forward(ctx, x, actv, w, b, act, slope, eps, prec, fork=False):
+        _chk(x); _chk(actv); _chk(w); _chk(b)
+        assert x.is_contiguous() and actv.is_contiguous()
+        B, H, W_, C = x.shape
+        HW, Ci = H * W_, actv.shape[-1]
+        d = ConvDesc(B, H, W_, Ci, H, W_, 2 * C, 3, 3, 1, 1, 0, L.ACT_NONE, 0.0, prec)
+        mean = torch.empty(B * C, dtype=torch.float32, device=x.device)
+        rstd = torch.empty_like(mean)
+        y = torch.empty_like(x)
+        gb = torch.empty((B, H, W_, 2 * C), dtype=torch.float32, device=x.device)
+        ws, have = _norm_workspace(L.lib.hoig_inorm_workspace_bytes(B, HW, C) // 4, x.device, take=(x.data_ptr(), B, HW, C))
+        if have:
+            L.call('hoig_inorm_stats_from_sums', _p(x), B, HW, C, eps, _p(mean), _p(rstd), _p(ws), _st())
+        else:
+            L.call('hoig_inorm_stats', _p(x), B, HW, C, eps, _p(mean), _p(rstd), _p(ws), _st())
+        hi, lo = _o._packed_planes(w, False, False)
+        if not L.attempt('hoig_conv2d_fwd_packed_spade', ctypes.byref(d), _p(actv), _p(hi), _p(lo), _p(b), _p(x), _p(mean), _p(rstd), act,
+                         slope, _p(y), _p(gb), 2 * C, _st()):
+            _o._conv_fwd_raw(d, actv, w, b, gb)
+            L.call('hoig_inorm_apply_ld', _p(x), _p(mean), _p(rstd), 2, _p(gb), gb.data_ptr() + 4 * C, 2 * C, act, slope, None,
+                   _p(y), B, HW, C, _st())
+        ctx.cfg = (act, slope, B, HW, C)
+        ctx.d = d
+        ctx.split_tok = _claim_split(x)
+        ctx.save_for_backward(x, mean, rstd, gb, y if act != L.ACT_NONE else None, actv, w, b)
+        if fork:
+            ctx.set_materialize_grads(False)
+            return y, x
+        return y
+
+    @staticmethod
+    def backward(ctx, dy, dxr=None):
+        x, mean, rstd, gb, y, actv, w, b = ctx.saved_tensors
+        if dy is None:
+            return (dxr,) + (None,) * 8
+        norm = types.SimpleNamespace(saved_tensors=(x, mean, rstd, gb, y), cfg=ctx.cfg, split_tok=ctx.split_tok)
+        dx, dgb = _SpadeFused.backward(norm, dy, dxr)[:2]
+        conv = types.SimpleNamespace(saved_tensors=(actv, w, b, None), d=ctx.d, transposed=False, has_bias=b is not None, has_addend=False,
+                                     needs_input_grad=ctx.needs_input_grad[1:4])
+        conv.d_dg, conv.d_wg = _o._bwd_descs(ctx.d)
+        dactv, dw, db = _o._Conv.backward(conv, dgb)[:3]
+        return dx, dactv, dw, db, None, None, None, None, None
+
+
+def spade_conv(x, actv, w, b=None, act=L.ACT_NONE, fork=False, slope=0.0, eps=1e-5, prec=None):
+    prec = _o.precision if prec is None else prec
+    if fork and not x.requires_grad:
+        return _SpadeConv.apply(x, actv, w, b, act, slope, eps, prec), x
+    return _SpadeConv.apply(x, actv, w, b, act, slope, eps, prec, fork)
diff --git a/include/hoig_kernels.h b/include/hoig_kernels.h
--- a/include/hoig_kernels.h
+++ b/include/hoig_kernels.h
@@ -81,6 +81,12 @@
 int hoig_conv2d_cat_fwd_packed_stats(const hoig_conv_desc *d, const float *x1, int C1, const float *x2, const uint16_t *w_hi,
                                      const uint16_t *w_lo, const float *bias , float *y, double *stats,
                                      hoig_stream_t stream);
+int hoig_conv2d_fwd_packed_add_stats(const hoig_conv_desc *d, const float *x, const uint16_t *w_hi, const uint16_t *w_lo,
+                                     const float *bias , const float *addend, float *y, double *stats ,
+                                     hoig_stream_t stream);
+int hoig_conv2d_fwd_packed_spade(const hoig_conv_desc *d, const float *actv, const uint16_t *w_hi, const uint16_t *w_lo,
+                                 const float *bias , const float *x, const float *mean, const float *rstd, int act, float slope,
+                                 float *y, float *gamma_out, int ld_gamma, hoig_stream_t stream);
 int hoig_conv2d_fwd_stats(const hoig_conv_desc *d, const float *x, const float *w, const float *bias , float *y, double *stats,
                           hoig_stream_t stream);
 int hoig_conv2d_bwd_data_packed_add(const hoig_conv_desc *d, const float *dy, const uint16_t *wt_hi, const uint16_t *wt_lo,
```

New measurement: 134.4 images/s, median of 6. About the same (+0.9%).
